# Vegeta2020/SE-SSD

Hardware: NVIDIA H100
Metric: frames_per_sec (higher is better)
Workload: dtype f32

## Files before the change

include/sessd_b200.h:

```cpp
#ifndef SESSD_B200_H
#define SESSD_B200_H

#include <stddef.h>
#include <stdint.h>

#ifdef __cplusplus
extern "C" {
#endif

#define SESSD_OK 0
#define SESSD_EINVAL (-1)
#define SESSD_ECAPACITY (-2)
#define SESSD_EWORKSPACE (-3)

const char *sessd_version(void);
long long sessd_launch_count(void);

typedef struct {
    float voxel_size[3];
    float range_min[3];
    float range_max[3];
    int grid[3];
    int max_points;
    int max_voxels;
    int num_feat;
} sessd_voxel_cfg;

size_t sessd_voxelize_workspace_bytes(int max_total_points, int batch, const sessd_voxel_cfg *cfg);

int sessd_voxelize(const float *d_points, const int *d_frame_off, int batch, int max_total_points,
                   const sessd_voxel_cfg *cfg, float *d_voxels, int *d_coors, int *d_num_points, float *d_mean,
                   int *d_num_voxels, void *workspace, size_t workspace_bytes, void *stream);

int sessd_voxelize_host(const float *h_points, int num_points, const sessd_voxel_cfg *cfg, float *h_voxels,
                        int *h_coors_zyx , int *h_num_points);

typedef struct {
    int batch;
    int shape[3];
} sessd_grid;

size_t sessd_hash_bytes(int max_rows, int *capacity_out);
int sessd_hash_build(const int *d_coors , const int *d_n, int max_rows, sessd_grid grid,
                     uint64_t *d_table, int capacity, void *stream);

size_t sessd_bitmap_words(sessd_grid grid);
size_t sessd_scan_scratch_bytes(size_t n_items);

int sessd_subm_rulebook(const int *d_coors, const int *d_n, int max_rows, sessd_grid grid, const int ksize[3],
                        int index_kind , const void *d_index, int hash_capacity,
                        int *d_nbr, void *stream);

int sessd_strided_rulebook(const int *d_in_coors, const int *d_n_in, int max_in, sessd_grid in_grid,
                           int in_index_kind, const void *d_in_index, int in_hash_capacity,
                           const int ksize[3], const int stride[3], const int padding[3],
                           sessd_grid out_grid, void *d_out_bitmap , void *d_scan_scratch,
                           int *d_out_coors, int *d_n_out, int max_out, int *d_nbr, int *d_status, void *stream);

int sessd_tile_list_stride(int kvol);
int sessd_rulebook_tile_lists(const int *d_nbr, int kvol, const int *d_n_out, int max_out, void *d_tiles, void *stream);
size_t sessd_rulebook_pairs_workspace_bytes(int max_rows, int kvol);
int sessd_rulebook_pairs(const int *d_nbr, const int *d_n_out, int max_rows, int kvol, int *d_pairs_in,
                         int *d_pairs_out, int *d_pair_num, void *workspace, size_t workspace_bytes, void *stream);

int sessd_spconv_forward(const float *d_in_feat, int cin, const int *d_nbr, int kvol, const int *d_n_out,
                         int max_out, const float *d_weight, int cout, const float *d_scale, const float *d_shift,
                         int relu, float *d_out_feat, void *stream);

int sessd_sparse_to_dense(const float *d_feat, const int *d_coors, const int *d_n, int max_rows, int channels,
                          sessd_grid grid, float *d_out, void *stream);
int sessd_sparse_to_dense_indexed(const float *d_feat, int max_rows, const void *d_bitmap_index, int channels, sessd_grid grid,
                                  float *d_out, void *stream);

int sessd_spconv_forward_rows(const float *d_in_feat, int cin, const int *d_nbr, int kvol, const int *d_n_out, int max_out,
                              const float *d_weight, int cout, const float *d_scale, const float *d_shift, int relu,
                              float *d_out_feat, float *d_amax_out, void *stream);
int sessd_spconv_forward_rows_planes(const float *d_in_feat, int cin, const int *d_nbr, int kvol, const int *d_n_out, int max_out,
                                     const float *d_weight, int cout, const float *d_scale, const float *d_shift, int relu,
                                     const float *d_amax_in, float gain, float shift_max, float *d_out_feat, void *d_out_planes, int cpo,
                                     float *d_out_info, void *stream);
int sessd_spconv_forward_cg(const void *d_in_planes, int cp, int plane_rows, const float *d_in_info, const void *d_tiles, int kvol,
                            const int *d_n_out, int max_out, const void *d_weight_h2, int cout, const float *d_scale, const float *d_shift,
                            int relu, float gain, float shift_max, float *d_out_f32, void *d_out_planes, float *d_out_info, void *stream);
void sessd_set_sp_cg_deep(int on);
int sessd_spconv_cg_blocks_per_sm(int cp, int cout, int deep);
int sessd_absmax_rows(const float *d_feat, const int *d_n, int max_rows, int channels, float *d_amax, void *stream);

int sessd_rulebook_transpose(const int *d_nbr, int kvol, const int *d_n_out, int max_out, int max_in, int *d_nbr_t, void *stream);
int sessd_sparse_split_planes(const float *d_x, const int *d_n, int max_rows, int channels, float *d_info, void *d_planes, int cp, void *stream);
int sessd_dense_grad_gather(const float *d_grad, const int *d_coors, const int *d_n, int max_rows, int channels, sessd_grid grid,
                            float *d_out, void *stream);
int sessd_spconv_wgrad_items(int max_out, int kvol);
size_t sessd_spconv_wgrad_workspace_bytes(int max_out, int kvol, int cin, int cout);
int sessd_spconv_wgrad_rows(const float *d_in_feat, int cin, const float *d_gout, int cout, const void *d_tiles, int kvol,
                            const int *d_n_out, int max_out, float *d_gw, void *d_ws, size_t ws_bytes, void *stream);
int sessd_spconv_wgrad_cg(const void *d_in_planes, int cp, const float *d_in_info, const void *d_g_planes, int cout, const float *d_g_info,
                          const void *d_tiles, int kvol, const int *d_n_out, int max_out, float *d_gw, void *d_ws, size_t ws_bytes,
                          void *stream);

typedef struct {
    int batch, in_h, in_w, cin;
    int out_h, out_w, cout;
    int grid_h, grid_w;
    int in_stride;
    int out_stride, out_off_y, out_off_x;
    int ntaps;
    int tap_dy[16], tap_dx[16];
    int relu;
} sessd_conv_desc;

int sessd_bev_conv_p2(const void *d_in_planes, const float *d_in_info, const void *d_weight_h2, int cout_pad, const float *d_scale,
                      const float *d_shift, const float *d_residual, const float *d_resid_info, float gain, float shift_max,
                      float *d_out_f32, void *d_out_planes, float *d_out_info, const sessd_conv_desc *desc, const int *d_items,
                      void *stream);
int sessd_bev_deconv_p2(const void *d_in_planes, const float *d_in_info, const void *d_weight_h2, int cout_pad, const float *d_scale,
                        const float *d_shift, const float *d_residual, const float *d_resid_info, float gain, float shift_max,
                        float *d_out_f32, void *d_out_planes, float *d_out_info, int batch, int in_h, int in_w, int cin, int cout,
                        int relu, const int *d_items, void *stream);
long long sessd_bev_skip_plan_words(int batch, int h, int w, int *offsets);
int sessd_bev_skip_plan(const void *d_bitmap_index, sessd_grid grid, int *d_plan, void *stream);
int sessd_bev_skip_fill(const int *d_record, float *d_out_f32, void *d_out_planes, int cout, void *stream);
int sessd_bev_wgrad_items(const sessd_conv_desc *desc);
size_t sessd_bev_wgrad_workspace_bytes(const sessd_conv_desc *desc);
int sessd_bev_wgrad(const void *d_in_planes, const float *d_in_info, const void *d_g_planes, const float *d_g_info,
                    const sessd_conv_desc *desc, float *d_gw, void *d_ws, size_t ws_bytes, void *stream);
int sessd_bev_split_planes(const float *d_x, long long n, float *d_info, void *d_planes, void *stream);
int sessd_sparse_to_dense_planes(const float *d_feat, int max_rows, const void *d_bitmap_index, int channels, sessd_grid grid,
                                 const float *d_amax, float *d_info, void *d_planes, void *stream);
int sessd_ssfa_fuse_planes(const float *d_x0, const float *d_x1, const float *d_w0, const float *d_w1, float s0, float t0, float s1,
                           float t1, int num_pixels, int channels, float *d_out, const float *d_info0, const float *d_info1,
                           float *d_out_info, void *d_planes, void *stream);

int sessd_absmax(const float *d_x, long long n, float *d_amax, void *stream);


typedef struct {
    float cnt_thresh;
    float dist_edge[4];
    float sigma2[3];
    float suppressed_thresh;
    float centerness_pow;
    int centerness;
} sessd_dinms_cfg;

#define SESSD_DINMS_MAX_PRE 4096

typedef struct {
    int batch;
    int num_anchors;
    int anchors_per_loc;
    int head_stride;
    float score_thresh;
    int nms_pre_max;
    int nms_post_max;
    float nms_iou_thresh;
    int nms_ge;
    float post_range[6];
    float direction_offset;
    int use_frustum;
    int nms_mode;
    sessd_dinms_cfg dinms;
} sessd_post_cfg;

size_t sessd_postprocess_workspace_bytes(const sessd_post_cfg *cfg);

int sessd_postprocess(const float *d_head, const float *d_anchors, const float *d_frustum,
                      const sessd_post_cfg *cfg, float *d_boxes, float *d_scores, int *d_labels, int *d_count,
                      int *d_aux, int *d_sel_anchor, void *workspace, size_t workspace_bytes, void *stream);

int sessd_postprocess_packed(const float *d_head, const float *d_anchors, const float *d_frustum,
                             const sessd_post_cfg *cfg, float *d_boxes, float *d_scores, int *d_labels, int *d_count,
                             int *d_aux, int *d_sel_anchor, float *d_packed, int *d_meta, const int *d_num_voxels,
                             const int *d_status, void *workspace, size_t workspace_bytes, void *stream);

size_t sessd_rotate_nms_workspace_bytes(int max_boxes, int pre_max);
int sessd_rotate_nms(const float *d_boxes5, const float *d_scores, const int *d_n, int max_boxes, int pre_max,
                     int post_max, float iou_thresh, int ge, int *d_keep, int *d_num_keep, void *workspace,
                     size_t workspace_bytes, void *stream);

size_t sessd_rotate_weighted_nms_workspace_bytes(int max_boxes, int pre_max);
int sessd_rotate_weighted_nms(const float *d_boxes7, const float *d_boxes5, const float *d_scores, const float *d_iou_preds,
                              const int *d_labels, const int *d_dirs, const float *d_anchors, const int *d_n, int max_boxes,
                              int pre_max, const sessd_dinms_cfg *cfg, float *d_out_boxes, float *d_out_scores, int *d_out_labels,
                              int *d_out_dirs, int *d_keep, int *d_selected, int *d_count, void *workspace, size_t workspace_bytes,
                              void *stream);

int sessd_boxes_overlap_bev(const float *d_a, int n, const float *d_b, int m, float *d_out, void *stream);
int sessd_boxes_aligned_overlap_bev(const float *d_a, const float *d_b, int n, float *d_out, void *stream);
int sessd_boxes_iou_bev(const float *d_a, int n, const float *d_b, int m, float *d_out, void *stream);
int sessd_boxes_iou3d(const float *d_a, int n, const float *d_b, int m, float *d_out, void *stream);
size_t sessd_nms_workspace_bytes(int n);
int sessd_nms_sorted(const float *d_boxes, int n, float thresh, int mode, long long *d_keep, int *d_num_keep,
                     void *workspace, size_t workspace_bytes, void *stream);

size_t sessd_assign_workspace_bytes(int num_anchors, int batch, int max_gt);
int sessd_assign_targets(const float *d_anchors, int num_anchors, const float *d_gt_boxes, const int *d_num_gt, int batch,
                         int max_gt, float matched_thr, float unmatched_thr, int *d_labels, float *d_bbox_targets,
                         float *d_bbox_outside_weights, int *d_pos_anchor, int *d_pos_gt_id, int *d_num_pos,
                         void *workspace, size_t workspace_bytes, void *stream);

#define SESSD_AUGMENT_MAX_GT 256
#define SESSD_AUGMENT_MAX_TRY 128
int sessd_box_collision(const double *d_boxes, int n, const double *d_qboxes, int k, uint8_t *d_out, void *stream);
int sessd_noise_per_box(const float *d_gt_boxes, const int *d_num_gt, const uint8_t *d_valid, int batch, int max_gt,
                        const double *d_loc_noise, const double *d_rot_noise, int num_try, double context, int *d_selected,
                        void *stream);
int sessd_points_in_boxes(const float *d_points, int n, int point_stride, const float *d_boxes, int m, double context, uint8_t *d_mask,
                          void *stream);
int sessd_augment_points(const float *d_points, const int *d_frame_off, int batch, int max_frame_points, const float *d_gt_boxes,
                         const int *d_num_gt, const uint8_t *d_valid, int max_gt, const double *d_loc_noise, const double *d_rot_noise,
                         int num_try, const int *d_selected, double context, const float *d_global, const int *d_perm,
                         const uint8_t *d_labeled, float *d_points_raw, float *d_points_out, void *stream);
int sessd_augment_boxes(const float *d_gt_boxes, const int *d_num_gt, const uint8_t *d_valid, const uint8_t *d_target, int batch,
                        int max_gt, const double *d_loc_noise, const double *d_rot_noise, int num_try, const int *d_selected,
                        const float *d_global, const float *range_bev, float *d_boxes_raw, int *d_num_raw, float *d_boxes_out,
                        int *d_num_out, float *d_boxes_global, int *d_num_global, void *stream);

int sessd_gtaug_select_host(const double *h_corners, int num_boxes, int num_cand, uint8_t *h_accepted);
size_t sessd_gtaug_paste_workspace_bytes(int batch, int num_points, int num_objects);
int sessd_gtaug_paste(const float *d_points, const int *d_frame_off, int batch, int num_points, const int *d_obj_off, const int *d_obj_ids,
                      int num_objects, int max_paste_points, const float *d_db_points, const int *d_db_off, const int *d_db_count,
                      const double *d_db_boxes, int db_size, void *d_workspace, size_t workspace_bytes, float *d_points_out, int capacity,
                      int *d_frame_off_out, void *stream);

#define SESSD_SADA_MAX_IDS (6 * SESSD_AUGMENT_MAX_GT)
int sessd_sada_pyramids(const float *d_boxes, int num_boxes, float *d_pyramids, float *d_planes, void *stream);
int sessd_sada_membership(const float *d_points, int n, const int *d_n, const float *d_planes, int num_pyramids, const int *d_ids, int num_ids,
                          uint32_t *d_bits, int *d_counts, void *stream);
size_t sessd_sada_compact_workspace_bytes(int n);
int sessd_sada_compact(const float *d_points, int n, const int *d_n, const uint32_t *d_bits, int num_ids, const int *d_counts, int min_count,
                       void *d_workspace, size_t workspace_bytes, float *d_out, int capacity, int *d_num_out, void *stream);
size_t sessd_sada_fps_workspace_bytes(int n, int num_ids);
int sessd_sada_fps(const float *d_points, int n, const int *d_n, const uint32_t *d_bits, int num_ids, const int *d_counts, int min_count, int k,
                   void *d_workspace, size_t workspace_bytes, float *d_out, int capacity, int *d_num, void *stream);
int sessd_sada_swap(const float *d_points, int n, const int *d_n, const uint32_t *d_bits, int num_pairs, const int *d_counts, const float *d_pyramids,
                    int num_pyramids, const int *d_ids, int max_swap_points, float *d_out, int capacity, const int *d_num_in,
                    int *d_num_out, void *stream);
int sessd_sada_shuffle(const float *d_points, const int *d_frame_off, int batch, int max_frame_points, const int *d_perm, float *d_out,
                       void *stream);

size_t sessd_prep_frustum_compact_workspace_bytes(int num_points);
int sessd_prep_frustum_compact(const float *d_points, const int *d_frame_off, int batch, int num_points, const double *d_planes,
                               void *d_workspace, size_t workspace_bytes, float *d_points_out, int capacity, int *d_frame_off_out, void *stream);
int sessd_prep_box_count(const float *d_points, const int *d_frame_off, int batch, int num_points, const double *d_box_planes,
                         const int *d_box_off, int num_boxes, int *d_counts, void *stream);
size_t sessd_prep_box_gather_workspace_bytes(int num_boxes);
int sessd_prep_box_gather(const float *d_points, const int *d_frame_off, int batch, int num_points, const double *d_box_planes,
                          const double *d_centres, const int *d_box_off, int num_boxes, const int *d_counts, int num_rows, void *d_workspace,
                          size_t workspace_bytes, float *d_rows_out, int capacity, int *d_obj_off, void *stream);

size_t sessd_head_loss_workspace_bytes(int batch);
size_t sessd_odiou_loss_workspace_bytes(int batch);
int sessd_odiou_loss(const float *d_head, const float *d_anchors, const int *d_labels, const float *d_reg_targets, int batch,
                     int num_anchors, int anchors_per_loc, int head_stride, float w_odiou, const float *d_losses, float *d_odiou_sum,
                     float *d_grad_head, void *workspace, size_t workspace_bytes, void *stream);
int sessd_odiou_pairs_host(const float *h_gboxes, const float *h_qboxes, int n, float *h_odiou, float *h_grad_q);
size_t sessd_iou_pred_loss_workspace_bytes(int batch);
int sessd_iou_pred_loss(const float *d_head, const float *d_anchors, const int *d_labels, const float *d_reg_targets, int batch,
                        int num_anchors, int anchors_per_loc, int head_stride, float sigma, float w_iou, float *d_losses,
                        float *d_grad_head, void *workspace, size_t workspace_bytes, void *stream);
int sessd_head_loss(const float *d_head, const float *d_anchors, const int *d_labels, const float *d_reg_targets, int batch,
                    int num_anchors, int anchors_per_loc, int head_stride, float alpha, float sigma, float dir_offset,
                    float pos_cls_weight, float neg_cls_weight, float w_cls, float w_loc, float w_dir, float *d_losses,
                    float *d_grad_head, void *workspace, size_t workspace_bytes, void *stream);

int sessd_axpby(float *d_y, const float *d_x, float a, float b, long long n, void *stream);
int sessd_adamw_step(float *d_param, const float *d_grad, float *d_exp_avg, float *d_exp_avg_sq, long long n, float lr, float beta1,
                     float beta2, float eps, float weight_decay, int step, void *stream);
size_t sessd_grad_sqnorm_workspace_bytes(long long n);
int sessd_grad_sqnorm(const float *d_x, long long n, float max_norm, float *d_out, void *d_workspace, void *stream);
int sessd_adamw_clip_ema_step(float *d_param, float *d_grad, float *d_exp_avg, float *d_exp_avg_sq, long long n, float lr, float beta1,
                              float beta2, float eps, float weight_decay, int step, const float *d_clip_coef, float *d_ema, double ema_alpha,
                              void *stream);

#define SESSD_KITTI_REC 13
#define SESSD_KITTI_PERSON_SITTING 11
#define SESSD_KITTI_VAN 12
typedef struct {
    int num_frames;
    const int *gt_off;
    const double *gt;
    const int *gt_code;
    const int *gt_occluded;
    const int *dc_off;
    const double *dc;
    const int *dt_off;
    const int *dt_cnt;
    const double *dt;
    const int *dt_code;
    const long long *ov_off;
} SessdKittiFrames;
size_t sessd_kitti_convert_workspace_bytes(long long capacity);
int sessd_kitti_convert_detections(const float *d_boxes7, const float *d_scores, const int *d_labels, const int *d_off, int num_frames,
                                   long long capacity, const double *d_calib, const int *d_image_hw, const int *d_label_code,
                                   int num_labels, double *d_rec, int *d_label, int *d_code, int *d_cnt, void *workspace,
                                   size_t workspace_bytes, void *stream);
int sessd_kitti_overlaps(const SessdKittiFrames *frames, int metric, int z_axis, double z_center, double *d_overlaps, void *stream);
size_t sessd_kitti_eval_workspace_bytes(int num_frames, long long total_gt, long long overlap_elems, int num_configs, int compute_aos);
int sessd_kitti_eval(const SessdKittiFrames *frames, int max_frame_dt, int metric, int z_axis, double z_center, int num_configs,
                     const int *d_cfg, const double *d_min_overlap, int compute_aos, long long total_gt, long long overlap_elems,
                     double *d_thresholds, int *d_num_thresholds, double *d_precision, double *d_aos, double *d_map, void *workspace,
                     size_t workspace_bytes, void *stream);

#ifdef __cplusplus
}
#endif
#endif
```

se-ssd_b200/csrc/bevconv_p2.cu:

```cuda
#include "bevconv_p2.cuh"

namespace sessd {

__global__ void __launch_bounds__(256) bev_split_planes_kernel(const float4 *__restrict__ x, long long n4, float *__restrict__ info,
                                                               __half *__restrict__ planes, long long plane_stride) {
    const float s = pow2_scale_for_bound(__ldg(info));
    if (blockIdx.x == 0 && threadIdx.x == 0) info[1] = s;
    for (long long i = blockIdx.x * (long long)blockDim.x + threadIdx.x; i < n4; i += (long long)gridDim.x * blockDim.x) {
        const float4 v = __ldg(x + i);
        const float a[4] = {v.x * s, v.y * s, v.z * s, v.w * s};
        __align__(8) __half hi[4], lo[4];
#pragma unroll
        for (int t = 0; t < 4; ++t) {
            hi[t] = __float2half_rn(a[t]);
            lo[t] = __float2half_rn(a[t] - __half2float(hi[t]));
        }
        *reinterpret_cast<uint2 *>(planes + 4 * i) = *reinterpret_cast<const uint2 *>(hi);
        *reinterpret_cast<uint2 *>(planes + plane_stride + 4 * i) = *reinterpret_cast<const uint2 *>(lo);
    }
}

}

using namespace sessd;

extern "C" int sessd_bev_conv_p2(const void *d_in_planes, const float *d_in_info, const void *d_weight_h2, int cout_pad, const float *d_scale,
                                 const float *d_shift, const float *d_residual, const float *d_resid_info, float gain, float shift_max,
                                 float *d_out_f32, void *d_out_planes, float *d_out_info, const sessd_conv_desc *desc, const int *d_items,
                                 void *stream) {
    return p2_conv<kP2Planes>(d_in_planes, d_in_info, d_weight_h2, cout_pad, d_scale, d_shift, d_residual, d_resid_info, gain, shift_max,
                              d_out_f32, d_out_planes, d_out_info, desc, stream, d_items);
}

extern "C" int sessd_bev_deconv_p2(const void *d_in_planes, const float *d_in_info, const void *d_weight_h2, int cout_pad, const float *d_scale,
                                   const float *d_shift, const float *d_residual, const float *d_resid_info, float gain, float shift_max,
                                   float *d_out_f32, void *d_out_planes, float *d_out_info, int batch, int in_h, int in_w, int cin, int cout,
                                   int relu, const int *d_items, void *stream) {
    return p2_deconv<kP2Planes>(d_in_planes, d_in_info, d_weight_h2, cout_pad, d_scale, d_shift, d_residual, d_resid_info, gain, shift_max,
                                d_out_f32, d_out_planes, d_out_info, batch, in_h, in_w, cin, cout, relu, stream, d_items);
}

extern "C" int sessd_bev_split_planes(const float *d_x, long long n, float *d_info, void *d_planes, void *stream) {
    if (!d_x || !d_info || !d_planes || n < 4 || (n & 3) || ((uintptr_t)d_x & 15)) return SESSD_EINVAL;
    SESSD_LAUNCH(bev_split_planes_kernel, persistent_grid(n / 4, 256), 256, 0, stream, reinterpret_cast<const float4 *>(d_x), n / 4, d_info,
                 (__half *)d_planes, n);
    return last_error();
}
```

se-ssd_b200/csrc/bevconv_p2.cuh:

```cuda
#pragma once
#include <cuda_fp16.h>

#include "tc_common.cuh"

namespace sessd {

constexpr int kP2TileU = 8, kP2TileV = 16;
constexpr int kP2MaxCopies = 6, kP2MaxRowsV = 18;
constexpr int kP2BStages = 6, kP2MaxBStages = 12;
constexpr int kP2MmaWarps = 8;
constexpr int kP2PatchWarp = 8, kP2WeightWarp = 9;
constexpr int kP2Threads = 320;
constexpr int kP2ThreadsRegA = 384, kP2RegsConsumer = 232, kP2RegsProducer = 40;
static_assert(2 * (kP2RegsConsumer - 168) <= 168 - kP2RegsProducer, "the consumers take what the producers release");
constexpr int kP2MaxSmem = 227 * 1024;
constexpr int kP2Chunk = 32;
constexpr int kP2ItemsHeader = 32;
enum { kP2Planes = 0, kP2SplitF16 = 1 };
enum { kP2NoProbe = 0, kP2ProbeClocks = 1, kP2ProbeLoads = 2 };

struct P2Params {
    int batch, cin, cout;
    int in_stride;
    int out_h, out_w;
    int grid_u, grid_v;
    int u_is_x;
    int out_stride, nclass;
    int cls_ntaps[4], cls_off_u[4], cls_off_v[4];
    int tap_copy[4][9], tap_row[4][9], tap_w[4][9];
    int ncopies, rows_v, pitch_u;
    int copy_u[kP2MaxCopies], copy_v[kP2MaxCopies];
    int copy_bytes, patch_bytes, npatch;
    int load_bytes, staging_bytes;
    int bring_bytes;
    int out_info_scale;
    const float *in_amax;
    int relu, n_tile, nblocks;
    int bstages, bstage_bytes;
    int tiles_u, tiles_v, tiles, total;
    int cls_order[4];
    const float *in_info;
    const float *resid_info;
    float gain, shift_max;
    float *out_info;
    long long out_plane_stride;
    const int *items;
    long long *prof;
};

enum P2Prof {
    kProfCta,
    kProfItems,
    kProfSteps,
    kProfItemClk,
    kProfBFull,
    kProfPatchFull,
    kProfMmaWait,
    kProfEpilogue,
    kProfPatchEmpty,
    kProfPatchTotal,
    kProfBEmpty,
    kProfBTotal,
    kP2ProfWords = 16
};

__device__ __forceinline__ int p2_item_count(const P2Params &p) { return p.items ? __ldg(p.items) : p.total; }
__device__ __forceinline__ int p2_item(const P2Params &p, int k) { return p.items ? __ldg(p.items + kP2ItemsHeader + k) : k; }

struct P2ItemIndex { int rank, nb, t; };
__host__ __device__ __forceinline__ P2ItemIndex p2_item_index(int g, int nblocks, int tiles) {
    const int rank = g / (nblocks * tiles), rem = g - rank * (nblocks * tiles), nb = rem / tiles;
    return {rank, nb, rem - nb * tiles};
}

struct P2Item { int cls, n0, b, u0, v0, ntaps; };

__device__ __forceinline__ P2Item p2_decode(const P2Params &p, int g) {
    P2Item it;
    const P2ItemIndex ix = p2_item_index(g, p.nblocks, p.tiles);
    int t = ix.t;
    it.cls = p.cls_order[ix.rank];
    it.n0 = ix.nb * p.n_tile;
    const int tu = t % p.tiles_u; t /= p.tiles_u;
    const int tv = t % p.tiles_v;
    it.b = t / p.tiles_v;
    it.u0 = tu * kP2TileU; it.v0 = tv * kP2TileV;
    it.ntaps = p.cls_ntaps[it.cls];
    return it;
}

template <int N>
__device__ __forceinline__ void p2_wgmma(float *d, uint64_t da, uint64_t db, uint32_t accumulate) {
    if constexpr (N == 32) wgmma_f16_n32(d, da, db, accumulate);
    else if constexpr (N == 64) wgmma_f16_n64(d, da, db, accumulate);
    else if constexpr (N == 128) wgmma_f16_n128(d, da, db, accumulate);
    else wgmma_f16_n256(d, da, db, accumulate);
}

template <int N>
__device__ __forceinline__ void p2_wgmma_ra(float *d, const uint32_t *a, uint64_t db, uint32_t accumulate) {
    if constexpr (N == 32) wgmma_f16_ra_n32(d, a, db, accumulate);
    else if constexpr (N == 64) wgmma_f16_ra_n64(d, a, db, accumulate);
    else if constexpr (N == 128) wgmma_f16_ra_n128(d, a, db, accumulate);
    else wgmma_f16_ra_n256(d, a, db, accumulate);
}

template <bool PROFILE>
__device__ __forceinline__ long long p2_tick() {
    if constexpr (PROFILE) return clock64();
    return 0;
}
template <bool PROFILE>
__device__ __forceinline__ void p2_tock(long long &clk, long long t0) {
    if constexpr (PROFILE) clk += clock64() - t0;
}

__device__ __forceinline__ void p2_split_patch(const P2Params &p, const unsigned char *staging, unsigned char *planes, float s_in, int ctid) {
    const int rows = p.rows_v * kP2TileU;
    const int copy_in = p.staging_bytes / p.ncopies;
    const int items = p.ncopies * rows * 4;
    for (int i = ctid; i < items; i += kP2MmaWarps * 32) {
        const int j = i & 3, r = (i >> 2) % rows, c = (i >> 2) / rows;
        unsigned char *hi = planes + 2 * c * p.copy_bytes + r * 64 + ((j ^ ((r >> 1) & 3)) << 4);
        const float4 *src = reinterpret_cast<const float4 *>(staging + c * copy_in + r * 128 + j * 32);
        const float4 a = src[0], b = src[1];
        const float x[8] = {a.x * s_in, a.y * s_in, a.z * s_in, a.w * s_in, b.x * s_in, b.y * s_in, b.z * s_in, b.w * s_in};
        __align__(16) __half h[8], l[8];
#pragma unroll
        for (int t = 0; t < 8; ++t) { h[t] = __float2half_rn(x[t]); l[t] = __float2half_rn(x[t] - __half2float(h[t])); }
        *reinterpret_cast<uint4 *>(hi) = *reinterpret_cast<const uint4 *>(h);
        *reinterpret_cast<uint4 *>(hi + p.copy_bytes) = *reinterpret_cast<const uint4 *>(l);
    }
    asm volatile("fence.proxy.async.shared::cta;\n" ::: "memory");
    asm volatile("bar.sync 1, %0;\n" ::"n"(kP2MmaWarps * 32) : "memory");
}

template <int NT, int MODE, bool REGA = false, int PROBE = kP2NoProbe>
__global__ void __launch_bounds__(REGA ? kP2ThreadsRegA : kP2Threads, 1) bev_conv_p2_kernel(const __grid_constant__ CUtensorMap map_a,
                                                                   const __grid_constant__ CUtensorMap map_b,
                                                                   const float *__restrict__ scale, const float *__restrict__ shift,
                                                                   const float *__restrict__ resid, float *__restrict__ out_f32,
                                                                   __half *__restrict__ out_planes, P2Params p) {
    static_assert(!REGA || MODE == kP2Planes, "register-fed A reads the TMA-written planes");
    constexpr bool PROFILE = PROBE != kP2NoProbe, LOADS_ONLY = PROBE == kP2ProbeLoads;
    extern __shared__ unsigned char smem_raw[];
    unsigned char *tiles = (unsigned char *)(((uintptr_t)smem_raw + 1023) & ~(uintptr_t)1023);
    unsigned char *patches = tiles + p.bring_bytes;
    unsigned char *staging = patches + p.npatch * p.patch_bytes;
    uint64_t *bars = (uint64_t *)(staging + p.npatch * p.staging_bytes);
    uint64_t *patch_full = bars, *patch_empty = bars + 2, *b_full = bars + 4, *b_empty = bars + 4 + kP2MaxBStages;
    uint32_t *s_aoff = (uint32_t *)(b_empty + kP2MaxBStages);
    float *s_scale = (float *)(((uintptr_t)(s_aoff + 4 * 9) + 15) & ~(uintptr_t)15), *s_shift = s_scale + p.cout;

    const int warp = threadIdx.x >> 5, lane = threadIdx.x & 31;
    if (threadIdx.x == kP2PatchWarp * 32) prefetch_tensormap(&map_a);
    if (threadIdx.x == kP2WeightWarp * 32) prefetch_tensormap(&map_b);
    const int nchunks = p.cin / kP2Chunk;
    const int nitems = p2_item_count(p);
    const uint32_t b_plane_bytes = (uint32_t)p.n_tile * 64u;

    if (threadIdx.x == 0) {
        for (int s = 0; s < 2; ++s) { mbar_init(&patch_full[s], 1); mbar_init(&patch_empty[s], kP2MmaWarps); }
        for (int s = 0; s < p.bstages; ++s) { mbar_init(&b_full[s], 1); mbar_init(&b_empty[s], kP2MmaWarps); }
        asm volatile("fence.mbarrier_init.release.cluster;\n" ::: "memory");
    }
    for (int idx = threadIdx.x; idx < p.nclass * 9; idx += blockDim.x) {
        const int c = idx / 9, t = idx - c * 9;
        s_aoff[idx] = REGA ? (uint32_t)p.tap_row[c][t] : (uint32_t)((2 * p.tap_copy[c][t] * p.copy_bytes + p.tap_row[c][t] * 512) >> 4);
    }
    for (int n = threadIdx.x; n < p.cout; n += blockDim.x) {
        s_scale[n] = scale ? __ldg(scale + n) : 1.f;
        s_shift[n] = shift ? __ldg(shift + n) : 0.f;
    }
    __syncthreads();
    long long clk[kP2ProfWords] = {};
    const long long t_start = p2_tick<PROFILE>();
    long long *prof_rec = PROFILE ? p.prof + (size_t)blockIdx.x * kP2ProfWords : nullptr;

    if (warp >= kP2MmaWarps) {
        if constexpr (REGA) setmaxnreg_dec<kP2RegsProducer>();
        if (warp == kP2PatchWarp) {
            int pb = 0;
            uint32_t pph = 0;
            const uint32_t patches_u32 = smem_u32(patches);
            for (int k = blockIdx.x; k < nitems; k += gridDim.x) {
                const P2Item it = p2_decode(p, p2_item(p, k));
                const int bu = it.u0 * p.in_stride, bv = it.v0 * p.in_stride;
                for (int cc = 0; cc < nchunks; ++cc) {
                    { const long long t0 = p2_tick<PROFILE>(); mbar_wait<REGA>(&patch_empty[pb], pph ^ 1u); p2_tock<PROFILE>(clk[kProfPatchEmpty], t0); }
                    if (elect_one()) {
                        mbar_expect_tx(&patch_full[pb], (uint32_t)p.load_bytes);
                        if constexpr (MODE == kP2Planes) {
                            uint32_t dst = patches_u32 + (uint32_t)(pb * p.patch_bytes);
                            for (int c = 0; c < p.ncopies; ++c, dst += 2u * (uint32_t)p.copy_bytes) {
                                const int cu = bu + p.copy_u[c], cv = bv + p.copy_v[c];
                                tma_load_5d(dst, &map_a, &patch_full[pb], cc * kP2Chunk, cu, cv, it.b, 0);
                                tma_load_5d(dst + (uint32_t)p.copy_bytes, &map_a, &patch_full[pb], cc * kP2Chunk, cu, cv, it.b, 1);
                            }
                        } else {
                            const uint32_t copy_in = (uint32_t)(p.staging_bytes / p.ncopies);
                            uint32_t dst = smem_u32(staging) + (uint32_t)(pb * p.staging_bytes);
                            for (int c = 0; c < p.ncopies; ++c, dst += copy_in)
                                tma_load_5d(dst, &map_a, &patch_full[pb], cc * kP2Chunk, bu + p.copy_u[c], bv + p.copy_v[c], it.b, 0);
                        }
                    }
                    __syncwarp();
                    if (++pb == p.npatch) { pb = 0; pph ^= 1u; }
                }
            }
            if constexpr (PROFILE)
                if (lane == 0) {
                    prof_rec[kProfPatchEmpty] = clk[kProfPatchEmpty];
                    prof_rec[kProfPatchTotal] = clock64() - t_start;
                }
        } else if (warp == kP2WeightWarp) {
            int S = 0;
            uint32_t bph = 0;
            for (int k = blockIdx.x; k < nitems; k += gridDim.x) {
                const P2Item it = p2_decode(p, p2_item(p, k));
                for (int cc = 0; cc < nchunks; ++cc)
                    for (int tap = 0; tap < it.ntaps; ++tap) {
                        { const long long t0 = p2_tick<PROFILE>(); mbar_wait<REGA>(&b_empty[S], bph ^ 1u); p2_tock<PROFILE>(clk[kProfBEmpty], t0); }
                        if (elect_one()) {
                            unsigned char *st = tiles + S * p.bstage_bytes;
                            const int wtap = p.tap_w[it.cls][tap];
                            mbar_expect_tx(&b_full[S], 2 * b_plane_bytes);
                            tma_load_4d(st + b_plane_bytes, &map_b, &b_full[S], cc * kP2Chunk, it.n0, wtap, 0);
                            tma_load_4d(st, &map_b, &b_full[S], cc * kP2Chunk, it.n0, wtap, 1);
                        }
                        __syncwarp();
                        if (++S == p.bstages) { S = 0; bph ^= 1u; }
                    }
            }
            if constexpr (PROFILE)
                if (lane == 0) {
                    prof_rec[kProfBEmpty] = clk[kProfBEmpty];
                    prof_rec[kProfBTotal] = clock64() - t_start;
                }
        }
    } else {
        if constexpr (REGA) setmaxnreg_inc<kP2RegsConsumer>();
        const int wg = warp >> 2, wq = warp & 3;
        constexpr int kAcc = NT / 2;
        const uint32_t a_rows = (uint32_t)(wg * 64 * 64) >> 4;
        const uint32_t tiles_lo = desc_lo(smem_u32(tiles));
        const uint32_t patch_lo = desc_lo(smem_u32(patches)) + a_rows;
        const uint32_t plane_lo = b_plane_bytes >> 4;
        const uint32_t copy_lo = (uint32_t)(p.copy_bytes >> 4), patch_sz = (uint32_t)(p.patch_bytes >> 4);
        const uint32_t a_row = (uint32_t)((wg * 8 + wq * 2 + ((lane >> 3) & 1)) * p.pitch_u + (lane & 7)), a_chunk = (uint32_t)(lane >> 4);
        const uint32_t patches_u32 = smem_u32(patches);
        float amax_in = 0.f, s_in = 1.f;
        if constexpr (MODE == kP2Planes) { amax_in = __ldg(p.in_info); s_in = __ldg(p.in_info + 1); }
        if constexpr (MODE == kP2SplitF16) if (p.in_amax) { amax_in = __ldg(p.in_amax); s_in = pow2_scale_for_bound(amax_in); }
        const float inv_sa = 1.f / s_in;
        float bound = amax_in * p.gain + p.shift_max;
        if (p.resid_info) bound += __ldg(p.resid_info);
        const float s_out = pow2_scale_for_bound(bound);
        if (blockIdx.x == 0 && threadIdx.x == 0 && p.out_info && p.out_info_scale) p.out_info[1] = s_out;
        float vmax = 0.f;
        const int per_cls = p.nblocks * p.tiles;
        int S = 0, pb = 0;
        uint32_t bph = 0, pph = 0;
        for (int k = blockIdx.x; k < nitems; k += gridDim.x) {
            const long long t_item = p2_tick<PROFILE>();
            const int g = p2_item(p, k);
            const int cls = p.cls_order[g / per_cls];
            const int ntaps = p.cls_ntaps[cls];
            const uint32_t *aoff = s_aoff + cls * 9;
            float acc[NT];
#pragma unroll
            for (int i = 0; i < NT; ++i) acc[i] = 0.f;
            int prevS = -1, prev_pb = -1;
            bool first = true;
            if constexpr (REGA) {
                uint32_t frag[2][16];
                int tap = 0;
                uint32_t pbase = 0;
                auto load_frags = [&](uint32_t *fa) {
                    if (tap == 0) {
                        { const long long t0 = p2_tick<PROFILE>(); mbar_wait<REGA>(&patch_full[pb], pph); p2_tock<PROFILE>(clk[kProfPatchFull], t0); }
                        pbase = patches_u32 + (uint32_t)(pb * p.patch_bytes);
                    }
                    if constexpr (!LOADS_ONLY) {
                        const uint32_t r = a_row + aoff[tap];
                        const uint32_t a_hi = pbase + r * 64u + ((a_chunk ^ ((r >> 1) & 3u)) << 4), a_lo = a_hi + (uint32_t)p.copy_bytes;
                        ldsm_x4(fa, a_hi);
                        ldsm_x4(fa + 4, a_hi ^ 32u);
                        ldsm_x4(fa + 8, a_lo);
                        ldsm_x4(fa + 12, a_lo ^ 32u);
                    }
                };
                auto step_ra = [&](const uint32_t *fa, uint32_t *fn, bool more) {
                    { const long long t0 = p2_tick<PROFILE>(); mbar_wait<REGA>(&b_full[S], bph); p2_tock<PROFILE>(clk[kProfBFull], t0); }
                    const uint64_t db_lo = kDescSw64Hi | (uint64_t)(tiles_lo + (uint32_t)(S * (p.bstage_bytes >> 4)));
                    const uint64_t db_hi = db_lo + (uint64_t)plane_lo;
                    if constexpr (!LOADS_ONLY) {
                        wgmma_fence();
                        p2_wgmma_ra<2 * NT>(acc, fa, db_lo, first ? 0u : 1u);
                        p2_wgmma_ra<2 * NT>(acc, fa + 4, db_lo + 2, 1u);
                        wgmma_commit();
                    }
                    first = false;
                    if constexpr (PROFILE) ++clk[kProfSteps];
                    { const long long t0 = p2_tick<PROFILE>(); wgmma_wait<1>(); p2_tock<PROFILE>(clk[kProfMmaWait], t0); }
                    if (lane == 0 && prevS >= 0) mbar_arrive(&b_empty[prevS]);
                    prevS = S;
                    if (++S == p.bstages) { S = 0; bph ^= 1u; }
                    if (++tap == ntaps) {
                        tap = 0;
                        if (lane == 0) mbar_arrive(&patch_empty[pb]);
                        if (++pb == p.npatch) { pb = 0; pph ^= 1u; }
                    }
                    if (more) load_frags(fn);
                    if constexpr (!LOADS_ONLY) {
                        wgmma_fence();
                        p2_wgmma_ra<NT>(acc, fa + 8, db_hi, 1u);
                        p2_wgmma_ra<NT>(acc, fa + 12, db_hi + 2, 1u);
                        wgmma_commit();
                    }
                };
                const int nsteps = nchunks * ntaps;
                load_frags(frag[0]);
#pragma unroll 1
                for (int st = 0; st + 1 < nsteps; st += 2) { step_ra(frag[0], frag[1], true); step_ra(frag[1], frag[0], st + 2 < nsteps); }
                if (nsteps & 1) step_ra(frag[0], frag[1], false);
            } else {
                for (int cc = 0; cc < nchunks; ++cc) {
                    { const long long t0 = p2_tick<PROFILE>(); mbar_wait(&patch_full[pb], pph); p2_tock<PROFILE>(clk[kProfPatchFull], t0); }
                    if constexpr (MODE == kP2SplitF16)
                        p2_split_patch(p, staging + pb * p.staging_bytes, patches + pb * p.patch_bytes, s_in, threadIdx.x);
                    const uint32_t pbase = patch_lo + (uint32_t)pb * patch_sz;
#pragma unroll 1
                    for (int tap = 0; tap < ntaps; ++tap) {
                        { const long long t0 = p2_tick<PROFILE>(); mbar_wait(&b_full[S], bph); p2_tock<PROFILE>(clk[kProfBFull], t0); }
                        if constexpr (!LOADS_ONLY) {
                            const uint64_t da_hi = kDescSw64Hi | (uint64_t)(pbase + aoff[tap]);
                            const uint64_t da_lo = da_hi + (uint64_t)copy_lo;
                            const uint64_t db_lo = kDescSw64Hi | (uint64_t)(tiles_lo + (uint32_t)(S * (p.bstage_bytes >> 4)));
                            const uint64_t db_hi = db_lo + (uint64_t)plane_lo;
                            const uint32_t accum = first ? 0u : 1u;
                            wgmma_fence();
                            if constexpr (MODE == kP2Planes) {
                                p2_wgmma<2 * NT>(acc, da_hi, db_lo, accum);
                                p2_wgmma<2 * NT>(acc, da_hi + 2, db_lo + 2, 1u);
                            } else {
                                p2_wgmma<NT>(acc + kAcc, da_hi, db_hi, accum);
                                p2_wgmma<NT>(acc + kAcc, da_hi + 2, db_hi + 2, 1u);
                                p2_wgmma<NT>(acc, da_hi, db_lo, accum);
                                p2_wgmma<NT>(acc, da_hi + 2, db_lo + 2, 1u);
                            }
                            p2_wgmma<NT>(acc, da_lo, db_hi, 1u);
                            p2_wgmma<NT>(acc, da_lo + 2, db_hi + 2, 1u);
                            wgmma_commit();
                        }
                        first = false;
                        if constexpr (PROFILE) ++clk[kProfSteps];
                        { const long long t0 = p2_tick<PROFILE>(); wgmma_wait<1>(); p2_tock<PROFILE>(clk[kProfMmaWait], t0); }
                        if (lane == 0) {
                            if (prevS >= 0) mbar_arrive(&b_empty[prevS]);
                            if (prev_pb >= 0) mbar_arrive(&patch_empty[prev_pb]);
                        }
                        prevS = S;
                        prev_pb = (tap == ntaps - 1) ? pb : -1;
                        if (++S == p.bstages) { S = 0; bph ^= 1u; }
                    }
                    if (p.npatch == 1) {
                        { const long long t0 = p2_tick<PROFILE>(); wgmma_wait<0>(); p2_tock<PROFILE>(clk[kProfMmaWait], t0); }
                        if (lane == 0) {
                            mbar_arrive(&b_empty[prevS]);
                            mbar_arrive(&patch_empty[pb]);
                        }
                        prevS = prev_pb = -1;
                    }
                    if (++pb == p.npatch) { pb = 0; pph ^= 1u; }
                }
            }
            { const long long t0 = p2_tick<PROFILE>(); wgmma_wait<0>(); p2_tock<PROFILE>(clk[kProfMmaWait], t0); }
            const long long t_epi = p2_tick<PROFILE>();
            wgmma_fence_regs<NT>(acc);
            if (lane == 0) {
                if (prevS >= 0) mbar_arrive(&b_empty[prevS]);
                if (prev_pb >= 0) mbar_arrive(&patch_empty[prev_pb]);
            }
#pragma unroll
            for (int i = 0; i < kAcc; ++i) acc[i] = acc[kAcc + i] + acc[i];
            const P2Item it = p2_decode(p, g);
            const int q = lane & 3;
            const int r0 = wg * 64 + wq * 16 + (lane >> 2);
            bool rows_ok[2];
            size_t opixs[2];
#pragma unroll
            for (int h = 0; h < 2; ++h) {
                const int r = r0 + 8 * h;
                const int lv = r / kP2TileU, lu = r % kP2TileU;
                const int gu = it.u0 + lu, gv = it.v0 + lv;
                rows_ok[h] = it.b < p.batch && gu < p.grid_u && gv < p.grid_v;
                const int ou = gu * p.out_stride + p.cls_off_u[it.cls], ov = gv * p.out_stride + p.cls_off_v[it.cls];
                const int oy = p.u_is_x ? ov : ou, ox = p.u_is_x ? ou : ov;
                opixs[h] = ((size_t)it.b * p.out_h + (size_t)oy) * p.out_w + (size_t)ox;
            }
#pragma unroll
            for (int j = 0; j < (LOADS_ONLY ? 0 : NT / 32); ++j)
#pragma unroll
                for (int h = 0; h < 2; ++h) {
                    const bool row_ok = rows_ok[h];
                    const size_t opix = opixs[h];
                    float v[8], o[8] = {};
                    quad_transpose8(acc + 16 * j + 2 * h, q, v);
                    const int n = it.n0 + 32 * j + 8 * q;
                    const size_t off = opix * p.cout + n;
                    if (row_ok && n < p.cout) {
                        float sc[8], sh[8];
#pragma unroll
                        for (int t = 0; t < 8; t += 4) {
                            const float4 a = *reinterpret_cast<const float4 *>(s_scale + n + t);
                            const float4 b = *reinterpret_cast<const float4 *>(s_shift + n + t);
                            sc[t] = a.x; sc[t + 1] = a.y; sc[t + 2] = a.z; sc[t + 3] = a.w;
                            sh[t] = b.x; sh[t + 1] = b.y; sh[t + 2] = b.z; sh[t + 3] = b.w;
                        }
#pragma unroll
                        for (int t = 0; t < 8; ++t) {
                            o[t] = fmaf(v[t] * inv_sa, sc[t], sh[t]);
                            if (p.relu) o[t] = fmaxf(o[t], 0.f);
                        }
                        if (resid) {
#pragma unroll
                            for (int t = 0; t < 8; t += 4) {
                                const float4 rr = __ldg(reinterpret_cast<const float4 *>(resid + off + t));
                                o[t] += rr.x; o[t + 1] += rr.y; o[t + 2] += rr.z; o[t + 3] += rr.w;
                            }
                        }
#pragma unroll
                        for (int t = 0; t < 8; ++t) vmax = fmaxf(vmax, fabsf(o[t]));
                        if (out_planes) {
                            __align__(16) __half2 hi[4], lo[4];
#pragma unroll
                            for (int t = 0; t < 4; ++t) {
                                const float x0 = o[2 * t] * s_out, x1 = o[2 * t + 1] * s_out;
                                hi[t] = __floats2half2_rn(x0, x1);
                                const float2 f = __half22float2(hi[t]);
                                lo[t] = __floats2half2_rn(x0 - f.x, x1 - f.y);
                            }
                            *reinterpret_cast<uint4 *>(out_planes + off) = *reinterpret_cast<const uint4 *>(hi);
                            *reinterpret_cast<uint4 *>(out_planes + p.out_plane_stride + off) = *reinterpret_cast<const uint4 *>(lo);
                        }
                    }
                    if (out_f32) {
                        const bool up = q & 2;
                        float keep[4], recv[4];
#pragma unroll
                        for (int t = 0; t < 4; ++t) {
                            keep[t] = up ? o[4 + t] : o[t];
                            recv[t] = __shfl_xor_sync(0xFFFFFFFFu, up ? o[t] : o[4 + t], 2);
                        }
                        const int n_lo = it.n0 + 32 * j + 8 * (q & 1), c_lo = n_lo + 4 * (q >> 1);
                        const float4 w_lo = up ? make_float4(recv[0], recv[1], recv[2], recv[3]) : make_float4(keep[0], keep[1], keep[2], keep[3]);
                        const float4 w_hi = up ? make_float4(keep[0], keep[1], keep[2], keep[3]) : make_float4(recv[0], recv[1], recv[2], recv[3]);
                        if (row_ok && n_lo < p.cout) *reinterpret_cast<float4 *>(out_f32 + opix * p.cout + c_lo) = w_lo;
                        if (row_ok && n_lo + 16 < p.cout) *reinterpret_cast<float4 *>(out_f32 + opix * p.cout + c_lo + 16) = w_hi;
                    }
                }
            if constexpr (PROFILE) {
                const long long t_end = clock64();
                clk[kProfEpilogue] += t_end - t_epi;
                clk[kProfItemClk] += t_end - t_item;
                ++clk[kProfItems];
            }
        }
        if constexpr (PROFILE)
            if (threadIdx.x == 0) {
                clk[kProfCta] = clock64() - t_start;
                for (int w = kProfCta; w <= kProfEpilogue; ++w) prof_rec[w] = clk[w];
            }
        if (p.out_info) {
            const unsigned m = __reduce_max_sync(0xFFFFFFFFu, __float_as_uint(vmax));
            if (lane == 0 && m != 0u) atomicMax(reinterpret_cast<unsigned *>(p.out_info), m);
        }
    }
}

static int encode_map_nd(CUtensorMap *m, const void *base, int rank, const cuuint64_t *dims, const cuuint64_t *strides_bytes ,
                         const cuuint32_t *box, const cuuint32_t *estr, CUtensorMapSwizzle swz,
                         CUtensorMapDataType dtype = CU_TENSOR_MAP_DATA_TYPE_FLOAT16) {
    EncodeTiledFn enc = get_tensor_map_encoder();
    if (!enc) return SESSD_EINVAL;
    CUresult r = enc(m, dtype, (cuuint32_t)rank, const_cast<void *>(base), dims, strides_bytes, box, estr,
                     CU_TENSOR_MAP_INTERLEAVE_NONE, swz, CU_TENSOR_MAP_L2_PROMOTION_L2_256B, CU_TENSOR_MAP_FLOAT_OOB_FILL_NONE);
    return r == CUDA_SUCCESS ? 0 : 700 + (int)r;
}

struct P2Taps { int n, dy[9], dx[9], w[9], off_y, off_x; };

static void p2_deconv_classes(P2Taps cls[4]) {
    for (int c = 0; c < 4; ++c) {
        P2Taps &k = cls[c];
        k = {};
        k.off_y = c >> 1; k.off_x = c & 1;
        for (int dy = k.off_y; dy >= 0; --dy)
            for (int dx = k.off_x; dx >= 0; --dx, ++k.n) {
                k.dy[k.n] = dy; k.dx[k.n] = dx; k.w[k.n] = (k.off_y + 1 - 2 * dy) * 3 + (k.off_x + 1 - 2 * dx);
            }
    }
}

constexpr int p2_n_tile(int cout) { return cout <= 32 ? 32 : 128; }

struct P2Geometry {
    int u_is_x, grid_u, grid_v, tiles_u, tiles_v, tiles;
    int n_tile, nblocks, nclass, total;
    int ntaps[4], off_u[4], off_v[4], order[4];
};

static int p2_geometry(P2Geometry &g, int batch, int grid_h, int grid_w, int cout, int cout_pad, const P2Taps *cls, int nclass) {
    g = {};
    if (batch < 1 || grid_h < 1 || grid_w < 1 || cout < 8 || cout % 8) return SESSD_EINVAL;
    g.n_tile = p2_n_tile(cout);
    if (cout_pad % g.n_tile || cout_pad < cout) return SESSD_EINVAL;
    g.u_is_x = div_up(grid_w, kP2TileU) * div_up(grid_h, kP2TileV) <= div_up(grid_h, kP2TileU) * div_up(grid_w, kP2TileV);
    g.grid_u = g.u_is_x ? grid_w : grid_h; g.grid_v = g.u_is_x ? grid_h : grid_w;
    g.tiles_u = div_up(g.grid_u, kP2TileU); g.tiles_v = div_up(g.grid_v, kP2TileV);
    g.tiles = g.tiles_u * g.tiles_v * batch;
    g.nblocks = cout_pad / g.n_tile;
    g.nclass = nclass; g.total = nclass * g.nblocks * g.tiles;
    for (int c = 0; c < nclass; ++c) {
        g.ntaps[c] = cls[c].n;
        g.off_u[c] = g.u_is_x ? cls[c].off_x : cls[c].off_y;
        g.off_v[c] = g.u_is_x ? cls[c].off_y : cls[c].off_x;
        g.order[c] = c;
    }
    for (int i = 1; i < nclass; ++i)
        for (int k = i; k > 0 && g.ntaps[g.order[k]] > g.ntaps[g.order[k - 1]]; --k) {
            const int tmp = g.order[k]; g.order[k] = g.order[k - 1]; g.order[k - 1] = tmp;
        }
    return 0;
}

static int p2_plan(P2Params &p, const P2Taps *cls, int nclass, int grid_h, int grid_w, int cout_pad, int mode, bool reg_a, int *smem) {
    if (reg_a && (mode != kP2Planes || p.in_stride != 1)) return SESSD_EINVAL;
    if (p.cin < 64 || p.cin % 64) return SESSD_EINVAL;
    P2Geometry g;
    if (p2_geometry(g, p.batch, grid_h, grid_w, p.cout, cout_pad, cls, nclass)) return SESSD_EINVAL;
    p.u_is_x = g.u_is_x; p.grid_u = g.grid_u; p.grid_v = g.grid_v;
    p.tiles_u = g.tiles_u; p.tiles_v = g.tiles_v; p.tiles = g.tiles;
    p.n_tile = g.n_tile; p.nblocks = g.nblocks; p.nclass = g.nclass; p.total = g.total;
    for (int c = 0; c < 4; ++c) {
        p.cls_ntaps[c] = g.ntaps[c]; p.cls_off_u[c] = g.off_u[c]; p.cls_off_v[c] = g.off_v[c]; p.cls_order[c] = g.order[c];
    }
    const int s = p.in_stride;
    p.ncopies = 0;
    int key_u[kP2MaxCopies], key_vm[kP2MaxCopies], vmin[kP2MaxCopies], vmax[kP2MaxCopies];
    for (int c = 0; c < p.nclass; ++c)
        for (int t = 0; t < cls[c].n; ++t) {
            const int tu = p.u_is_x ? cls[c].dx[t] : cls[c].dy[t], tv = p.u_is_x ? cls[c].dy[t] : cls[c].dx[t];
            const int vm = ((tv % s) + s) % s;
            int k = 0;
            for (; k < p.ncopies; ++k)
                if (key_u[k] == tu && key_vm[k] == vm) break;
            if (k == p.ncopies) {
                if (p.ncopies == kP2MaxCopies) return SESSD_EINVAL;
                key_u[k] = tu; key_vm[k] = vm; vmin[k] = tv; vmax[k] = tv;
                ++p.ncopies;
            }
            vmin[k] = min(vmin[k], tv); vmax[k] = max(vmax[k], tv);
        }
    p.rows_v = 0;
    p.pitch_u = kP2TileU;
    for (int k = 0; k < p.ncopies; ++k) p.rows_v = max(p.rows_v, kP2TileV + (vmax[k] - vmin[k]) / s);
    if (p.rows_v > kP2MaxRowsV) return SESSD_EINVAL;
    for (int k = 0; k < p.ncopies; ++k) { p.copy_u[k] = key_u[k]; p.copy_v[k] = vmin[k]; }
    if (reg_a) {
        int umin = key_u[0], umax = key_u[0];
        for (int k = 1; k < p.ncopies; ++k) {
            umin = min(umin, key_u[k]); umax = max(umax, key_u[k]);
            vmin[0] = min(vmin[0], vmin[k]); vmax[0] = max(vmax[0], vmax[k]);
        }
        p.ncopies = 1;
        p.copy_u[0] = umin; p.copy_v[0] = vmin[0];
        p.pitch_u = kP2TileU + umax - umin; p.rows_v = kP2TileV + vmax[0] - vmin[0];
        if (p.pitch_u > 256 || p.rows_v > 256) return SESSD_EINVAL;
    }
    for (int c = 0; c < p.nclass; ++c) {
        for (int t = 0; t < cls[c].n; ++t) {
            const int tu = p.u_is_x ? cls[c].dx[t] : cls[c].dy[t], tv = p.u_is_x ? cls[c].dy[t] : cls[c].dx[t];
            const int vm = ((tv % s) + s) % s;
            int k = 0;
            for (; k < p.ncopies; ++k)
                if (key_u[k] == tu && key_vm[k] == vm) break;
            p.tap_copy[c][t] = reg_a ? 0 : k;
            p.tap_row[c][t] = reg_a ? (tv - p.copy_v[0]) * p.pitch_u + (tu - p.copy_u[0]) : (tv - vmin[k]) / s;
            p.tap_w[c][t] = cls[c].w[t];
        }
    }
    p.copy_bytes = (p.rows_v * p.pitch_u * 64 + 511) & ~511;
    p.patch_bytes = p.ncopies * 2 * p.copy_bytes;
    p.staging_bytes = mode == kP2Planes ? 0 : p.ncopies * p.rows_v * kP2TileU * kP2Chunk * 4;
    p.load_bytes = mode == kP2Planes ? p.ncopies * 2 * p.rows_v * p.pitch_u * 64 : p.staging_bytes;
    const int per_buf = p.patch_bytes + p.staging_bytes, bstage = 2 * p.n_tile * 64;
    const int tail = 1536 + 16 + 2 * 4 * p.cout;
    p.npatch = (kP2BStages * bstage + tail + 2 * per_buf <= kP2MaxSmem) ? 2 : 1;
    p.bstage_bytes = bstage;
    p.bstages = min((kP2MaxSmem - tail - p.npatch * per_buf) / bstage, kP2MaxBStages);
    if (p.bstages < 2) return SESSD_EINVAL;
    p.bring_bytes = p.bstages * bstage;
    *smem = p.bring_bytes + tail + p.npatch * per_buf;
    return 0;
}

template <int MODE, int PROBE = kP2NoProbe>
static int launch_p2(const void *d_in_planes, int in_h, int in_w, const float *d_in_info, const void *d_w, int w_taps, int cout_pad,
                     const float *d_scale, const float *d_shift, const float *d_residual, const float *d_resid_info, float gain,
                     float shift_max, float *d_out_f32, void *d_out_planes, float *d_out_info, P2Params &p, const P2Taps *cls, int nclass,
                     int grid_h, int grid_w, bool reg_a, void *stream) {
    if (!d_in_planes || !d_w || (!d_out_f32 && !d_out_planes)) return SESSD_EINVAL;
    if (MODE == kP2Planes && (!d_in_info || !d_scale)) return SESSD_EINVAL;
    if (MODE != kP2Planes && d_out_planes) return SESSD_EINVAL;
    if (((uintptr_t)d_scale | (uintptr_t)d_shift | (uintptr_t)d_residual | (uintptr_t)d_out_f32 | (uintptr_t)d_out_planes) & 15)
        return SESSD_EINVAL;
    int smem = 0;
    if (p2_plan(p, cls, nclass, grid_h, grid_w, cout_pad, MODE, reg_a, &smem)) return SESSD_EINVAL;
    if (p.items && cout_pad != div_up(p.cout, p.n_tile) * p.n_tile) return SESSD_EINVAL;
    const int s = p.in_stride;
    CUtensorMap map_a, map_b;
    if (MODE != kP2Planes) {
        const cuuint64_t row_w = (cuuint64_t)p.cin * 4, row_h = (cuuint64_t)in_w * p.cin * 4;
        const cuuint64_t dims[5] = {(cuuint64_t)p.cin, (cuuint64_t)(p.u_is_x ? in_w : in_h), (cuuint64_t)(p.u_is_x ? in_h : in_w),
                                    (cuuint64_t)p.batch, 1};
        const cuuint64_t strides[4] = {p.u_is_x ? row_w : row_h, p.u_is_x ? row_h : row_w, (cuuint64_t)in_h * in_w * p.cin * 4,
                                       (cuuint64_t)p.batch * in_h * in_w * p.cin * 4};
        const cuuint32_t box[5] = {(cuuint32_t)kP2Chunk, (cuuint32_t)(kP2TileU * s), (cuuint32_t)(p.rows_v * s), 1, 1};
        const cuuint32_t estr[5] = {1, (cuuint32_t)s, (cuuint32_t)s, 1, 1};
        int rc = encode_map_nd(&map_a, d_in_planes, 5, dims, strides, box, estr, CU_TENSOR_MAP_SWIZZLE_NONE, CU_TENSOR_MAP_DATA_TYPE_FLOAT32);
        if (rc) return rc;
    } else {
        const cuuint64_t row_w = (cuuint64_t)p.cin * 2, row_h = (cuuint64_t)in_w * p.cin * 2;
        const cuuint64_t dims[5] = {(cuuint64_t)p.cin, (cuuint64_t)(p.u_is_x ? in_w : in_h), (cuuint64_t)(p.u_is_x ? in_h : in_w),
                                    (cuuint64_t)p.batch, 2};
        const cuuint64_t strides[4] = {p.u_is_x ? row_w : row_h, p.u_is_x ? row_h : row_w, (cuuint64_t)in_h * in_w * p.cin * 2,
                                       (cuuint64_t)p.batch * in_h * in_w * p.cin * 2};
        const cuuint32_t box[5] = {(cuuint32_t)kP2Chunk, (cuuint32_t)(p.pitch_u * s), (cuuint32_t)(p.rows_v * s), 1, 1};
        const cuuint32_t estr[5] = {1, (cuuint32_t)s, (cuuint32_t)s, 1, 1};
        int rc = encode_map_nd(&map_a, d_in_planes, 5, dims, strides, box, estr, CU_TENSOR_MAP_SWIZZLE_64B);
        if (rc) return rc;
    }
    {
        const cuuint64_t dims[4] = {(cuuint64_t)p.cin, (cuuint64_t)cout_pad, (cuuint64_t)w_taps, 2};
        const cuuint64_t strides[3] = {(cuuint64_t)p.cin * 2, (cuuint64_t)cout_pad * p.cin * 2, (cuuint64_t)w_taps * cout_pad * p.cin * 2};
        const cuuint32_t box[4] = {(cuuint32_t)kP2Chunk, (cuuint32_t)p.n_tile, 1, 1};
        const cuuint32_t estr[4] = {1, 1, 1, 1};
        int rc = encode_map_nd(&map_b, d_w, 4, dims, strides, box, estr, CU_TENSOR_MAP_SWIZZLE_64B);
        if (rc) return rc;
    }
    constexpr bool kRegA = MODE == kP2Planes;
    auto kernel = bev_conv_p2_kernel<128, MODE, false, PROBE>;
    if (p.n_tile == 32) kernel = reg_a ? bev_conv_p2_kernel<32, MODE, kRegA, PROBE> : bev_conv_p2_kernel<32, MODE, false, PROBE>;
    else if (reg_a) kernel = bev_conv_p2_kernel<128, MODE, kRegA, PROBE>;
    static bool attr_done[2][2] = {};
    if (!attr_done[p.n_tile == 32][reg_a]) {
        SESSD_CUDA_TRY(cudaFuncSetAttribute(kernel, cudaFuncAttributeMaxDynamicSharedMemorySize, kP2MaxSmem));
        attr_done[p.n_tile == 32][reg_a] = true;
    }
    p.in_info = MODE == kP2Planes ? d_in_info : nullptr;
    p.in_amax = MODE == kP2SplitF16 ? d_in_info : nullptr;
    p.resid_info = d_residual ? d_resid_info : nullptr;
    if (d_residual && d_out_planes && !d_resid_info) return SESSD_EINVAL;
    p.gain = gain; p.shift_max = shift_max; p.out_info = d_out_info;
    p.out_info_scale = MODE == kP2Planes ? 1 : 0;
    if (d_out_planes && !d_out_info) return SESSD_EINVAL;
    p.out_plane_stride = (long long)p.batch * p.out_h * p.out_w * p.cout;
    static int num_sms = 0;
    if (!num_sms) {
        int dev = 0;
        SESSD_CUDA_TRY(cudaGetDevice(&dev));
        SESSD_CUDA_TRY(cudaDeviceGetAttribute(&num_sms, cudaDevAttrMultiProcessorCount, dev));
    }
    const int grid = p.total < num_sms ? p.total : num_sms;
    SESSD_LAUNCH(kernel, grid, reg_a ? kP2ThreadsRegA : kP2Threads, smem, (cudaStream_t)stream, map_a, map_b, d_scale, d_shift, d_residual, d_out_f32,
                 (__half *)d_out_planes, p);
    return last_error();
}


static int p2_conv_params(const sessd_conv_desc &d, P2Params &p, P2Taps &t) {
    if (d.ntaps < 1 || d.ntaps > 9 || (d.in_stride != 1 && d.in_stride != 2) || d.out_stride < 1) return SESSD_EINVAL;
    if ((d.grid_h - 1) * d.out_stride + d.out_off_y >= d.out_h || (d.grid_w - 1) * d.out_stride + d.out_off_x >= d.out_w) return SESSD_EINVAL;
    p = {};
    p.batch = d.batch; p.cin = d.cin; p.cout = d.cout; p.in_stride = d.in_stride;
    p.out_h = d.out_h; p.out_w = d.out_w; p.out_stride = d.out_stride; p.relu = d.relu;
    t = {};
    t.n = d.ntaps; t.off_y = d.out_off_y; t.off_x = d.out_off_x;
    for (int i = 0; i < d.ntaps; ++i) { t.dy[i] = d.tap_dy[i]; t.dx[i] = d.tap_dx[i]; t.w[i] = i; }
    return 0;
}

static void p2_deconv_params(int batch, int in_h, int in_w, int cin, int cout, int relu, P2Params &p, P2Taps cls[4]) {
    p = {};
    p.batch = batch; p.cin = cin; p.cout = cout; p.in_stride = 1;
    p.out_h = 2 * in_h; p.out_w = 2 * in_w; p.out_stride = 2; p.relu = relu;
    p2_deconv_classes(cls);
}

template <int MODE, int PROBE = kP2NoProbe>
static int p2_conv(const void *d_in_planes, const float *d_in_info, const void *d_weight_h2, int cout_pad, const float *d_scale,
                   const float *d_shift, const float *d_residual, const float *d_resid_info, float gain, float shift_max,
                   float *d_out_f32, void *d_out_planes, float *d_out_info, const sessd_conv_desc *desc, void *stream,
                   const int *d_items = nullptr, long long *d_prof = nullptr, bool smem_a = false) {
    if (!desc || (PROBE != kP2NoProbe && !d_prof)) return SESSD_EINVAL;
    const sessd_conv_desc &d = *desc;
    P2Params p;
    P2Taps t;
    if (p2_conv_params(d, p, t)) return SESSD_EINVAL;
    p.items = d_items;
    p.prof = d_prof;
    return launch_p2<MODE, PROBE>(d_in_planes, d.in_h, d.in_w, d_in_info, d_weight_h2, d.ntaps, cout_pad, d_scale, d_shift, d_residual, d_resid_info, gain,
                     shift_max, d_out_f32, d_out_planes, d_out_info, p, &t, 1, d.grid_h, d.grid_w, MODE == kP2Planes && d.in_stride == 1 && !smem_a,
                     stream);
}

template <int MODE, int PROBE = kP2NoProbe>
static int p2_deconv(const void *d_in_planes, const float *d_in_info, const void *d_weight_h2, int cout_pad, const float *d_scale,
                     const float *d_shift, const float *d_residual, const float *d_resid_info, float gain, float shift_max,
                     float *d_out_f32, void *d_out_planes, float *d_out_info, int batch, int in_h, int in_w, int cin, int cout,
                     int relu, void *stream, const int *d_items = nullptr, long long *d_prof = nullptr) {
    if (PROBE != kP2NoProbe && !d_prof) return SESSD_EINVAL;
    P2Params p;
    P2Taps cls[4];
    p2_deconv_params(batch, in_h, in_w, cin, cout, relu, p, cls);
    p.items = d_items;
    p.prof = d_prof;
    return launch_p2<MODE, PROBE>(d_in_planes, in_h, in_w, d_in_info, d_weight_h2, 9, cout_pad, d_scale, d_shift, d_residual, d_resid_info, gain, shift_max,
                     d_out_f32, d_out_planes, d_out_info, p, cls, 4, in_h, in_w, MODE == kP2Planes, stream);
}

}
```

se-ssd_b200/csrc/bevskip.cu:

```cuda
#include "bevconv_p2.cuh"

namespace sessd {

enum {
    kRecCount = 0, kRecSkipped = 1, kRecNclass = 2, kRecTiles = 3, kRecTilesU = 4, kRecTilesV = 5, kRecUisX = 6, kRecOutStride = 7,
    kRecOutH = 8, kRecOutW = 9, kRecBatch = 10, kRecOffY = 11, kRecOffX = 15, kRecRep = 19, kRecSkipOff = 23, kRecFlagOff = 24
};

enum { kMX, kMB0a, kMB0b, kMX0, kMM0, kMM1, kMO0, kMO1, kMOut, kMTmp, kMB1a, kMB1b, kMX1, kMTmpH, kNumMaps };
constexpr int kNumFullMaps = kMTmp + 1;
constexpr int kSkipLaunches = 13;
constexpr int kSkipThreads = 1024;

struct SkipLaunch : P2Geometry {
    int map;
    int out_stride, out_h, out_w;
    int rec;
};

struct SkipPlan {
    int batch, depth, h, w, h2, w2, nwf, nwh;
    SkipLaunch l[kSkipLaunches];
};

static int skip_launch(SkipLaunch &L, int map, int batch, int grid_h, int grid_w, int out_h, int out_w, int cout, bool deconv) {
    P2Taps cls[4] = {};
    if (deconv) p2_deconv_classes(cls);
    else cls[0].n = 1;
    L.map = map;
    L.out_stride = deconv ? 2 : 1;
    L.out_h = out_h; L.out_w = out_w;
    return p2_geometry(L, batch, grid_h, grid_w, cout, div_up(cout, p2_n_tile(cout)) * p2_n_tile(cout), cls, deconv ? 4 : 1);
}

static long long skip_plan(SkipPlan &P, int batch, int h, int w) {
    if (batch < 1 || h < 4 || w < 4 || (h & 1) || (w & 1)) return 0;
    P.batch = batch; P.h = h; P.w = w; P.h2 = h / 2; P.w2 = w / 2;
    P.nwf = div_up(w, 32); P.nwh = div_up(P.w2, 32);
    const int h2 = P.h2, w2 = P.w2;
    SkipLaunch *L = P.l;
    const int rc = skip_launch(L[0], kMB0a, batch, h, w, h, w, 128, false)
                 | skip_launch(L[1], kMB0b, batch, h, w, h, w, 128, false)
                 | skip_launch(L[2], kMX0, batch, h, w, h, w, 128, false)
                 | skip_launch(L[3], kMB1a, batch, h2, w2, h2, w2, 256, false)
                 | skip_launch(L[4], kMB1b, batch, h2, w2, h2, w2, 256, false)
                 | skip_launch(L[5], kMX1, batch, h2, w2, h2, w2, 256, false)
                 | skip_launch(L[6], kMX0, batch, h, w, h, w, 128, false)
                 | skip_launch(L[7], kMX1, batch, h2, w2, h2, w2, 256, false)
                 | skip_launch(L[8], kMM0, batch, h2, w2, h, w, 128, true)
                 | skip_launch(L[9], kMM1, batch, h2, w2, h, w, 128, true)
                 | skip_launch(L[10], kMO0, batch, h, w, h, w, 128, false)
                 | skip_launch(L[11], kMO1, batch, h, w, h, w, 128, false)
                 | skip_launch(L[12], kMOut, batch, h, w, h, w, 24, false);
    long long words = 0;
    for (int i = 0; i < kSkipLaunches; ++i) {
        L[i].rec = (int)words;
        words += kP2ItemsHeader + L[i].total + 2LL * L[i].nclass * L[i].tiles;
    }
    return rc ? 0 : words;
}

struct BitMap {
    uint32_t *w;
    int h, wd, nw;
    __device__ __forceinline__ bool get(int y, int x) const { return (w[y * nw + (x >> 5)] >> (x & 31)) & 1u; }
    __device__ __forceinline__ uint32_t valid(int i) const {
        const int rem = wd - 32 * i;
        return rem >= 32 ? ~0u : ((1u << rem) - 1u);
    }
};

__device__ void skip_dilate3(const BitMap &in, const BitMap &tmp, const BitMap &out) {
    const int n = in.h * in.nw, last = (in.wd - 1) >> 5;
    for (int idx = threadIdx.x; idx < n; idx += blockDim.x) {
        const int y = idx / in.nw, i = idx - y * in.nw;
        const uint32_t *r = in.w + y * in.nw;
        const uint32_t c = r[i], l = i > 0 ? r[i - 1] : 0u, rr = i + 1 < in.nw ? r[i + 1] : 0u;
        uint32_t hv = c | (c << 1) | (l >> 31) | (c >> 1) | (rr << 31);
        if (i == 0) hv |= 1u;
        if (i == last) hv |= 1u << ((in.wd - 1) & 31);
        tmp.w[idx] = hv & in.valid(i);
    }
    __syncthreads();
    for (int idx = threadIdx.x; idx < n; idx += blockDim.x) {
        const int y = idx / in.nw, i = idx - y * in.nw;
        out.w[idx] = (y == 0 || y == in.h - 1) ? in.valid(i) : (tmp.w[idx - in.nw] | tmp.w[idx] | tmp.w[idx + in.nw]);
    }
    __syncthreads();
}

template <class F>
__device__ void skip_map_from(const BitMap &out, F f) {
    const int warp = threadIdx.x >> 5, lane = threadIdx.x & 31, nwarps = blockDim.x >> 5;
    for (int idx = warp; idx < out.h * out.nw; idx += nwarps) {
        const int y = idx / out.nw, x = (idx - y * out.nw) * 32 + lane;
        const unsigned bits = __ballot_sync(0xFFFFFFFFu, x < out.wd && f(y, x));
        if (lane == 0) out.w[idx] = bits;
    }
    __syncthreads();
}

template <class Pred>
__device__ int skip_compact(int n, Pred pred, int *out, int *s_scan) {
    const int warp = threadIdx.x >> 5, lane = threadIdx.x & 31, nwarps = blockDim.x >> 5;
    int base = 0;
    for (int start = 0; start < n; start += blockDim.x) {
        const int i = start + threadIdx.x;
        const bool v = i < n && pred(i);
        const unsigned bal = __ballot_sync(0xFFFFFFFFu, v);
        if (lane == 0) s_scan[warp] = __popc(bal);
        __syncthreads();
        if (warp == 0) {
            const int own = lane < nwarps ? s_scan[lane] : 0;
            int x = own;
#pragma unroll
            for (int o = 1; o < 32; o <<= 1) {
                const int y = __shfl_up_sync(0xFFFFFFFFu, x, o);
                if (lane >= o) x += y;
            }
            if (lane < nwarps) s_scan[lane] = x - own;
            if (lane == 31) s_scan[32] = x;
        }
        __syncthreads();
        if (v) out[base + s_scan[warp] + __popc(bal & ((1u << lane) - 1u))] = i;
        base += s_scan[32];
        __syncthreads();
    }
    return base;
}

__global__ void __launch_bounds__(kSkipThreads) bev_skip_plan_kernel(const uint2 *__restrict__ bitmap, int *__restrict__ plan, SkipPlan P) {
    extern __shared__ uint32_t s_bits[];
    __shared__ int s_scan[33], s_rep[4];
    BitMap m[kNumMaps];
    {
        uint32_t *p = s_bits;
        for (int i = 0; i < kNumMaps; ++i) {
            const bool full = i < kNumFullMaps;
            m[i].w = p; m[i].h = full ? P.h : P.h2; m[i].wd = full ? P.w : P.w2; m[i].nw = full ? P.nwf : P.nwh;
            p += m[i].h * m[i].nw;
        }
    }
    for (int b = 0; b < P.batch; ++b) {
        const BitMap X = m[kMX];
        for (int idx = threadIdx.x; idx < X.h * X.nw; idx += blockDim.x) {
            const int y = idx / X.nw, i = idx - y * X.nw;
            const int nbits = min(32, X.wd - 32 * i);
            uint32_t acc = 0u;
            for (int z = 0; z < P.depth; ++z) {
                const unsigned long long lin = (((unsigned long long)b * P.depth + z) * P.h + y) * P.w + 32 * i;
                const unsigned sh = (unsigned)(lin & 31);
                const uint32_t lo = __ldg(&bitmap[lin >> 5]).x, hi = sh + nbits > 32 ? __ldg(&bitmap[(lin >> 5) + 1]).x : 0u;
                acc |= __funnelshift_r(lo, hi, sh);
            }
            X.w[idx] = acc & X.valid(i);
        }
        __syncthreads();
        skip_dilate3(m[kMX], m[kMTmp], m[kMB0a]);
        skip_dilate3(m[kMB0a], m[kMTmp], m[kMB0b]);
        skip_dilate3(m[kMB0b], m[kMTmp], m[kMX0]);
        skip_dilate3(m[kMX0], m[kMTmp], m[kMX]);
        {
            const BitMap D = m[kMX];
            skip_map_from(m[kMB1a], [&](int y, int x) { return D.get(2 * y, 2 * x); });
        }
        skip_dilate3(m[kMB1a], m[kMTmpH], m[kMB1b]);
        skip_dilate3(m[kMB1b], m[kMTmpH], m[kMX1]);
        {
            const BitMap T = m[kMX1], R = m[kMX0];
            auto tget = [&](int gy, int gx) { return gy >= T.h || gx >= T.wd || T.get(gy, gx); };
            auto dc = [&](int oy, int ox) {
                const int py = oy & 1, px = ox & 1, gy = oy >> 1, gx = ox >> 1;
                return tget(gy, gx) || (py && tget(gy + 1, gx)) || (px && tget(gy, gx + 1)) || (py && px && tget(gy + 1, gx + 1));
            };
            skip_map_from(m[kMM0], [&](int y, int x) { return dc(y, x) || R.get(y, x); });
            skip_map_from(m[kMM1], dc);
        }
        skip_dilate3(m[kMM0], m[kMTmp], m[kMO0]);
        skip_dilate3(m[kMM1], m[kMTmp], m[kMO1]);
        for (int i = threadIdx.x; i < P.h * P.nwf; i += blockDim.x) m[kMOut].w[i] = m[kMO0].w[i] | m[kMO1].w[i];
        __syncthreads();
        for (int li = 0; li < kSkipLaunches; ++li) {
            const SkipLaunch &L = P.l[li];
            const BitMap &o = m[L.map];
            int *flags = plan + L.rec + kP2ItemsHeader + L.total + L.nclass * L.tiles;
            const int per_frame = L.tiles_u * L.tiles_v;
            for (int idx = threadIdx.x; idx < L.nclass * per_frame; idx += blockDim.x) {
                const int c = idx / per_frame, tf = idx - c * per_frame;
                const int tu = tf % L.tiles_u, tv = tf / L.tiles_u;
                const int u0 = tu * kP2TileU, v0 = tv * kP2TileV;
                bool run = u0 + kP2TileU > L.grid_u || v0 + kP2TileV > L.grid_v;
                if (!run && L.out_stride == 1) {
                    const int y0 = L.u_is_x ? v0 : u0, x0 = L.u_is_x ? u0 : v0;
                    const int ny = L.u_is_x ? kP2TileV : kP2TileU, nx = L.u_is_x ? kP2TileU : kP2TileV;
                    const uint32_t field = (1u << nx) - 1u;
                    for (int y = y0; y < y0 + ny && !run; ++y) run = (o.w[y * o.nw + (x0 >> 5)] >> (x0 & 31)) & field;
                } else if (!run) {
                    for (int r = 0; r < kP2TileU * kP2TileV && !run; ++r) {
                        const int ou = (u0 + (r & 7)) * L.out_stride + L.off_u[c], ov = (v0 + (r >> 3)) * L.out_stride + L.off_v[c];
                        run = L.u_is_x ? o.get(ov, ou) : o.get(ou, ov);
                    }
                }
                flags[c * L.tiles + b * per_frame + tf] = run ? 1 : 0;
            }
        }
        __syncthreads();
    }
    for (int li = 0; li < kSkipLaunches; ++li) {
        const SkipLaunch &L = P.l[li];
        int *rec = plan + L.rec;
        int *items = rec + kP2ItemsHeader, *skipped = items + L.total;
        const int *flags = skipped + L.nclass * L.tiles;
        if (threadIdx.x < 4) s_rep[threadIdx.x] = 0x7FFFFFFF;
        __syncthreads();
        for (int e = threadIdx.x; e < L.nclass * L.tiles; e += blockDim.x)
            if (!flags[e]) atomicMin(&s_rep[e / L.tiles], e % L.tiles);
        __syncthreads();
        const int count = skip_compact(L.total, [&](int g) {
            const P2ItemIndex ix = p2_item_index(g, L.nblocks, L.tiles);
            return flags[L.order[ix.rank] * L.tiles + ix.t] != 0 || ix.t == s_rep[L.order[ix.rank]];
        }, items, s_scan);
        const int nskip = skip_compact(L.nclass * L.tiles, [&](int e) {
            return flags[e] == 0 && e % L.tiles != s_rep[e / L.tiles];
        }, skipped, s_scan);
        if (threadIdx.x == 0) {
            rec[kRecCount] = count; rec[kRecSkipped] = nskip;
            rec[kRecNclass] = L.nclass; rec[kRecTiles] = L.tiles; rec[kRecTilesU] = L.tiles_u; rec[kRecTilesV] = L.tiles_v;
            rec[kRecUisX] = L.u_is_x; rec[kRecOutStride] = L.out_stride; rec[kRecOutH] = L.out_h; rec[kRecOutW] = L.out_w;
            rec[kRecBatch] = P.batch;
            for (int c = 0; c < 4; ++c) {
                rec[kRecOffY + c] = L.u_is_x ? L.off_v[c] : L.off_u[c]; rec[kRecOffX + c] = L.u_is_x ? L.off_u[c] : L.off_v[c];
                rec[kRecRep + c] = c < L.nclass && s_rep[c] != 0x7FFFFFFF ? s_rep[c] : -1;
            }
            rec[kRecSkipOff] = kP2ItemsHeader + L.total;
            rec[kRecFlagOff] = kP2ItemsHeader + L.total + L.nclass * L.tiles;
        }
        __syncthreads();
    }
}

__global__ void __launch_bounds__(256) bev_skip_fill_kernel(const int *__restrict__ rec, float *__restrict__ out_f32,
                                                            __half *__restrict__ out_planes, int cout) {
    const int nskip = __ldg(rec + kRecSkipped);
    if ((int)blockIdx.x >= nskip) return;
    const int tiles = __ldg(rec + kRecTiles), tiles_u = __ldg(rec + kRecTilesU), tiles_v = __ldg(rec + kRecTilesV);
    const int u_is_x = __ldg(rec + kRecUisX), os = __ldg(rec + kRecOutStride), out_h = __ldg(rec + kRecOutH), out_w = __ldg(rec + kRecOutW);
    const long long plane_stride = (long long)__ldg(rec + kRecBatch) * out_h * out_w * cout;
    const int *skipped = rec + __ldg(rec + kRecSkipOff);
    for (int e = blockIdx.x; e < nskip; e += gridDim.x) {
        const int ent = __ldg(skipped + e);
        const int c = ent / tiles, t = ent - c * tiles, r = __ldg(rec + kRecRep + c);
        const int oy0 = __ldg(rec + kRecOffY + c), ox0 = __ldg(rec + kRecOffX + c);
        auto pixel = [&](int tt, int lu, int lv) -> size_t {
            const int tu = tt % tiles_u, rest = tt / tiles_u, tv = rest % tiles_v, b = rest / tiles_v;
            const int gu = tu * kP2TileU + lu, gv = tv * kP2TileV + lv;
            const int gy = u_is_x ? gv : gu, gx = u_is_x ? gu : gv;
            return ((size_t)b * out_h + (size_t)(gy * os + oy0)) * out_w + (size_t)(gx * os + ox0);
        };
        if (out_f32) {
            const int q = cout / 4;
            for (int i = threadIdx.x; i < kP2TileU * kP2TileV * q; i += blockDim.x) {
                const int px = i / q, j = i - px * q;
                const float4 v = reinterpret_cast<const float4 *>(out_f32 + pixel(r, px & 7, px >> 3) * cout)[j];
                reinterpret_cast<float4 *>(out_f32 + pixel(t, px & 7, px >> 3) * cout)[j] = v;
            }
        }
        if (out_planes) {
            const int q = cout / 8, n = kP2TileU * kP2TileV * q;
            for (int i = threadIdx.x; i < 2 * n; i += blockDim.x) {
                const int pl = i / n, k = i - pl * n, px = k / q, j = k - px * q;
                const __half *src = out_planes + pl * plane_stride + pixel(r, px & 7, px >> 3) * cout;
                __half *dst = out_planes + pl * plane_stride + pixel(t, px & 7, px >> 3) * cout;
                reinterpret_cast<uint4 *>(dst)[j] = reinterpret_cast<const uint4 *>(src)[j];
            }
        }
    }
}

}

using namespace sessd;

extern "C" long long sessd_bev_skip_plan_words(int batch, int h, int w, int *offsets) {
    SkipPlan P;
    const long long words = skip_plan(P, batch, h, w);
    if (words && offsets)
        for (int i = 0; i < kSkipLaunches; ++i) offsets[i] = P.l[i].rec;
    return words;
}

extern "C" int sessd_bev_skip_plan(const void *d_bitmap_index, sessd_grid grid, int *d_plan, void *stream) {
    if (!d_bitmap_index || !d_plan || grid.shape[0] < 1) return SESSD_EINVAL;
    SkipPlan P;
    if (!skip_plan(P, grid.batch, grid.shape[1], grid.shape[2])) return SESSD_EINVAL;
    P.depth = grid.shape[0];
    const int smem = 4 * (kNumFullMaps * P.h * P.nwf + (kNumMaps - kNumFullMaps) * P.h2 * P.nwh);
    if (smem > 200 * 1024) return SESSD_EINVAL;
    static int attr_smem = 48 * 1024;
    if (smem > attr_smem) {
        SESSD_CUDA_TRY(cudaFuncSetAttribute(bev_skip_plan_kernel, cudaFuncAttributeMaxDynamicSharedMemorySize, smem));
        attr_smem = smem;
    }
    SESSD_LAUNCH(bev_skip_plan_kernel, 1, kSkipThreads, smem, (cudaStream_t)stream, (const uint2 *)d_bitmap_index, d_plan, P);
    return last_error();
}

extern "C" int sessd_bev_skip_fill(const int *d_record, float *d_out_f32, void *d_out_planes, int cout, void *stream) {
    if (!d_record || (!d_out_f32 && !d_out_planes) || cout < 8 || cout % 8) return SESSD_EINVAL;
    SESSD_LAUNCH(bev_skip_fill_kernel, 2 * kNumSMs, 256, 0, (cudaStream_t)stream, d_record, d_out_f32, (__half *)d_out_planes, cout);
    return last_error();
}
```

se-ssd_b200/sessd_b200/_lib.py:

```python
import ctypes as C
import os

_HERE = os.path.dirname(os.path.abspath(__file__))
LIB_PATH = os.path.join(os.path.dirname(_HERE), "libsessd_b200.so")
LAB_PATH = os.path.join(os.path.dirname(_HERE), "libsessd_b200_lab.so")


class SessdError(RuntimeError):
    pass


class VoxelCfg(C.Structure):
    _fields_ = [("voxel_size", C.c_float * 3), ("range_min", C.c_float * 3), ("range_max", C.c_float * 3),
                ("grid", C.c_int * 3), ("max_points", C.c_int), ("max_voxels", C.c_int), ("num_feat", C.c_int)]


class Grid(C.Structure):
    _fields_ = [("batch", C.c_int), ("shape", C.c_int * 3)]


class ConvDesc(C.Structure):
    _fields_ = [("batch", C.c_int), ("in_h", C.c_int), ("in_w", C.c_int), ("cin", C.c_int),
                ("out_h", C.c_int), ("out_w", C.c_int), ("cout", C.c_int),
                ("grid_h", C.c_int), ("grid_w", C.c_int), ("in_stride", C.c_int),
                ("out_stride", C.c_int), ("out_off_y", C.c_int), ("out_off_x", C.c_int),
                ("ntaps", C.c_int), ("tap_dy", C.c_int * 16), ("tap_dx", C.c_int * 16), ("relu", C.c_int)]


class DinmsCfg(C.Structure):
    _fields_ = [("cnt_thresh", C.c_float), ("dist_edge", C.c_float * 4), ("sigma2", C.c_float * 3), ("suppressed_thresh", C.c_float),
                ("centerness_pow", C.c_float), ("centerness", C.c_int)]


class PostCfg(C.Structure):
    _fields_ = [("batch", C.c_int), ("num_anchors", C.c_int), ("anchors_per_loc", C.c_int), ("head_stride", C.c_int),
                ("score_thresh", C.c_float), ("nms_pre_max", C.c_int), ("nms_post_max", C.c_int),
                ("nms_iou_thresh", C.c_float), ("nms_ge", C.c_int), ("post_range", C.c_float * 6),
                ("direction_offset", C.c_float), ("use_frustum", C.c_int), ("nms_mode", C.c_int), ("dinms", DinmsCfg)]


class KittiFrames(C.Structure):
    _fields_ = [("num_frames", C.c_int), ("gt_off", C.c_void_p), ("gt", C.c_void_p), ("gt_code", C.c_void_p),
                ("gt_occluded", C.c_void_p), ("dc_off", C.c_void_p), ("dc", C.c_void_p), ("dt_off", C.c_void_p),
                ("dt_cnt", C.c_void_p), ("dt", C.c_void_p), ("dt_code", C.c_void_p), ("ov_off", C.c_void_p)]


_vp, _i, _f, _sz, _ll = C.c_void_p, C.c_int, C.c_float, C.c_size_t, C.c_longlong
_I3 = C.POINTER(C.c_int)

SIGNATURES = {
    "sessd_version": (C.c_char_p, []),
    "sessd_launch_count": (_ll, []),
    "sessd_voxelize_workspace_bytes": (_sz, [_i, _i, C.POINTER(VoxelCfg)]),
    "sessd_voxelize": (_i, [_vp, _vp, _i, _i, C.POINTER(VoxelCfg), _vp, _vp, _vp, _vp, _vp, _vp, _sz, _vp]),
    "sessd_voxelize_host": (_i, [_vp, _i, C.POINTER(VoxelCfg), _vp, _vp, _vp]),
    "sessd_hash_bytes": (_sz, [_i, _I3]),
    "sessd_hash_build": (_i, [_vp, _vp, _i, Grid, _vp, _i, _vp]),
    "sessd_bitmap_words": (_sz, [Grid]),
    "sessd_scan_scratch_bytes": (_sz, [_sz]),
    "sessd_subm_rulebook": (_i, [_vp, _vp, _i, Grid, _I3, _i, _vp, _i, _vp, _vp]),
    "sessd_strided_rulebook": (_i, [_vp, _vp, _i, Grid, _i, _vp, _i, _I3, _I3, _I3, Grid, _vp, _vp, _vp, _vp, _i, _vp, _vp, _vp]),
    "sessd_tile_list_stride": (_i, [_i]),
    "sessd_rulebook_tile_lists": (_i, [_vp, _i, _vp, _i, _vp, _vp]),
    "sessd_rulebook_pairs_workspace_bytes": (_sz, [_i, _i]),
    "sessd_rulebook_pairs": (_i, [_vp, _vp, _i, _i, _vp, _vp, _vp, _vp, _sz, _vp]),
    "sessd_spconv_forward": (_i, [_vp, _i, _vp, _i, _vp, _i, _vp, _i, _vp, _vp, _i, _vp, _vp]),
    "sessd_spconv_forward_rows": (_i, [_vp, _i, _vp, _i, _vp, _i, _vp, _i, _vp, _vp, _i, _vp, _vp, _vp]),
    "sessd_spconv_forward_rows_planes": (_i, [_vp, _i, _vp, _i, _vp, _i, _vp, _i, _vp, _vp, _i, _vp, _f, _f, _vp, _vp, _i, _vp, _vp]),
    "sessd_spconv_forward_cg": (_i, [_vp, _i, _i, _vp, _vp, _i, _vp, _i, _vp, _i, _vp, _vp, _i, _f, _f, _vp, _vp, _vp, _vp]),
    "sessd_set_sp_cg_deep": (None, [_i]),
    "sessd_spconv_cg_blocks_per_sm": (_i, [_i, _i, _i]),
    "sessd_absmax_rows": (_i, [_vp, _vp, _i, _i, _vp, _vp]),
    "sessd_rulebook_transpose": (_i, [_vp, _i, _vp, _i, _i, _vp, _vp]),
    "sessd_sparse_split_planes": (_i, [_vp, _vp, _i, _i, _vp, _vp, _i, _vp]),
    "sessd_dense_grad_gather": (_i, [_vp, _vp, _vp, _i, _i, Grid, _vp, _vp]),
    "sessd_spconv_wgrad_items": (_i, [_i, _i]),
    "sessd_spconv_wgrad_workspace_bytes": (_sz, [_i, _i, _i, _i]),
    "sessd_spconv_wgrad_rows": (_i, [_vp, _i, _vp, _i, _vp, _i, _vp, _i, _vp, _vp, _sz, _vp]),
    "sessd_spconv_wgrad_cg": (_i, [_vp, _i, _vp, _vp, _i, _vp, _vp, _i, _vp, _i, _vp, _vp, _sz, _vp]),
    "sessd_sparse_to_dense_indexed": (_i, [_vp, _i, _vp, _i, Grid, _vp, _vp]),
    "sessd_sparse_to_dense": (_i, [_vp, _vp, _vp, _i, _i, Grid, _vp, _vp]),
    "sessd_bev_conv_p2": (_i, [_vp, _vp, _vp, _i, _vp, _vp, _vp, _vp, _f, _f, _vp, _vp, _vp, C.POINTER(ConvDesc), _vp, _vp]),
    "sessd_bev_deconv_p2": (_i, [_vp, _vp, _vp, _i, _vp, _vp, _vp, _vp, _f, _f, _vp, _vp, _vp, _i, _i, _i, _i, _i, _i, _vp, _vp]),
    "sessd_bev_skip_plan_words": (_ll, [_i, _i, _i, _I3]),
    "sessd_bev_skip_plan": (_i, [_vp, Grid, _vp, _vp]),
    "sessd_bev_skip_fill": (_i, [_vp, _vp, _vp, _i, _vp]),
    "sessd_bev_wgrad_items": (_i, [C.POINTER(ConvDesc)]),
    "sessd_bev_wgrad_workspace_bytes": (_sz, [C.POINTER(ConvDesc)]),
    "sessd_bev_wgrad": (_i, [_vp, _vp, _vp, _vp, C.POINTER(ConvDesc), _vp, _vp, _sz, _vp]),
    "sessd_bev_split_planes": (_i, [_vp, _ll, _vp, _vp, _vp]),
    "sessd_sparse_to_dense_planes": (_i, [_vp, _i, _vp, _i, Grid, _vp, _vp, _vp, _vp]),
    "sessd_ssfa_fuse_planes": (_i, [_vp, _vp, _vp, _vp, _f, _f, _f, _f, _i, _i, _vp, _vp, _vp, _vp, _vp, _vp]),
    "sessd_absmax": (_i, [_vp, C.c_longlong, _vp, _vp]),
    "sessd_postprocess_workspace_bytes": (_sz, [C.POINTER(PostCfg)]),
    "sessd_postprocess": (_i, [_vp, _vp, _vp, C.POINTER(PostCfg), _vp, _vp, _vp, _vp, _vp, _vp, _vp, _sz, _vp]),
    "sessd_postprocess_packed": (_i, [_vp, _vp, _vp, C.POINTER(PostCfg), _vp, _vp, _vp, _vp, _vp, _vp, _vp, _vp, _vp, _vp, _vp, _sz, _vp]),
    "sessd_rotate_nms_workspace_bytes": (_sz, [_i, _i]),
    "sessd_rotate_nms": (_i, [_vp, _vp, _vp, _i, _i, _i, _f, _i, _vp, _vp, _vp, _sz, _vp]),
    "sessd_rotate_weighted_nms_workspace_bytes": (_sz, [_i, _i]),
    "sessd_rotate_weighted_nms": (_i, [_vp, _vp, _vp, _vp, _vp, _vp, _vp, _vp, _i, _i, C.POINTER(DinmsCfg), _vp, _vp, _vp, _vp, _vp, _vp, _vp,
                                       _vp, _sz, _vp]),
    "sessd_boxes_overlap_bev": (_i, [_vp, _i, _vp, _i, _vp, _vp]),
    "sessd_boxes_aligned_overlap_bev": (_i, [_vp, _vp, _i, _vp, _vp]),
    "sessd_boxes_iou_bev": (_i, [_vp, _i, _vp, _i, _vp, _vp]),
    "sessd_boxes_iou3d": (_i, [_vp, _i, _vp, _i, _vp, _vp]),
    "sessd_nms_workspace_bytes": (_sz, [_i]),
    "sessd_nms_sorted": (_i, [_vp, _i, _f, _i, _vp, _vp, _vp, _sz, _vp]),
    "sessd_head_loss_workspace_bytes": (_sz, [_i]),
    "sessd_head_loss": (_i, [_vp, _vp, _vp, _vp, _i, _i, _i, _i, _f, _f, _f, _f, _f, _f, _f, _f, _vp, _vp, _vp, _sz, _vp]),
    "sessd_odiou_loss_workspace_bytes": (_sz, [_i]),
    "sessd_odiou_loss": (_i, [_vp, _vp, _vp, _vp, _i, _i, _i, _i, _f, _vp, _vp, _vp, _vp, _sz, _vp]),
    "sessd_odiou_pairs_host": (_i, [_vp, _vp, _i, _vp, _vp]),
    "sessd_iou_pred_loss_workspace_bytes": (_sz, [_i]),
    "sessd_iou_pred_loss": (_i, [_vp, _vp, _vp, _vp, _i, _i, _i, _i, _f, _f, _vp, _vp, _vp, _sz, _vp]),
    "sessd_axpby": (_i, [_vp, _vp, _f, _f, _ll, _vp]),
    "sessd_adamw_step": (_i, [_vp, _vp, _vp, _vp, _ll, _f, _f, _f, _f, _f, _i, _vp]),
    "sessd_grad_sqnorm_workspace_bytes": (_sz, [_ll]),
    "sessd_grad_sqnorm": (_i, [_vp, _ll, _f, _vp, _vp, _vp]),
    "sessd_adamw_clip_ema_step": (_i, [_vp, _vp, _vp, _vp, _ll, _f, _f, _f, _f, _f, _i, _vp, _vp, C.c_double, _vp]),
    "sessd_assign_workspace_bytes": (_sz, [_i, _i, _i]),
    "sessd_assign_targets": (_i, [_vp, _i, _vp, _vp, _i, _i, _f, _f, _vp, _vp, _vp, _vp, _vp, _vp, _vp, _sz, _vp]),
    "sessd_box_collision": (_i, [_vp, _i, _vp, _i, _vp, _vp]),
    "sessd_noise_per_box": (_i, [_vp, _vp, _vp, _i, _i, _vp, _vp, _i, C.c_double, _vp, _vp]),
    "sessd_points_in_boxes": (_i, [_vp, _i, _i, _vp, _i, C.c_double, _vp, _vp]),
    "sessd_augment_points": (_i, [_vp, _vp, _i, _i, _vp, _vp, _vp, _i, _vp, _vp, _i, _vp, C.c_double, _vp, _vp, _vp, _vp, _vp, _vp]),
    "sessd_augment_boxes": (_i, [_vp, _vp, _vp, _vp, _i, _i, _vp, _vp, _i, _vp, _vp, C.POINTER(C.c_float), _vp, _vp, _vp, _vp, _vp, _vp, _vp]),
    "sessd_gtaug_select_host": (_i, [_vp, _i, _i, _vp]),
    "sessd_gtaug_paste_workspace_bytes": (_sz, [_i, _i, _i]),
    "sessd_gtaug_paste": (_i, [_vp, _vp, _i, _i, _vp, _vp, _i, _i, _vp, _vp, _vp, _vp, _i, _vp, _sz, _vp, _i, _vp, _vp]),
    "sessd_sada_pyramids": (_i, [_vp, _i, _vp, _vp, _vp]),
    "sessd_sada_membership": (_i, [_vp, _i, _vp, _vp, _i, _vp, _i, _vp, _vp, _vp]),
    "sessd_sada_compact_workspace_bytes": (_sz, [_i]),
    "sessd_sada_compact": (_i, [_vp, _i, _vp, _vp, _i, _vp, _i, _vp, _sz, _vp, _i, _vp, _vp]),
    "sessd_sada_fps_workspace_bytes": (_sz, [_i, _i]),
    "sessd_sada_fps": (_i, [_vp, _i, _vp, _vp, _i, _vp, _i, _i, _vp, _sz, _vp, _i, _vp, _vp]),
    "sessd_sada_swap": (_i, [_vp, _i, _vp, _vp, _i, _vp, _vp, _i, _vp, _i, _vp, _i, _vp, _vp, _vp]),
    "sessd_sada_shuffle": (_i, [_vp, _vp, _i, _i, _vp, _vp, _vp]),
    "sessd_prep_frustum_compact_workspace_bytes": (_sz, [_i]),
    "sessd_prep_frustum_compact": (_i, [_vp, _vp, _i, _i, _vp, _vp, _sz, _vp, _i, _vp, _vp]),
    "sessd_prep_box_count": (_i, [_vp, _vp, _i, _i, _vp, _vp, _i, _vp, _vp]),
    "sessd_prep_box_gather_workspace_bytes": (_sz, [_i]),
    "sessd_prep_box_gather": (_i, [_vp, _vp, _i, _i, _vp, _vp, _vp, _i, _vp, _i, _vp, _sz, _vp, _i, _vp, _vp]),
    "sessd_kitti_convert_workspace_bytes": (_sz, [_ll]),
    "sessd_kitti_convert_detections": (_i, [_vp, _vp, _vp, _vp, _i, _ll, _vp, _vp, _vp, _i, _vp, _vp, _vp, _vp, _vp, _sz, _vp]),
    "sessd_kitti_overlaps": (_i, [C.POINTER(KittiFrames), _i, _i, C.c_double, _vp, _vp]),
    "sessd_kitti_eval_workspace_bytes": (_sz, [_i, _ll, _ll, _i, _i]),
    "sessd_kitti_eval": (_i, [C.POINTER(KittiFrames), _i, _i, _i, C.c_double, _i, _vp, _vp, _i, _ll, _ll, _vp, _vp, _vp, _vp, _vp, _vp,
                              _sz, _vp]),
}


LAB_SIGNATURES = {
    "sessd_bev_conv_h2": (_i, [_vp, _vp, _i, _vp, _vp, _vp, _vp, C.POINTER(ConvDesc), _vp, _vp, _vp]),
    "sessd_bev_deconv_h2": (_i, [_vp, _vp, _i, _vp, _vp, _vp, _vp, _i, _i, _i, _i, _i, _i, _vp, _vp, _vp]),
    "sessd_bev_conv_p2_profile": (_i, [_vp, _vp, _vp, _i, _vp, _vp, _vp, _vp, _f, _f, _vp, _vp, _vp, C.POINTER(ConvDesc), _vp, _vp, _vp]),
    "sessd_bev_deconv_p2_profile": (_i, [_vp, _vp, _vp, _i, _vp, _vp, _vp, _vp, _f, _f, _vp, _vp, _vp, _i, _i, _i, _i, _i, _i, _vp, _vp,
                                         _vp]),
    "sessd_bev_conv_p2_loads": (_i, [_vp, _vp, _vp, _i, _vp, _vp, _vp, _vp, _f, _f, _vp, _vp, _vp, C.POINTER(ConvDesc), _vp, _i, _vp, _vp]),
    "sessd_bev_p2_plan": (_i, [C.POINTER(ConvDesc), _i, _i, _i, _i, _I3]),
}


def _load(path, signatures, mode=C.DEFAULT_MODE):
    if not os.path.exists(path):
        raise ImportError(
            "sessd_b200: %s is missing -- the CUDA library has not been built (run `python se-ssd_b200/build.py`). "
            "There is no CPU fallback." % path)
    lib = C.CDLL(path, mode=mode)
    for name, (res, args) in signatures.items():
        fn = getattr(lib, name)
        fn.restype = res
        fn.argtypes = args
    return lib


class _Libs:

    def __init__(self):
        self._prod = _load(LIB_PATH, SIGNATURES, C.RTLD_GLOBAL)
        self._lab = None

    def lab(self):
        if self._lab is None:
            self._lab = _load(LAB_PATH, LAB_SIGNATURES)
        return self._lab

    @property
    def lab_loaded(self):
        return self._lab is not None

    def __getattr__(self, name):
        if name in LAB_SIGNATURES:
            return getattr(self.lab(), name)
        return getattr(self._prod, name)


lib = _Libs()


def check(rc, what):
    if rc != 0:
        kind = {-1: "invalid argument", -2: "capacity exceeded", -3: "workspace too small"}.get(rc, "cudaError %d" % rc)
        raise SessdError("%s failed: %s" % (what, kind))


def version():
    return lib.sessd_version().decode()


def launch_count():
    return int(lib.sessd_launch_count())
```

se-ssd_b200/sessd_b200/ops.py:

```python
import ctypes as C

import numpy as np
import torch

from . import _lib
from ._lib import ConvDesc, DinmsCfg, Grid, PostCfg, VoxelCfg, check, lib


def _p(t):
    return C.c_void_p(t.data_ptr()) if t is not None else C.c_void_p(0)


def _st():
    return C.c_void_p(torch.cuda.current_stream().cuda_stream)


def _cuda(t, dtype, name):
    if not (isinstance(t, torch.Tensor) and t.is_cuda and t.dtype == dtype and t.is_contiguous()):
        raise ValueError("%s must be a contiguous CUDA %s tensor" % (name, dtype))
    return t


def _i3(v):
    return (C.c_int * 3)(*[int(x) for x in v])


def make_grid(batch, shape_dhw):
    g = Grid()
    g.batch = int(batch)
    g.shape[0], g.shape[1], g.shape[2] = [int(v) for v in shape_dhw]
    return g


def make_voxel_cfg(voxel_size, pc_range, max_points, max_voxels, num_feat=4):
    cfg = VoxelCfg()
    vs = np.asarray(voxel_size, np.float32)
    rg = np.asarray(pc_range, np.float32)
    grid = np.round((rg[3:] - rg[:3]) / vs).astype(np.int64)
    for j in range(3):
        cfg.voxel_size[j] = float(vs[j])
        cfg.range_min[j] = float(rg[j])
        cfg.range_max[j] = float(rg[3 + j])
        cfg.grid[j] = int(grid[j])
    cfg.max_points, cfg.max_voxels, cfg.num_feat = int(max_points), int(max_voxels), int(num_feat)
    return cfg


class VoxelBuffers:

    def __init__(self, cfg, batch, max_total_points, device, with_mean=True):
        self.cfg, self.batch, self.max_total_points = cfg, batch, max_total_points
        nv = batch * cfg.max_voxels
        self.voxels = torch.empty((nv, cfg.max_points, cfg.num_feat), dtype=torch.float32, device=device)
        self.coors = torch.empty((nv, 4), dtype=torch.int32, device=device)
        self.num_points = torch.empty((nv,), dtype=torch.int32, device=device)
        self.mean = torch.empty((nv, cfg.num_feat), dtype=torch.float32, device=device) if with_mean else None
        self.num_voxels = torch.zeros((batch + 1,), dtype=torch.int32, device=device)
        ws = lib.sessd_voxelize_workspace_bytes(max_total_points, batch, C.byref(cfg))
        self.ws = torch.empty((ws,), dtype=torch.uint8, device=device)


def voxelize(points, frame_off, buf):
    _cuda(points, torch.float32, "points")
    _cuda(frame_off, torch.int32, "frame_off")
    if points.shape[0] > buf.max_total_points or points.shape[1] != buf.cfg.num_feat or frame_off.numel() != buf.batch + 1:
        raise ValueError("voxelize: shape/capacity mismatch")
    rc = lib.sessd_voxelize(_p(points), _p(frame_off), buf.batch, buf.max_total_points, C.byref(buf.cfg), _p(buf.voxels),
                            _p(buf.coors), _p(buf.num_points), _p(buf.mean), _p(buf.num_voxels), _p(buf.ws), buf.ws.numel(), _st())
    check(rc, "sessd_voxelize")
    return buf


def voxelize_host(points_np, cfg):
    pts = np.ascontiguousarray(points_np, np.float32)
    if pts.ndim != 2 or pts.shape[1] != cfg.num_feat:
        raise ValueError("points must be [N,%d]" % cfg.num_feat)
    voxels = np.zeros((cfg.max_voxels, cfg.max_points, cfg.num_feat), np.float32)
    coors = np.zeros((cfg.max_voxels, 3), np.int32)
    num = np.zeros((cfg.max_voxels,), np.int32)
    m = lib.sessd_voxelize_host(pts.ctypes.data_as(C.c_void_p), pts.shape[0], C.byref(cfg), voxels.ctypes.data_as(C.c_void_p),
                                coors.ctypes.data_as(C.c_void_p), num.ctypes.data_as(C.c_void_p))
    if m < 0:
        raise _lib.SessdError("sessd_voxelize_host failed (%d)" % m)
    return voxels[:m].copy(), coors[:m].copy(), num[:m].copy()


def hash_capacity(max_rows):
    cap = C.c_int(0)
    lib.sessd_hash_bytes(int(max_rows), C.byref(cap))
    return cap.value


def hash_build(coors, n, max_rows, grid, table=None):
    cap = hash_capacity(max_rows)
    if table is None:
        table = torch.empty((cap,), dtype=torch.int64, device=coors.device)
    check(lib.sessd_hash_build(_p(coors), _p(n), int(max_rows), grid, _p(table), cap, _st()), "sessd_hash_build")
    return table


def bitmap_alloc(grid, device):
    words = lib.sessd_bitmap_words(grid)
    bitmap = torch.empty((words, 2), dtype=torch.int32, device=device)
    scratch = torch.empty((lib.sessd_scan_scratch_bytes(words),), dtype=torch.uint8, device=device)
    return bitmap, scratch


def subm_rulebook(coors, n, max_rows, grid, ksize, index_kind, index, nbr=None):
    kvol = int(ksize[0] * ksize[1] * ksize[2])
    if nbr is None:
        nbr = torch.empty((max_rows, kvol), dtype=torch.int32, device=coors.device)
    cap = index.numel() if index_kind == 0 else 0
    check(lib.sessd_subm_rulebook(_p(coors), _p(n), int(max_rows), grid, _i3(ksize), int(index_kind), _p(index), cap, _p(nbr), _st()),
          "sessd_subm_rulebook")
    return nbr


def strided_rulebook(in_coors, n_in, max_in, in_grid, in_index_kind, in_index, ksize, stride, padding, out_grid, bitmap,
                     scratch, out_coors, n_out, max_out, nbr, status):
    cap = in_index.numel() if in_index_kind == 0 else 0
    check(lib.sessd_strided_rulebook(_p(in_coors), _p(n_in), int(max_in), in_grid, int(in_index_kind), _p(in_index), cap, _i3(ksize),
                                     _i3(stride), _i3(padding), out_grid, _p(bitmap), _p(scratch), _p(out_coors), _p(n_out),
                                     int(max_out), _p(nbr), _p(status), _st()), "sessd_strided_rulebook")


def rulebook_pairs(nbr, n, max_rows, kvol):
    dev = nbr.device
    pin = torch.full((kvol, max_rows), -1, dtype=torch.int32, device=dev)
    pout = torch.full((kvol, max_rows), -1, dtype=torch.int32, device=dev)
    num = torch.zeros((kvol,), dtype=torch.int32, device=dev)
    ws = torch.empty((lib.sessd_rulebook_pairs_workspace_bytes(int(max_rows), int(kvol)),), dtype=torch.uint8, device=dev)
    check(lib.sessd_rulebook_pairs(_p(nbr), _p(n), int(max_rows), int(kvol), _p(pin), _p(pout), _p(num), _p(ws), ws.numel(), _st()),
          "sessd_rulebook_pairs")
    return pin, pout, num


def spconv_forward(in_feat, nbr, n_out, max_out, weight, scale, shift, relu, out=None):
    kvol, cin, cout = weight.shape
    if out is None:
        out = torch.empty((max_out, cout), dtype=torch.float32, device=in_feat.device)
    check(lib.sessd_spconv_forward(_p(in_feat), int(cin), _p(nbr), int(kvol), _p(n_out), int(max_out), _p(weight), int(cout),
                                   _p(scale), _p(shift), int(bool(relu)), _p(out), _st()), "sessd_spconv_forward")
    return out


def spconv_forward_rows(in_feat, nbr, n_out, max_out, weight, scale, shift, relu, out, amax_out=None):
    kvol, cin, cout = weight.shape
    check(lib.sessd_spconv_forward_rows(_p(in_feat), int(cin), _p(nbr), int(kvol), _p(n_out), int(max_out), _p(weight), int(cout),
                                        _p(scale), _p(shift), int(bool(relu)), _p(out), _p(amax_out), _st()), "sessd_spconv_forward_rows")
    return out


def _fp16_split(wt):
    amax = wt.abs().amax(dim=(0, 2))
    _, ex = torch.frexp(amax)
    e = torch.where(amax > 0, 11 - ex, torch.zeros_like(ex)).clamp(-100, 100).to(torch.float32)
    ws = wt * torch.exp2(e)[None, :, None]
    hi = ws.to(torch.float16)
    return hi, (ws - hi.to(torch.float32)).to(torch.float16), torch.exp2(-e).contiguous()


def pack_weight_sp_h2(wp, cp):
    kvol, cin, cout = wp.shape
    assert cp in (32, 64) and cin == cp
    hi, lo, inv = _fp16_split(wp.permute(0, 2, 1).contiguous().to(torch.float32))
    return torch.stack([hi, lo], 1).contiguous(), inv


def alloc_planes(max_rows, cp, device):
    return torch.zeros((max_rows + 1, 2 * cp), dtype=torch.float16, device=device)


def absmax_rows(feat, n, max_rows, amax):
    check(lib.sessd_absmax_rows(_p(feat), _p(n), int(max_rows), int(feat.shape[1]), _p(amax), _st()), "sessd_absmax_rows")
    return amax


def spconv_forward_rows_planes(in_feat, nbr, n_out, max_out, weight, scale, shift, relu, amax_in, gain, shift_max, out, out_planes, out_info):
    kvol, cin, cout = weight.shape
    check(lib.sessd_spconv_forward_rows_planes(_p(in_feat), int(cin), _p(nbr), int(kvol), _p(n_out), int(max_out), _p(weight), int(cout),
                                               _p(scale), _p(shift), int(bool(relu)), _p(amax_in), float(gain), float(shift_max), _p(out),
                                               _p(out_planes), int(out_planes.shape[1] // 2), _p(out_info), _st()),
          "sessd_spconv_forward_rows_planes")
    return out_planes


def alloc_tile_lists(max_out, kvol, device):
    return torch.zeros((-(-int(max_out) // 128), int(lib.sessd_tile_list_stride(int(kvol)))), dtype=torch.int32, device=device)


def rulebook_tile_lists(nbr, n_out, max_out, tiles):
    check(lib.sessd_rulebook_tile_lists(_p(nbr), int(nbr.shape[1]), _p(n_out), int(max_out), _p(tiles), _st()), "sessd_rulebook_tile_lists")
    return tiles


def spconv_forward_cg(in_planes, in_info, tiles, n_out, max_out, weight_h2, scale, shift, relu, gain, shift_max, out, out_planes, out_info):
    cp = in_planes.shape[1] // 2
    kvol = weight_h2.shape[0]
    cout = weight_h2.shape[2]
    check(lib.sessd_spconv_forward_cg(_p(in_planes), int(cp), int(in_planes.shape[0]), _p(in_info), _p(tiles), int(kvol), _p(n_out), int(max_out),
                                      _p(weight_h2), int(cout), _p(scale), _p(shift), int(bool(relu)), float(gain), float(shift_max), _p(out),
                                      _p(out_planes), _p(out_info), _st()), "sessd_spconv_forward_cg")
    return out if out is not None else out_planes


def set_sp_cg_deep(on):
    lib.sessd_set_sp_cg_deep(int(on))


def spconv_cg_blocks_per_sm(cp, cout, deep=0):
    n = int(lib.sessd_spconv_cg_blocks_per_sm(int(cp), int(cout), int(deep)))
    check(min(n, 0), "sessd_spconv_cg_blocks_per_sm")
    return n


def rulebook_transpose(nbr, n_out, max_out, max_in, nbr_t=None):
    kvol = int(nbr.shape[1])
    if nbr_t is None:
        nbr_t = torch.empty((int(max_in), kvol), dtype=torch.int32, device=nbr.device)
    check(lib.sessd_rulebook_transpose(_p(nbr), kvol, _p(n_out), int(max_out), int(max_in), _p(nbr_t), _st()), "sessd_rulebook_transpose")
    return nbr_t


def sparse_split_planes(x, n, max_rows, info, planes):
    check(lib.sessd_sparse_split_planes(_p(x), _p(n), int(max_rows), int(x.shape[1]), _p(info), _p(planes), int(planes.shape[1] // 2), _st()),
          "sessd_sparse_split_planes")
    return planes


def dense_grad_gather(grad, coors, n, max_rows, grid, channels, out=None):
    if out is None:
        out = torch.empty((int(max_rows), int(channels)), dtype=torch.float32, device=grad.device)
    check(lib.sessd_dense_grad_gather(_p(grad), _p(coors), _p(n), int(max_rows), int(channels), grid, _p(out), _st()), "sessd_dense_grad_gather")
    return out


def wgrad_items(max_out, kvol):
    return int(lib.sessd_spconv_wgrad_items(int(max_out), int(kvol)))


def wgrad_workspace(max_out, kvol, cin, cout, device):
    return torch.empty((int(lib.sessd_spconv_wgrad_workspace_bytes(int(max_out), int(kvol), int(cin), int(cout))),), dtype=torch.uint8,
                       device=device)


def spconv_wgrad_rows(in_feat, gout, tiles, n_out, max_out, kvol, gw=None, ws=None):
    cin, cout = int(in_feat.shape[1]), int(gout.shape[1])
    if gw is None:
        gw = torch.empty((int(kvol), cin, cout), dtype=torch.float32, device=gout.device)
    if ws is None:
        ws = wgrad_workspace(max_out, kvol, cin, cout, gout.device)
    check(lib.sessd_spconv_wgrad_rows(_p(in_feat), cin, _p(gout), cout, _p(tiles), int(kvol), _p(n_out), int(max_out), _p(gw), _p(ws), ws.numel(),
                                      _st()), "sessd_spconv_wgrad_rows")
    return gw


def spconv_wgrad_cg(in_planes, in_info, g_planes, g_info, tiles, n_out, max_out, kvol, gw=None, ws=None):
    cp, cout = int(in_planes.shape[1] // 2), int(g_planes.shape[1] // 2)
    if gw is None:
        gw = torch.empty((int(kvol), cp, cout), dtype=torch.float32, device=g_planes.device)
    if ws is None:
        ws = wgrad_workspace(max_out, kvol, cp, cout, g_planes.device)
    check(lib.sessd_spconv_wgrad_cg(_p(in_planes), cp, _p(in_info), _p(g_planes), cout, _p(g_info), _p(tiles), int(kvol), _p(n_out), int(max_out),
                                    _p(gw), _p(ws), ws.numel(), _st()), "sessd_spconv_wgrad_cg")
    return gw


def sparse_planes_to_float(planes, info, channels):
    cp = planes.shape[1] // 2
    return (planes[:, :channels].float() + planes[:, cp:cp + channels].float()) / info[1]


def sparse_to_dense(feat, coors, n, max_rows, grid, out=None):
    c = feat.shape[1]
    d, h, w = grid.shape[0], grid.shape[1], grid.shape[2]
    if out is None:
        out = torch.empty((grid.batch, h, w, c * d), dtype=torch.float32, device=feat.device)
    check(lib.sessd_sparse_to_dense(_p(feat), _p(coors), _p(n), int(max_rows), int(c), grid, _p(out), _st()), "sessd_sparse_to_dense")
    return out


def sparse_to_dense_indexed(feat, bitmap_index, grid, out):
    check(lib.sessd_sparse_to_dense_indexed(_p(feat), int(feat.shape[0]), _p(bitmap_index), int(feat.shape[1]), grid, _p(out), _st()),
          "sessd_sparse_to_dense_indexed")
    return out


def conv_desc(batch, in_hw, cin, out_hw, cout, grid_hw, taps, in_stride=1, out_stride=1, out_off=(0, 0), relu=True):
    d = ConvDesc()
    d.batch, d.in_h, d.in_w, d.cin = int(batch), int(in_hw[0]), int(in_hw[1]), int(cin)
    d.out_h, d.out_w, d.cout = int(out_hw[0]), int(out_hw[1]), int(cout)
    d.grid_h, d.grid_w = int(grid_hw[0]), int(grid_hw[1])
    d.in_stride, d.out_stride, d.out_off_y, d.out_off_x = int(in_stride), int(out_stride), int(out_off[0]), int(out_off[1])
    d.ntaps = len(taps)
    for t, (dy, dx) in enumerate(taps):
        d.tap_dy[t], d.tap_dx[t] = int(dy), int(dx)
    d.relu = int(bool(relu))
    return d


def pack_weight_h2(wp, cout_pad):
    taps, cin, cout = wp.shape
    wt = torch.zeros((taps, cout_pad, cin), dtype=torch.float32, device=wp.device)
    wt[:, :cout] = wp.permute(0, 2, 1)
    hi, lo, inv = _fp16_split(wt)
    return torch.stack([hi, lo], 0).contiguous(), inv


def bev_conv_h2(x, weight_h2, scale, shift, residual, out, desc, amax_in=None, amax_out=None):
    check(lib.sessd_bev_conv_h2(_p(x), _p(weight_h2), int(weight_h2.shape[2]), _p(scale), _p(shift), _p(residual), _p(out), C.byref(desc),
                                _p(amax_in), _p(amax_out), _st()), "sessd_bev_conv_h2")
    return out


def bev_deconv_h2(x, weight_h2, scale, shift, residual, out, relu=True, amax_in=None, amax_out=None):
    b, h, w, cin = x.shape
    check(lib.sessd_bev_deconv_h2(_p(x), _p(weight_h2), int(weight_h2.shape[2]), _p(scale), _p(shift), _p(residual), _p(out),
                                  int(b), int(h), int(w), int(cin), int(out.shape[-1]), int(bool(relu)), _p(amax_in), _p(amax_out), _st()),
          "sessd_bev_deconv_h2")
    return out


def alloc_bev_planes(batch, h, w, c, device):
    return torch.zeros((2, batch, h, w, c), dtype=torch.float16, device=device)


def conv_gain(wp, scale):
    g = wp.abs().sum(dim=(0, 1)) * scale.abs().to(wp.device)[: wp.shape[2]]
    return float(g.max()) * (1.0 + 1e-5)


def bev_conv_p2(in_planes, in_info, weight_h2, scale, shift, residual, resid_info, gain, shift_max, out_f32, out_planes, out_info, desc,
                items=None):
    check(lib.sessd_bev_conv_p2(_p(in_planes), _p(in_info), _p(weight_h2), int(weight_h2.shape[2]), _p(scale), _p(shift), _p(residual),
                                _p(resid_info), float(gain), float(shift_max), _p(out_f32), _p(out_planes), _p(out_info), C.byref(desc),
                                _p(items), _st()), "sessd_bev_conv_p2")


def bev_deconv_p2(in_planes, in_info, weight_h2, scale, shift, residual, resid_info, gain, shift_max, out_f32, out_planes, out_info, relu=True,
                  items=None):
    _two, b, h, w, cin = in_planes.shape
    cout = (out_f32 if out_f32 is not None else out_planes).shape[-1]
    check(lib.sessd_bev_deconv_p2(_p(in_planes), _p(in_info), _p(weight_h2), int(weight_h2.shape[2]), _p(scale), _p(shift), _p(residual),
                                  _p(resid_info), float(gain), float(shift_max), _p(out_f32), _p(out_planes), _p(out_info), int(b), int(h),
                                  int(w), int(cin), int(cout), int(bool(relu)), _p(items), _st()), "sessd_bev_deconv_p2")


class BevSkipPlan:

    LAUNCHES = 13

    def __init__(self, batch, h, w, device):
        offs = (C.c_int * self.LAUNCHES)()
        words = lib.sessd_bev_skip_plan_words(int(batch), int(h), int(w), offs)
        if words <= 0:
            raise ValueError("no skip plan for a [%d, %d, %d] neck" % (batch, h, w))
        self.offsets = list(offs)
        self.buf = torch.zeros((int(words),), dtype=torch.int32, device=device)

    def record(self, i):
        return self.buf[self.offsets[i]:]

    def build(self, bitmap_index, grid):
        check(lib.sessd_bev_skip_plan(_p(bitmap_index), grid, _p(self.buf), _st()), "sessd_bev_skip_plan")

    def fill(self, i, out_f32, out_planes, cout):
        check(lib.sessd_bev_skip_fill(_p(self.record(i)), _p(out_f32), _p(out_planes), int(cout), _st()), "sessd_bev_skip_fill")


def bev_split_planes(x, info, planes):
    check(lib.sessd_bev_split_planes(_p(x), int(x.numel()), _p(info), _p(planes), _st()), "sessd_bev_split_planes")
    return planes


def bev_wgrad_workspace(desc, device):
    n = int(lib.sessd_bev_wgrad_workspace_bytes(C.byref(desc)))
    if n == 0:
        raise ValueError("sessd_bev_wgrad: no weight gradient for this descriptor")
    return torch.empty((n,), dtype=torch.uint8, device=device)


def bev_wgrad(in_planes, in_info, g_planes, g_info, desc, gw=None, ws=None):
    if gw is None:
        gw = torch.empty((desc.ntaps, desc.cin, desc.cout), dtype=torch.float32, device=g_planes.device)
    if ws is None:
        ws = bev_wgrad_workspace(desc, g_planes.device)
    check(lib.sessd_bev_wgrad(_p(in_planes), _p(in_info), _p(g_planes), _p(g_info), C.byref(desc), _p(gw), _p(ws), ws.numel(), _st()),
          "sessd_bev_wgrad")
    return gw


def planes_to_float(planes, info):
    return (planes[0].float() + planes[1].float()) / info[1]


def sparse_to_dense_planes(feat, bitmap_index, grid, amax, info, planes):
    check(lib.sessd_sparse_to_dense_planes(_p(feat), int(feat.shape[0]), _p(bitmap_index), int(feat.shape[1]), grid, _p(amax), _p(info),
                                           _p(planes), _st()), "sessd_sparse_to_dense_planes")
    return planes


def ssfa_fuse_planes(x0, x1, w0, w1, s0, t0, s1, t1, out, info0, info1, out_info, planes):
    npix = x0.numel() // x0.shape[-1]
    check(lib.sessd_ssfa_fuse_planes(_p(x0), _p(x1), _p(w0), _p(w1), float(s0), float(t0), float(s1), float(t1), int(npix), int(x0.shape[-1]),
                                     _p(out), _p(info0), _p(info1), _p(out_info), _p(planes), _st()), "sessd_ssfa_fuse_planes")
    return out


def absmax(x, amax):
    check(lib.sessd_absmax(_p(x), int(x.numel()), _p(amax), _st()), "sessd_absmax")
    return amax


NMS_TYPES = ("rotate_nms", "rotate_weighted_nms")
DINMS_MAX_PRE = 4096


def make_dinms_cfg(nms_cnt_thresh=2.6, nms_sigma_dist_interval=(0, 20, 40, 60), nms_sigma_square=(0.0009, 0.009, 0.1, 1),
                   suppressed_thresh=0.3, centerness_pow=2, enable_centerness=True):
    if len(nms_sigma_dist_interval) != 4 or len(nms_sigma_square) < 3:
        raise ValueError("DI-NMS takes four distance edges (three bands) and their three sigma^2")
    d = DinmsCfg()
    d.cnt_thresh, d.suppressed_thresh, d.centerness_pow = float(nms_cnt_thresh), float(suppressed_thresh), float(centerness_pow)
    for j in range(4):
        d.dist_edge[j] = float(nms_sigma_dist_interval[j])
    for j in range(3):
        d.sigma2[j] = float(nms_sigma_square[j])
    d.centerness = int(bool(enable_centerness))
    return d


def make_post_cfg(batch, num_anchors=70400, anchors_per_loc=2, head_stride=24, score_thresh=0.3, nms_pre_max=1000, nms_post_max=100,
                  nms_iou_thresh=0.01, nms_ge=True, post_range=(0, -40.0, -5.0, 70.4, 40.0, 5.0), direction_offset=0.0,
                  use_frustum=False, nms_type="rotate_nms"):
    if nms_type not in NMS_TYPES:
        raise ValueError("nms_type must be one of %s, not %r" % (NMS_TYPES, nms_type))
    c = PostCfg()
    c.batch, c.num_anchors, c.anchors_per_loc, c.head_stride = int(batch), int(num_anchors), int(anchors_per_loc), int(head_stride)
    c.score_thresh, c.nms_pre_max, c.nms_post_max = float(score_thresh), int(nms_pre_max), int(nms_post_max)
    c.nms_iou_thresh, c.nms_ge = float(nms_iou_thresh), int(bool(nms_ge))
    for j in range(6):
        c.post_range[j] = float(post_range[j])
    c.direction_offset, c.use_frustum = float(direction_offset), int(bool(use_frustum))
    if nms_type == "rotate_weighted_nms":
        c.nms_mode, c.dinms = 1, make_dinms_cfg()
    return c


def post_capacity(cfg):
    return cfg.nms_pre_max if cfg.nms_mode == 1 else cfg.nms_post_max


class PostBuffers:
    def __init__(self, cfg, device):
        self.cfg = cfg
        b, p = cfg.batch, post_capacity(cfg)
        self.boxes = torch.zeros((b, p, 7), dtype=torch.float32, device=device)
        self.scores = torch.zeros((b, p), dtype=torch.float32, device=device)
        self.labels = torch.zeros((b, p), dtype=torch.int32, device=device)
        self.count = torch.zeros((b,), dtype=torch.int32, device=device)
        self.aux = torch.zeros((b, 4), dtype=torch.int32, device=device)
        self.sel_anchor = torch.zeros((b, p), dtype=torch.int32, device=device)
        self.ws = torch.empty((lib.sessd_postprocess_workspace_bytes(C.byref(cfg)),), dtype=torch.uint8, device=device)


def postprocess(head, anchors, frustum_planes, buf):
    check(lib.sessd_postprocess(_p(head), _p(anchors), _p(frustum_planes), C.byref(buf.cfg), _p(buf.boxes), _p(buf.scores), _p(buf.labels),
                                _p(buf.count), _p(buf.aux), _p(buf.sel_anchor), _p(buf.ws), buf.ws.numel(), _st()), "sessd_postprocess")
    return buf


def postprocess_packed(head, anchors, frustum_planes, buf, packed, meta, num_voxels=None, status=None):
    check(lib.sessd_postprocess_packed(_p(head), _p(anchors), _p(frustum_planes), C.byref(buf.cfg), _p(buf.boxes), _p(buf.scores),
                                       _p(buf.labels), _p(buf.count), _p(buf.aux), _p(buf.sel_anchor), _p(packed), _p(meta),
                                       _p(num_voxels), _p(status), _p(buf.ws), buf.ws.numel(), _st()), "sessd_postprocess_packed")
    return buf


def rotate_nms(boxes5, scores, n, max_boxes, pre_max, post_max, iou_thresh, ge=True):
    dev = boxes5.device
    keep = torch.empty((post_max,), dtype=torch.int32, device=dev)
    num = torch.zeros((1,), dtype=torch.int32, device=dev)
    ws = torch.empty((lib.sessd_rotate_nms_workspace_bytes(int(max_boxes), int(pre_max)),), dtype=torch.uint8, device=dev)
    check(lib.sessd_rotate_nms(_p(boxes5), _p(scores), _p(n), int(max_boxes), int(pre_max), int(post_max), float(iou_thresh),
                               int(bool(ge)), _p(keep), _p(num), _p(ws), ws.numel(), _st()), "sessd_rotate_nms")
    return keep, num


def rotate_weighted_nms(boxes7, boxes5, scores, iou_preds, labels, dirs, anchors, n, max_boxes, pre_max, dinms_cfg, ws=None):
    dev = scores.device
    for t, dt, name in ((boxes7, torch.float32, "boxes7"), (boxes5, torch.float32, "boxes5"), (scores, torch.float32, "scores"),
                        (iou_preds, torch.float32, "iou_preds"), (labels, torch.int32, "labels"), (dirs, torch.int32, "dirs"),
                        (n, torch.int32, "n")):
        _cuda(t, dt, name)
    if anchors is not None:
        _cuda(anchors, torch.float32, "anchors")
    p = int(pre_max)
    out = dict(boxes=torch.empty((p, 7), dtype=torch.float32, device=dev), scores=torch.empty((p,), dtype=torch.float32, device=dev),
               labels=torch.empty((p,), dtype=torch.int32, device=dev), dirs=torch.empty((p,), dtype=torch.int32, device=dev),
               keep=torch.empty((p,), dtype=torch.int32, device=dev), selected=torch.empty((p,), dtype=torch.int32, device=dev),
               count=torch.zeros((2,), dtype=torch.int32, device=dev))
    if ws is None:
        ws = torch.empty((max(lib.sessd_rotate_weighted_nms_workspace_bytes(int(max_boxes), p), 1),), dtype=torch.uint8, device=dev)
    check(lib.sessd_rotate_weighted_nms(_p(boxes7), _p(boxes5), _p(scores), _p(iou_preds), _p(labels), _p(dirs), _p(anchors), _p(n),
                                        int(max_boxes), p, C.byref(dinms_cfg), _p(out["boxes"]), _p(out["scores"]), _p(out["labels"]),
                                        _p(out["dirs"]), _p(out["keep"]), _p(out["selected"]), _p(out["count"]), _p(ws), ws.numel(),
                                        _st()), "sessd_rotate_weighted_nms")
    return out


def boxes_overlap_bev(a, b, out):
    check(lib.sessd_boxes_overlap_bev(_p(a), a.shape[0], _p(b), b.shape[0], _p(out), _st()), "sessd_boxes_overlap_bev")
    return out


def boxes_aligned_overlap_bev(a, b, out):
    check(lib.sessd_boxes_aligned_overlap_bev(_p(a), _p(b), a.shape[0], _p(out), _st()), "sessd_boxes_aligned_overlap_bev")
    return out


def boxes_iou_bev(a, b, out):
    check(lib.sessd_boxes_iou_bev(_p(a), a.shape[0], _p(b), b.shape[0], _p(out), _st()), "sessd_boxes_iou_bev")
    return out


def boxes_iou3d(a, b, out):
    check(lib.sessd_boxes_iou3d(_p(a), a.shape[0], _p(b), b.shape[0], _p(out), _st()), "sessd_boxes_iou3d")
    return out


def nms_sorted(boxes, thresh, mode):
    n = boxes.shape[0]
    dev = boxes.device
    keep = torch.empty((max(n, 1),), dtype=torch.int64, device=dev)
    num = torch.zeros((1,), dtype=torch.int32, device=dev)
    ws = torch.empty((lib.sessd_nms_workspace_bytes(n),), dtype=torch.uint8, device=dev)
    check(lib.sessd_nms_sorted(_p(boxes), n, float(thresh), int(mode), _p(keep), _p(num), _p(ws), ws.numel(), _st()), "sessd_nms_sorted")
    return keep, num


class AssignBuffers:

    def __init__(self, num_anchors, batch, max_gt, device):
        self.num_anchors, self.batch, self.max_gt = int(num_anchors), int(batch), int(max_gt)
        z = lambda shape, dt: torch.zeros(shape, dtype=dt, device=device)
        self.labels = z((batch, num_anchors), torch.int32)
        self.bbox_targets = z((batch, num_anchors, 7), torch.float32)
        self.bbox_outside_weights = z((batch, num_anchors), torch.float32)
        self.pos_anchor = z((batch, num_anchors), torch.int32)
        self.pos_gt_id = z((batch, num_anchors), torch.int32)
        self.num_pos = z((batch,), torch.int32)
        self.ws = torch.empty((lib.sessd_assign_workspace_bytes(self.num_anchors, self.batch, self.max_gt),), dtype=torch.uint8,
                              device=device)


def assign_targets(anchors, gt_boxes, num_gt, buf, matched_thr=0.6, unmatched_thr=0.45):
    _cuda(anchors, torch.float32, "anchors"); _cuda(gt_boxes, torch.float32, "gt_boxes"); _cuda(num_gt, torch.int32, "num_gt")
    assert anchors.shape == (buf.num_anchors, 7) and tuple(gt_boxes.shape) == (buf.batch, buf.max_gt, 7) and num_gt.numel() == buf.batch
    check(lib.sessd_assign_targets(_p(anchors), buf.num_anchors, _p(gt_boxes), _p(num_gt), buf.batch, buf.max_gt, float(matched_thr),
                                   float(unmatched_thr), _p(buf.labels), _p(buf.bbox_targets), _p(buf.bbox_outside_weights),
                                   _p(buf.pos_anchor), _p(buf.pos_gt_id), _p(buf.num_pos), _p(buf.ws), buf.ws.numel(), _st()),
          "sessd_assign_targets")
    return buf


def head_loss(head, anchors, labels, reg_targets, alpha=0.25, sigma=3.0, dir_offset=0.0, pos_cls_weight=1.0, neg_cls_weight=1.0,
              w_cls=1.0, w_loc=2.0, w_dir=0.2, w_iou=None, with_grad=True):
    _cuda(head, torch.float32, "head"); _cuda(anchors, torch.float32, "anchors"); _cuda(labels, torch.int32, "labels")
    _cuda(reg_targets, torch.float32, "reg_targets")
    B, A = labels.shape
    assert head.shape[0] == B and head.shape[1] * 2 == A and anchors.shape == (A, 7) and tuple(reg_targets.shape) == (B, A, 7)
    losses = torch.empty((B, 8), dtype=torch.float32, device=head.device)
    grad = torch.empty_like(head) if with_grad else None
    ws = torch.empty((lib.sessd_head_loss_workspace_bytes(int(B)),), dtype=torch.uint8, device=head.device)
    check(lib.sessd_head_loss(_p(head), _p(anchors), _p(labels), _p(reg_targets), int(B), int(A), 2, int(head.shape[2]), float(alpha), float(sigma),
                              float(dir_offset), float(pos_cls_weight), float(neg_cls_weight), float(w_cls), float(w_loc), float(w_dir),
                              _p(losses), _p(grad), _p(ws), ws.numel(), _st()), "sessd_head_loss")
    if w_iou is not None:
        ws2 = torch.empty((lib.sessd_iou_pred_loss_workspace_bytes(int(B)),), dtype=torch.uint8, device=head.device)
        check(lib.sessd_iou_pred_loss(_p(head), _p(anchors), _p(labels), _p(reg_targets), int(B), int(A), 2, int(head.shape[2]), float(sigma),
                                      float(w_iou), _p(losses), _p(grad), _p(ws2), ws2.numel(), _st()), "sessd_iou_pred_loss")
    return losses, grad


def odiou_pairs_host(gboxes, qboxes, with_grad=True):
    g = np.ascontiguousarray(gboxes, np.float32).reshape(-1, 7)
    q = np.ascontiguousarray(qboxes, np.float32).reshape(-1, 7)
    assert g.shape == q.shape
    out = np.zeros((g.shape[0],), np.float32)
    grad = np.zeros_like(q) if with_grad else None
    check(lib.sessd_odiou_pairs_host(g.ctypes.data_as(C.c_void_p), q.ctypes.data_as(C.c_void_p), int(g.shape[0]), out.ctypes.data_as(C.c_void_p),
                                     grad.ctypes.data_as(C.c_void_p) if with_grad else C.c_void_p(0)), "sessd_odiou_pairs_host")
    return out, grad


def odiou_loss(head, anchors, labels, reg_targets, losses, grad_head=None, w_odiou=2.0):
    B, A = labels.shape
    out = torch.empty((B,), dtype=torch.float32, device=head.device)
    ws = torch.empty((lib.sessd_odiou_loss_workspace_bytes(int(B)),), dtype=torch.uint8, device=head.device)
    check(lib.sessd_odiou_loss(_p(head), _p(anchors), _p(labels), _p(reg_targets), int(B), int(A), 2, int(head.shape[2]), float(w_odiou),
                               _p(losses), _p(out), _p(grad_head), _p(ws), ws.numel(), _st()), "sessd_odiou_loss")
    return out


def box_collision(boxes, qboxes, out=None):
    _cuda(boxes, torch.float64, "boxes"); _cuda(qboxes, torch.float64, "qboxes")
    n, k = boxes.shape[0], qboxes.shape[0]
    if out is None:
        out = torch.empty((n, k), dtype=torch.uint8, device=boxes.device)
    check(lib.sessd_box_collision(_p(boxes), int(n), _p(qboxes), int(k), _p(out), _st()), "sessd_box_collision")
    return out


def _aug_inputs(gt_boxes, num_gt, valid, loc_noise, rot_noise, selected=None):
    _cuda(gt_boxes, torch.float32, "gt_boxes"); _cuda(num_gt, torch.int32, "num_gt"); _cuda(valid, torch.uint8, "valid")
    _cuda(loc_noise, torch.float64, "loc_noise"); _cuda(rot_noise, torch.float64, "rot_noise")
    B, M = valid.shape
    T = rot_noise.shape[2]
    if (tuple(gt_boxes.shape) != (B, M, 7) or num_gt.numel() != B or tuple(loc_noise.shape) != (B, M, T, 3)
            or tuple(rot_noise.shape) != (B, M, T)):
        raise ValueError("augmentation inputs: shape mismatch")
    if selected is not None:
        _cuda(selected, torch.int32, "selected")
        if tuple(selected.shape) != (B, M):
            raise ValueError("selected must be [B, M]")
    return B, M, T


def points_in_boxes(points, boxes, context=-1.0, mask=None):
    _cuda(points, torch.float32, "points"); _cuda(boxes, torch.float32, "boxes")
    if points.dim() != 2 or points.shape[1] < 3 or boxes.dim() != 2 or boxes.shape[1] != 7:
        raise ValueError("points_in_boxes: points [N, >=3], boxes [M, 7]")
    n, m = points.shape[0], boxes.shape[0]
    if mask is None:
        mask = torch.empty((n, m), dtype=torch.uint8, device=points.device)
    check(lib.sessd_points_in_boxes(_p(points), int(n), int(points.shape[1]), _p(boxes), int(m), float(context), _p(mask), _st()),
          "sessd_points_in_boxes")
    return mask


def noise_per_box(gt_boxes, num_gt, valid, loc_noise, rot_noise, context=-1.0, selected=None):
    B, M, T = _aug_inputs(gt_boxes, num_gt, valid, loc_noise, rot_noise)
    if selected is None:
        selected = torch.empty((B, M), dtype=torch.int32, device=gt_boxes.device)
    _cuda(selected, torch.int32, "selected")
    check(lib.sessd_noise_per_box(_p(gt_boxes), _p(num_gt), _p(valid), int(B), int(M), _p(loc_noise), _p(rot_noise), int(T),
                                  float(context), _p(selected), _st()), "sessd_noise_per_box")
    return selected


def augment_points(points, frame_off, max_frame_points, gt_boxes, num_gt, valid, loc_noise, rot_noise, selected, glob, perm, labeled=None,
                   context=-1.0, points_raw=None, points_out=None, with_raw=True):
    B, M, T = _aug_inputs(gt_boxes, num_gt, valid, loc_noise, rot_noise, selected)
    _cuda(points, torch.float32, "points"); _cuda(frame_off, torch.int32, "frame_off"); _cuda(glob, torch.float32, "glob")
    _cuda(perm, torch.int32, "perm")
    if labeled is not None:
        _cuda(labeled, torch.uint8, "labeled")
        if labeled.numel() != B:
            raise ValueError("labeled must be [B]")
    if points.dim() != 2 or points.shape[1] != 4 or frame_off.numel() != B + 1 or perm.numel() != points.shape[0] or tuple(glob.shape) != (B, 5):
        raise ValueError("augment_points: shape mismatch")
    if not with_raw:
        points_raw = None
    elif points_raw is None:
        points_raw = torch.empty_like(points)
    if points_out is None:
        points_out = torch.empty_like(points)
    written = (("points_raw", points_raw), ("points_out", points_out)) if with_raw else (("points_out", points_out),)
    for name, t in written:
        _cuda(t, torch.float32, name)
        if t.shape != points.shape:
            raise ValueError("%s must be shaped like points" % name)
    if any(t.data_ptr() % 16 for t in (points, points_out) + ((points_raw,) if with_raw else ())):
        raise ValueError("augment_points: point rows are read and written as float4 and must be 16-byte aligned")
    check(lib.sessd_augment_points(_p(points), _p(frame_off), int(B), int(max_frame_points), _p(gt_boxes), _p(num_gt), _p(valid), int(M),
                                   _p(loc_noise), _p(rot_noise), int(T), _p(selected), float(context), _p(glob), _p(perm), _p(labeled),
                                   _p(points_raw), _p(points_out), _st()), "sessd_augment_points")
    return points_raw, points_out


def augment_boxes(gt_boxes, num_gt, valid, target, loc_noise, rot_noise, selected, glob, range_bev, global_boxes=False):
    B, M, T = _aug_inputs(gt_boxes, num_gt, valid, loc_noise, rot_noise, selected)
    _cuda(glob, torch.float32, "glob")
    if tuple(glob.shape) != (B, 5):
        raise ValueError("glob must be [B, 5]")
    if target is not None:
        _cuda(target, torch.uint8, "target")
        if tuple(target.shape) != (B, M):
            raise ValueError("target must be [B, M]")
    dev = gt_boxes.device
    boxes_raw = torch.empty((B, M, 7), dtype=torch.float32, device=dev)
    boxes_out = torch.empty((B, M, 7), dtype=torch.float32, device=dev)
    num_raw = torch.empty((B,), dtype=torch.int32, device=dev)
    num_out = torch.empty((B,), dtype=torch.int32, device=dev)
    boxes_glob = torch.empty((B, M, 7), dtype=torch.float32, device=dev) if global_boxes else None
    num_glob = torch.empty((B,), dtype=torch.int32, device=dev) if global_boxes else None
    rg = (C.c_float * 4)(*[float(v) for v in range_bev])
    check(lib.sessd_augment_boxes(_p(gt_boxes), _p(num_gt), _p(valid), _p(target), int(B), int(M), _p(loc_noise), _p(rot_noise), int(T),
                                  _p(selected), _p(glob), rg, _p(boxes_raw), _p(num_raw), _p(boxes_out), _p(num_out), _p(boxes_glob),
                                  _p(num_glob), _st()), "sessd_augment_boxes")
    res = (boxes_raw, num_raw, boxes_out, num_out)
    return res + (boxes_glob, num_glob) if global_boxes else res


def gtaug_select_host(corners, num_boxes):
    corners = np.ascontiguousarray(corners, np.float64)
    if corners.ndim != 3 or corners.shape[1:] != (4, 2) or not 0 <= num_boxes <= corners.shape[0]:
        raise ValueError("gtaug_select_host: corners [num_boxes + K, 4, 2], 0 <= num_boxes <= rows")
    k = corners.shape[0] - int(num_boxes)
    acc = np.zeros(max(k, 1), np.uint8)
    rc = lib.sessd_gtaug_select_host(corners.ctypes.data_as(C.c_void_p), int(num_boxes), int(k), acc.ctypes.data_as(C.c_void_p))
    if rc < 0:
        check(rc, "sessd_gtaug_select_host")
    return acc[:k].astype(bool)


def gtaug_paste(points, frame_off, obj_off, obj_ids, db_points, db_off, db_count, db_boxes, max_paste_points, out=None,
                frame_off_out=None):
    _cuda(points, torch.float32, "points"); _cuda(frame_off, torch.int32, "frame_off"); _cuda(db_points, torch.float32, "db_points")
    _cuda(db_off, torch.int32, "db_off"); _cuda(db_count, torch.int32, "db_count"); _cuda(db_boxes, torch.float64, "db_boxes")
    B = frame_off.numel() - 1
    N = db_count.numel()
    if isinstance(obj_ids, np.ndarray) or isinstance(obj_off, np.ndarray):
        ids = np.asarray(obj_ids).reshape(-1); off = np.asarray(obj_off).reshape(-1)
        if ids.size and (ids.min() < 0 or ids.max() >= N):
            raise ValueError("gtaug_paste: object id out of range [0, %d)" % N)
        if off.size != B + 1 or off[0] != 0 or off[-1] != ids.size or (np.diff(off) < 0).any():
            raise ValueError("gtaug_paste: obj_off must be a CSR offset array [B+1] over the ids")
        host = np.concatenate([off.astype(np.int32), ids.astype(np.int32)])
        dev_ids = torch.from_numpy(host).to(points.device)
        obj_off, obj_ids = dev_ids[:B + 1], dev_ids[B + 1:]
    _cuda(obj_off, torch.int32, "obj_off"); _cuda(obj_ids, torch.int32, "obj_ids")
    if (B < 1 or points.dim() != 2 or points.shape[1] != 4 or obj_off.numel() != B + 1 or db_points.dim() != 2 or db_points.shape[1] != 4
            or db_off.numel() != N or tuple(db_boxes.shape) != (N, 7)):
        raise ValueError("gtaug_paste: shape mismatch")
    cap = int(points.shape[0]) + int(max_paste_points)
    dev = points.device
    if out is None:
        out = torch.empty((max(cap, 1), 4), dtype=torch.float32, device=dev)
    if frame_off_out is None:
        frame_off_out = torch.empty((B + 1,), dtype=torch.int32, device=dev)
    _cuda(out, torch.float32, "out"); _cuda(frame_off_out, torch.int32, "frame_off_out")
    if out.dim() != 2 or out.shape[1] != 4 or frame_off_out.numel() != B + 1:
        raise ValueError("gtaug_paste: out [capacity, 4], frame_off_out [B+1]")
    if any(t.data_ptr() % 16 for t in (points, db_points, out)):
        raise ValueError("gtaug_paste: point rows are read and written as float4 and must be 16-byte aligned")
    K = obj_ids.numel()
    ws = torch.empty((int(lib.sessd_gtaug_paste_workspace_bytes(B, int(points.shape[0]), K)),), dtype=torch.uint8, device=dev)
    check(lib.sessd_gtaug_paste(_p(points), _p(frame_off), int(B), int(points.shape[0]), _p(obj_off), _p(obj_ids), int(K),
                                int(max_paste_points), _p(db_points), _p(db_off), _p(db_count), _p(db_boxes), int(N), _p(ws),
                                ws.numel(), _p(out), int(out.shape[0]), _p(frame_off_out), _st()), "sessd_gtaug_paste")
    return out, frame_off_out


SADA_MAX_IDS = 6 * 256


def _rows4(points, name):
    _cuda(points, torch.float32, name)
    if points.dim() != 2 or points.shape[1] != 4:
        raise ValueError("%s must be [N, 4]" % name)
    if points.data_ptr() % 16:
        raise ValueError("%s: point rows are read and written as float4 and must be 16-byte aligned" % name)
    return points


def _count(d_n, name="n"):
    if d_n is not None:
        _cuda(d_n, torch.int32, name)
        if d_n.numel() < 1:
            raise ValueError("%s must hold one count" % name)
    return d_n


def _ids(ids, num_pyramids, device):
    if not isinstance(ids, torch.Tensor):
        ids = np.asarray(ids, np.int64).reshape(-1)
        if ids.size and (ids.min() < 0 or ids.max() >= num_pyramids):
            raise ValueError("pyramid id out of range [0, %d)" % num_pyramids)
        if ids.size > SADA_MAX_IDS:
            raise ValueError("at most %d listed pyramids" % SADA_MAX_IDS)
        ids = torch.from_numpy(ids.astype(np.int32)).to(device)
    return _cuda(ids, torch.int32, "ids")


def sada_pyramids(boxes):
    _cuda(boxes, torch.float32, "boxes")
    if boxes.dim() != 2 or boxes.shape[1] != 7:
        raise ValueError("sada_pyramids: boxes [K, 7]")
    K = boxes.shape[0]
    pyr = torch.empty((6 * K, 15), dtype=torch.float32, device=boxes.device)
    planes = torch.empty((6 * K, 5, 4), dtype=torch.float32, device=boxes.device)
    if K == 0:
        return pyr, planes
    check(lib.sessd_sada_pyramids(_p(boxes), int(K), _p(pyr), _p(planes), _st()), "sessd_sada_pyramids")
    return pyr, planes


def sada_membership(points, planes, ids, n=None, with_bits=True):
    _rows4(points, "points"); _cuda(planes, torch.float32, "planes"); _count(n)
    if planes.dim() != 3 or tuple(planes.shape[1:]) != (5, 4):
        raise ValueError("planes must be [P, 5, 4]")
    dev = points.device
    ids = _ids(ids, planes.shape[0], dev)
    A, N = ids.numel(), points.shape[0]
    bits = torch.empty((N, max(-(-A // 32), 1)), dtype=torch.int32, device=dev) if with_bits else None
    counts = torch.zeros((max(A, 1),), dtype=torch.int32, device=dev)
    check(lib.sessd_sada_membership(_p(points), int(N), _p(n), _p(planes), int(planes.shape[0]), _p(ids), int(A), _p(bits), _p(counts),
                                    _st()), "sessd_sada_membership")
    return bits, counts[:A], ids


def sada_compact(points, bits, counts, min_count=-1, n=None, out=None):
    _rows4(points, "points"); _cuda(bits, torch.int32, "bits"); _cuda(counts, torch.int32, "counts"); _count(n)
    N, A = points.shape[0], counts.numel()
    if bits.shape[0] != N or bits.shape[1] * 32 < A:
        raise ValueError("sada_compact: bits [N, ceil(A / 32)]")
    dev = points.device
    out = _rows4(torch.empty((max(N, 1), 4), dtype=torch.float32, device=dev) if out is None else out, "out")
    num = torch.empty((1,), dtype=torch.int32, device=dev)
    ws = torch.empty((max(int(lib.sessd_sada_compact_workspace_bytes(int(N))), 16),), dtype=torch.uint8, device=dev)
    check(lib.sessd_sada_compact(_p(points), int(N), _p(n), _p(bits), int(A), _p(counts), int(min_count), _p(ws), ws.numel(), _p(out),
                                 int(out.shape[0]), _p(num), _st()), "sessd_sada_compact")
    return out, num


def sada_fps(points, bits, counts, min_count, k, out, num, n=None):
    _rows4(points, "points"); _cuda(bits, torch.int32, "bits"); _cuda(counts, torch.int32, "counts"); _rows4(out, "out")
    _count(num, "num"); _count(n)
    N, A = points.shape[0], counts.numel()
    if bits.shape[0] != N or bits.shape[1] * 32 < A:
        raise ValueError("sada_fps: bits [N, ceil(A / 32)]")
    ws = torch.empty((max(int(lib.sessd_sada_fps_workspace_bytes(int(N), int(A))), 16),), dtype=torch.uint8, device=points.device)
    check(lib.sessd_sada_fps(_p(points), int(N), _p(n), _p(bits), int(A), _p(counts), int(min_count), int(k), _p(ws), ws.numel(), _p(out),
                             int(out.shape[0]), _p(num), _st()), "sessd_sada_fps")
    return out, num


def sada_swap(points, bits, counts, pyramids, ids, max_swap_points, out, num_in, n=None):
    _rows4(points, "points"); _cuda(bits, torch.int32, "bits"); _cuda(counts, torch.int32, "counts"); _rows4(out, "out")
    _cuda(pyramids, torch.float32, "pyramids"); _cuda(ids, torch.int32, "ids"); _count(num_in, "num_in"); _count(n)
    N, A = points.shape[0], ids.numel()
    if A % 2 or counts.numel() != A or bits.shape[0] != N or bits.shape[1] * 32 < A or pyramids.dim() != 2 or pyramids.shape[1] != 15:
        raise ValueError("sada_swap: shape mismatch")
    num_out = torch.empty((1,), dtype=torch.int32, device=points.device)
    check(lib.sessd_sada_swap(_p(points), int(N), _p(n), _p(bits), int(A // 2), _p(counts), _p(pyramids), int(pyramids.shape[0]), _p(ids),
                              int(max_swap_points), _p(out), int(out.shape[0]), _p(num_in), _p(num_out), _st()), "sessd_sada_swap")
    return out, num_out


def sada_shuffle(points, frame_off, max_frame_points, perm, out=None):
    _rows4(points, "points"); _cuda(frame_off, torch.int32, "frame_off"); _cuda(perm, torch.int32, "perm")
    if perm.numel() != points.shape[0]:
        raise ValueError("sada_shuffle: perm [P]")
    out = _rows4(torch.empty_like(points) if out is None else out, "out")
    if out.shape != points.shape:
        raise ValueError("sada_shuffle: out must be shaped like points")
    check(lib.sessd_sada_shuffle(_p(points), _p(frame_off), int(frame_off.numel() - 1), int(max_frame_points), _p(perm), _p(out), _st()),
          "sessd_sada_shuffle")
    return out


def _rows16(name, *ts):
    if any(t is not None and t.data_ptr() % 16 for t in ts):
        raise ValueError("%s: point rows are read and written as float4 and must be 16-byte aligned" % name)


def prep_frustum_compact(points, frame_off, planes, out=None, frame_off_out=None):
    _cuda(points, torch.float32, "points"); _cuda(frame_off, torch.int32, "frame_off"); _cuda(planes, torch.float64, "planes")
    B = frame_off.numel() - 1
    P = int(points.shape[0])
    if B < 1 or points.dim() != 2 or points.shape[1] != 4 or tuple(planes.shape) != (B, 6, 4):
        raise ValueError("prep_frustum_compact: points [P, 4], frame_off [B+1], planes [B, 6, 4]")
    dev = points.device
    if out is None:
        out = torch.empty((max(P, 1), 4), dtype=torch.float32, device=dev)
    if frame_off_out is None:
        frame_off_out = torch.empty((B + 1,), dtype=torch.int32, device=dev)
    _cuda(out, torch.float32, "out"); _cuda(frame_off_out, torch.int32, "frame_off_out")
    _rows16("prep_frustum_compact", points, out)
    ws = torch.empty((max(int(lib.sessd_prep_frustum_compact_workspace_bytes(P)), 16),), dtype=torch.uint8, device=dev)
    check(lib.sessd_prep_frustum_compact(_p(points), _p(frame_off), int(B), P, _p(planes), _p(ws), ws.numel(), _p(out), int(out.shape[0]),
                                         _p(frame_off_out), _st()), "sessd_prep_frustum_compact")
    return out, frame_off_out


def prep_box_count(points, frame_off, box_planes, box_off, counts=None):
    _cuda(points, torch.float32, "points"); _cuda(frame_off, torch.int32, "frame_off"); _cuda(box_planes, torch.float64, "box_planes")
    _cuda(box_off, torch.int32, "box_off")
    B = frame_off.numel() - 1
    K = int(box_planes.shape[0])
    if B < 1 or points.dim() != 2 or points.shape[1] != 4 or tuple(box_planes.shape[1:]) != (6, 4) or box_off.numel() != B + 1:
        raise ValueError("prep_box_count: points [P, 4], frame_off [B+1], box_planes [K, 6, 4], box_off [B+1]")
    if counts is None:
        counts = torch.empty((max(K, 1),), dtype=torch.int32, device=points.device)
    _cuda(counts, torch.int32, "counts")
    _rows16("prep_box_count", points)
    check(lib.sessd_prep_box_count(_p(points), _p(frame_off), int(B), int(points.shape[0]), _p(box_planes), _p(box_off), K, _p(counts),
                                   _st()), "sessd_prep_box_count")
    return counts[:K]


def prep_box_gather(points, frame_off, box_planes, centres, box_off, counts, num_rows, out=None, obj_off=None):
    _cuda(points, torch.float32, "points"); _cuda(frame_off, torch.int32, "frame_off"); _cuda(box_planes, torch.float64, "box_planes")
    _cuda(centres, torch.float64, "centres"); _cuda(box_off, torch.int32, "box_off"); _cuda(counts, torch.int32, "counts")
    B = frame_off.numel() - 1
    K = int(box_planes.shape[0])
    if (B < 1 or points.dim() != 2 or points.shape[1] != 4 or tuple(box_planes.shape[1:]) != (6, 4) or tuple(centres.shape) != (K, 3)
            or box_off.numel() != B + 1 or counts.numel() < K):
        raise ValueError("prep_box_gather: shape mismatch")
    dev = points.device
    if out is None:
        out = torch.empty((max(int(num_rows), 1), 4), dtype=torch.float32, device=dev)
    if obj_off is None:
        obj_off = torch.empty((K + 1,), dtype=torch.int32, device=dev)
    _cuda(out, torch.float32, "out"); _cuda(obj_off, torch.int32, "obj_off")
    _rows16("prep_box_gather", points, out)
    ws = torch.empty((max(int(lib.sessd_prep_box_gather_workspace_bytes(K)), 16),), dtype=torch.uint8, device=dev)
    check(lib.sessd_prep_box_gather(_p(points), _p(frame_off), int(B), int(points.shape[0]), _p(box_planes), _p(centres), _p(box_off), K,
                                    _p(counts), int(num_rows), _p(ws), ws.numel(), _p(out), int(out.shape[0]), _p(obj_off), _st()),
          "sessd_prep_box_gather")
    return out[:int(num_rows)], obj_off
```

se-ssd_b200/sessd_b200/runners.py:

```python
import itertools
import math

import torch
from sessd_data.layers import SPMIDDLE_LAYERS
from sessd_data.layers import SSFA_LAUNCHES, ssfa_extents

from . import ops

BN_EPS = 1e-3

def conv_out_shape(shape, ksize, stride, padding):
    return tuple((int(i) + 2 * p - k) // s + 1 for i, k, s, p in zip(shape, ksize, stride, padding))


def fold_bn(gamma, beta, mean, var, eps=BN_EPS):
    scale = gamma.float() / torch.sqrt(var.float() + eps)
    shift = beta.float() - mean.float() * scale
    return scale.contiguous(), shift.contiguous()


def sparse_impl(cin, use_tc=True):
    if not use_tc:
        return "simt"
    return "rows" if cin <= 16 else "cg"


def plane_width(channels):
    return 32 if channels <= 32 else 64


def spmiddle_plan(use_tc=True, keep_f32=False, cin0=4):
    plan, cin, lvl = [], cin0, 0
    for kind, cout, ks, st, pd, key in SPMIDDLE_LAYERS:
        lout = lvl if kind == "subm" else lvl + 1
        rb = key if kind == "subm" else "sp%d" % lout
        impl = sparse_impl(cin, use_tc)
        plan.append(dict(kind=kind, key=key, ks=ks, st=st, pd=pd, cin=cin, cout=cout, lin=lvl, lout=lout, rb=rb,
                         build_rb=all(p["rb"] != rb for p in plan), impl=impl, cp_in=plane_width(cin) if impl == "cg" else None))
        cin, lvl = cout, lout
    nxt = {}
    for p in reversed(plan):
        p["tile_lists"] = p["build_rb"] and any(q["impl"] == "cg" for q in plan if q["rb"] == p["rb"])
        p["cp_out"] = nxt.get("cp_in")
        p["out_f32"] = keep_f32 or p["cp_out"] is None
        p["out_info"] = p["impl"] == "cg" or p["cp_out"] is not None or (nxt.get("impl") == "rows" and nxt["cp_out"] is not None)
        nxt = p
    return plan


class SpMiddleRunner:

    GROWTH = (1.0, 4.0, 6.0, 5.0, 3.0)

    def __init__(self, batch, max_voxels_total, input_shape_xyz=(1408, 1600, 40), num_input_features=4, device="cuda",
                 growth=None, use_tc=True, keep_f32=False):
        self.batch, self.device = batch, torch.device(device)
        self.use_tc, self.keep_f32 = bool(use_tc), bool(keep_f32)
        shape = (int(input_shape_xyz[2]) + 1, int(input_shape_xyz[1]), int(input_shape_xyz[0]))
        growth = growth or self.GROWTH
        self.levels = []
        self._add_level(shape, int(max_voxels_total), hash_index=True)
        self.plan = spmiddle_plan(self.use_tc, self.keep_f32, num_input_features)
        rulebooks = {}
        for p in self.plan:
            if p["kind"] != "subm":
                oshape = conv_out_shape(self.levels[p["lin"]]["shape"], p["ks"], p["st"], p["pd"])
                cells = batch * oshape[0] * oshape[1] * oshape[2]
                self._add_level(oshape, min(cells, int(math.ceil(max_voxels_total * growth[p["lout"]]))), hash_index=False)
            if p["build_rb"]:
                cap, kvol = self.levels[p["lout"]]["cap"], p["ks"][0] * p["ks"][1] * p["ks"][2]
                rulebooks[p["rb"]] = (torch.empty((cap, kvol), dtype=torch.int32, device=self.device),
                                      ops.alloc_tile_lists(cap, kvol, self.device) if p["tile_lists"] else None)
            p["nbr"], p["tiles"] = rulebooks[p["rb"]]
        caps = [self.levels[p["lout"]]["cap"] for p in self.plan]
        self.feats = [torch.zeros((cap, p["cout"]), dtype=torch.float32, device=self.device) if p["out_f32"] else None
                      for p, cap in zip(self.plan, caps)]
        self.planes = [ops.alloc_planes(cap, p["cp_out"], self.device) if p["cp_out"] else None for p, cap in zip(self.plan, caps)]
        assert all(pl is None or pl.shape[0] <= (1 << 25) for pl in self.planes)
        last = self.levels[-1]
        self.out_channels = self.plan[-1]["cout"] * last["shape"][0]
        self.dense = torch.zeros((batch, last["shape"][1], last["shape"][2], self.out_channels), dtype=torch.float32,
                                 device=self.device)
        self.status = torch.zeros((1,), dtype=torch.int32, device=self.device)
        self.weights = None
        self.info = torch.zeros((len(self.plan), 2), dtype=torch.float32, device=self.device)

    def layer_output(self, li):
        p = self.plan[li]
        if p["out_f32"]:
            return self.feats[li]
        return ops.sparse_planes_to_float(self.planes[li][:-1], self.info[li], p["cout"])

    def _add_level(self, shape, cap, hash_index):
        grid = ops.make_grid(self.batch, shape)
        lv = dict(shape=shape, cap=cap, grid=grid, n=torch.zeros((1,), dtype=torch.int32, device=self.device))
        if hash_index:
            lv["index_kind"] = 0
            lv["index"] = torch.empty((ops.hash_capacity(cap),), dtype=torch.int64, device=self.device)
            lv["coors"] = None
        else:
            lv["index_kind"] = 1
            lv["index"], lv["scratch"] = ops.bitmap_alloc(grid, self.device)
            lv["coors"] = torch.zeros((cap, 4), dtype=torch.int32, device=self.device)
        self.levels.append(lv)

    def load_weights(self, layers):
        assert len(layers) == len(self.plan)
        self.weights = []
        for p, l in zip(self.plan, layers):
            w = torch.as_tensor(l["weight"], dtype=torch.float32, device=self.device)
            assert tuple(w.shape) == (*p["ks"], p["cin"], p["cout"]), (w.shape, p)
            sc, sh = fold_bn(*[torch.as_tensor(l[k], device=self.device) for k in ("gamma", "beta", "mean", "var")], eps=float(l.get("eps", BN_EPS)))
            wp = w.reshape(-1, p["cin"], p["cout"]).contiguous()
            p["gain"], p["shift_max"] = ops.conv_gain(wp, sc), float(sh.abs().max())
            if p["impl"] == "cg":
                tiles, inv = ops.pack_weight_sp_h2(wp, p["cp_in"])
                self.weights.append((tiles, (sc * inv).contiguous(), sh))
            else:
                self.weights.append((wp, sc, sh))

    def forward(self, feat0, coors0, n0, mark=None, dense_planes=None):
        mark = mark or (lambda label: None)
        assert self.weights is not None, "load_weights first"
        L0 = self.levels[0]
        cap0 = min(coors0.shape[0], L0["cap"])
        L0["coors"], L0["n_ext"] = coors0, n0
        ops.hash_build(coors0, n0, cap0, L0["grid"], L0["index"])
        mark("hash_build")
        if self.use_tc:
            self.info.zero_()
        x = feat0
        for li, p in enumerate(self.plan):
            lin, lout = self.levels[p["lin"]], self.levels[p["lout"]]
            n_in = lin["n_ext"] if p["lin"] == 0 else lin["n"]
            cap_in = cap0 if p["lin"] == 0 else lin["cap"]
            n_out, cap_out = (n_in, cap_in) if p["kind"] == "subm" else (lout["n"], lout["cap"])
            if p["build_rb"]:
                if p["kind"] == "subm":
                    ops.subm_rulebook(lin["coors"], n_in, cap_in, lin["grid"], p["ks"], lin["index_kind"], lin["index"], p["nbr"])
                else:
                    ops.strided_rulebook(lin["coors"], n_in, cap_in, lin["grid"], lin["index_kind"], lin["index"], p["ks"], p["st"],
                                         p["pd"], lout["grid"], lout["index"], lout["scratch"], lout["coors"], lout["n"], lout["cap"],
                                         p["nbr"], self.status)
                if p["tiles"] is not None:
                    ops.rulebook_tile_lists(p["nbr"], n_out, cap_out, p["tiles"])
                mark("rulebook:" + p["rb"])
            w, sc, sh = self.weights[li]
            out = self.feats[li]
            if p["impl"] == "rows" and p["cp_out"]:
                ops.spconv_forward_rows_planes(x, p["nbr"], n_out, cap_out, w, sc, sh, True, self.info[li - 1, 0:1], p["gain"], p["shift_max"],
                                               out, self.planes[li], self.info[li])
            elif p["impl"] == "rows":
                ops.spconv_forward_rows(x, p["nbr"], n_out, cap_out, w, sc, sh, True, out, self.info[li, 0:1] if p["out_info"] else None)
            elif p["impl"] == "cg":
                ops.spconv_forward_cg(self.planes[li - 1], self.info[li - 1], p["tiles"], n_out, cap_out, w, sc, sh, True, p["gain"],
                                      p["shift_max"], out, self.planes[li], self.info[li])
            else:
                ops.spconv_forward(x, p["nbr"], n_out, cap_out, w, sc, sh, True, out)
            mark("conv:%d" % li)
            x = out
        last = self.levels[-1]
        if dense_planes is not None:
            assert self.plan[-1]["out_info"], "the planes' scale needs the last layer's abs-max (use_tc)"
            out = ops.sparse_to_dense_planes(x, last["index"], last["grid"], self.info[-1, 0:1], dense_planes[1], dense_planes[0])
        else:
            out = ops.sparse_to_dense_indexed(x, last["index"], last["grid"], self.dense)
        mark("dense")
        return out


class RunnerCache:

    def __init__(self):
        self.runner = self.key = self.weights = None

    def get(self, module, key, build, load):
        if self.runner is None or key != self.key:
            self.runner, self.key, self.weights = build(), key, None
        weights = tuple((t.data_ptr(), t._version) for t in itertools.chain(module.parameters(), module.buffers()))
        if weights != self.weights:
            load(self.runner)
            self.weights = weights
        return self.runner


_SSFA = {L.name: L for L in SSFA_LAUNCHES}


def conv_taps(k):
    return [(dy - k // 2, dx - k // 2) for dy in range(k) for dx in range(k)]


def _pack_conv(w):
    cout, cin, kh, kw = w.shape
    packed = w.permute(2, 3, 1, 0).reshape(kh * kw, cin, cout).contiguous()
    return packed, [(ky, kx) for ky in range(kh) for kx in range(kw)]


def launch_weight(L, w):
    if L.kind == "deconv":
        return w.permute(2, 3, 0, 1).reshape(9, L.cin, L.cout).contiguous(), None
    return _pack_conv(w)[0], conv_taps(L.k)


def launch_desc(L, batch, in_hw, out_hw, taps, relu=None):
    return ops.conv_desc(batch, in_hw, L.cin, out_hw, L.cout, out_hw, taps, in_stride=L.stride, relu=L.relu if relu is None else relu)


def head_weight(param):
    w, b = (torch.cat([param(c + s) for c in ("conv_box", "conv_cls", "conv_dir", "conv_iou")], 0) for s in (".weight", ".bias"))
    pad = _SSFA["head"].cout - w.shape[0]
    return torch.cat([w, w.new_zeros((pad,) + tuple(w.shape[1:]))], 0), torch.cat([b, b.new_zeros((pad,))], 0)


def pack_head(head_sd, prefix, device):
    return head_weight(lambda name: head_sd[prefix + name].to(device, torch.float32))


def fold_ssfa_bn(sd, conv_name, device, eps=BN_EPS):
    blk, idx = conv_name.rsplit(".", 1)
    b = "%s.%d." % (blk, int(idx) + 1)
    return fold_bn(*(sd[b + k].to(device, torch.float32) for k in ("weight", "bias", "running_mean", "running_var")), eps=eps)


def pack_h2(wp, taps, scale, shift):
    planes, inv = ops.pack_weight_h2(wp, _cout_pad(wp.shape[2]))
    scale = torch.ones(wp.shape[2], device=wp.device) if scale is None else scale
    return dict(w=planes, scale=(scale * inv[:scale.numel()]).contiguous(), shift=shift.contiguous(), gain=ops.conv_gain(wp, scale),
                shift_max=float(shift.abs().max()), taps=taps)


def _cout_pad(cout):
    n_tile = 32 if cout <= 32 else 128
    return -(-cout // n_tile) * n_tile


def ssfa_weights(ssfa_sd, head_sd, head_prefix, device, bn_eps=BN_EPS):
    for L in SSFA_LAUNCHES:
        if L.name != "head":
            wp, taps = launch_weight(L, ssfa_sd[L.name + ".weight"].to(device, torch.float32))
            yield (L, wp, taps) + fold_ssfa_bn(ssfa_sd, L.name, device, bn_eps)
        elif head_sd is not None:
            w, bias = pack_head(head_sd, head_prefix, device)
            yield (L, *launch_weight(L, w), None, bias)


def ssfa_fuse_weights(ssfa_sd, device, bn_eps=BN_EPS):
    out = {}
    for name in ("w_0.0", "w_1.0"):
        sc, sh = fold_ssfa_bn(ssfa_sd, name, device, bn_eps)
        out[name] = (ssfa_sd[name + ".weight"].to(device, torch.float32).reshape(-1).contiguous(), float(sc[0]), float(sh[0]))
    return out


SSFA_SLOT = {n: i for i, n in enumerate(["x"] + [L.dst for L in SSFA_LAUNCHES if not L.f32] + ["out"] + [L.dst for L in SSFA_LAUNCHES if L.f32])}


class SSFAPlanesRunner:

    HEAD_STRIDE = 24
    SLOT = SSFA_SLOT
    SKIP_LAUNCHES = tuple(L.name for L in SSFA_LAUNCHES)

    def __init__(self, batch, hw=(200, 176), device="cuda", skip_constant=False):
        self.batch, self.h, self.w, self.device = batch, int(hw[0]), int(hw[1]), torch.device(device)
        pl = lambda hw_, c: ops.alloc_bev_planes(batch, hw_[0], hw_[1], c, self.device)
        z = lambda hw_, c: torch.zeros((batch,) + hw_ + (c,), dtype=torch.float32, device=self.device)
        H, ext = (self.h, self.w), lambda L: ssfa_extents(L, self.h, self.w)[1]
        self.planes = dict(x=pl(H, 128), **{L.dst: pl(ext(L), L.cout) for L in SSFA_LAUNCHES if not L.f32}, out=pl(H, 128))
        self.buf = dict(**{L.dst: z(ext(L), L.cout) for L in SSFA_LAUNCHES[:-1] if L.f32}, out=z(H, 128), head=z(H, self.HEAD_STRIDE))
        self.info = torch.zeros((16, 2), dtype=torch.float32, device=self.device)
        self.params = None
        self.skip_constant = bool(skip_constant)
        self.skip = ops.BevSkipPlan(batch, self.h, self.w, self.device) if self.skip_constant else None

    def _info(self, name):
        return self.info[self.SLOT[name]]

    def load_state(self, ssfa_sd, head_sd=None, head_prefix="tasks.0.", bn_eps=BN_EPS):
        P = ssfa_fuse_weights(ssfa_sd, self.device, bn_eps)
        for L, *weight in ssfa_weights(ssfa_sd, head_sd, head_prefix, self.device, bn_eps):
            P[L.name] = pack_h2(*weight)
        self.params = P

    def _split(self, x, name):
        self.info.zero_()
        ops.absmax(x, self._info(name)[0:1])
        ops.bev_split_planes(x, self._info(name), self.planes[name])

    def _launch(self, L, skip=False):
        q = self.params[L.name]
        out_f32, out_planes = (self.buf[L.dst], None) if L.f32 else (None, self.planes[L.dst])
        resid, resid_info = (self.buf[L.residual], self._info(L.residual)) if L.residual else (None, None)
        i = self.SKIP_LAUNCHES.index(L.name)
        rec = self.skip.record(i) if skip else None
        if L.kind == "conv":
            d = launch_desc(L, self.batch, *ssfa_extents(L, self.h, self.w), q["taps"])
            ops.bev_conv_p2(self.planes[L.src], self._info(L.src), q["w"], q["scale"], q["shift"], resid, resid_info, q["gain"],
                            q["shift_max"], out_f32, out_planes, self._info(L.dst), d, items=rec)
        else:
            ops.bev_deconv_p2(self.planes[L.src], self._info(L.src), q["w"], q["scale"], q["shift"], resid, resid_info, q["gain"],
                              q["shift_max"], out_f32, out_planes, self._info(L.dst), L.relu, items=rec)
        if skip:
            self.skip.fill(i, out_f32, out_planes, L.cout)

    def forward(self, x=None, mark=None, occupancy=None):
        assert self.params is not None, "load_state first"
        mark = mark or (lambda label: None)
        if x is not None:
            self._split(x, "x")
        skip = self.skip_constant and occupancy is not None
        if skip:
            index, grid = occupancy
            assert (grid.batch, grid.shape[1], grid.shape[2]) == (self.batch, self.h, self.w), "occupancy of another map"
            self.skip.build(index, grid)
            mark("neck:skip_plan")
        for L in SSFA_LAUNCHES[:-1]:
            self._launch(L, skip)
            mark("neck:" + L.name)
        w0, s0, t0 = self.params["w_0.0"]
        w1, s1, t1 = self.params["w_1.0"]
        ops.ssfa_fuse_planes(self.buf["o0"], self.buf["o1"], w0, w1, s0, t0, s1, t1, self.buf["out"], self._info("o0"), self._info("o1"),
                             self._info("out"), self.planes["out"])
        if "head" not in self.params:
            mark("neck:fuse+head")
            return self.buf["out"], None
        self.head(skip=skip)
        mark("neck:fuse+head")
        return self.buf["out"], self.buf["head"]

    def head(self, skip=False):
        self._launch(SSFA_LAUNCHES[-1], skip)
        return self.buf["head"]

    def activation(self, name):
        if name in self.buf:
            return self.buf[name]
        return ops.planes_to_float(self.planes[name], self._info(name))

    def bench_layer(self, name="bottom_up_block_0.4"):

        def launch():
            self._launch(_SSFA[name]._replace(src="x0", dst="b0b"))

        return launch, "bev_conv_p2_kernel (fp16 wgmma from pre-split fp16 planes, two-term split)"


class HeadRunner(SSFAPlanesRunner):

    def __init__(self, batch, hw, device="cuda"):
        self.batch, self.h, self.w, self.device = batch, int(hw[0]), int(hw[1]), torch.device(device)
        self.planes = dict(out=ops.alloc_bev_planes(batch, self.h, self.w, 128, self.device))
        self.buf = dict(head=torch.zeros((batch, self.h, self.w, self.HEAD_STRIDE), dtype=torch.float32, device=self.device))
        self.info = torch.zeros((len(self.SLOT), 2), dtype=torch.float32, device=self.device)
        self.params = None

    def load_state(self, head_sd, prefix=""):
        w, bias = pack_head(head_sd, prefix, self.device)
        self.params = {"head": pack_h2(*launch_weight(_SSFA["head"], w), None, bias)}

    def forward(self, x):
        self._split(x, "out")
        return self.head()
```

Measured before the change: 1547.

## Pack partially occupied tiles into strip groups for BEV conv skipping

Extends the occupancy-based skip plan with a second granularity. Occupied 8x2 strips from partly empty 8x16 tiles are packed into groups of eight, and a new kernel builds these lists. In the stride-1 register-A path, the producer loads only those strips through a second tensor map, and each consumer warp maps its rows to one strip. The skip fill kernel is taught to fill the empty strips. This aims to cut MMA and load work on sparse BEV maps, at the cost of an extra list-building launch, more per-strip TMA descriptors and more complex indexing.

```diff
diff --git a/include/sessd_b200.h b/include/sessd_b200.h
--- a/include/sessd_b200.h
+++ b/include/sessd_b200.h
@@ -112,14 +112,15 @@
 int sessd_bev_conv_p2(const void *d_in_planes, const float *d_in_info, const void *d_weight_h2, int cout_pad, const float *d_scale,
                       const float *d_shift, const float *d_residual, const float *d_resid_info, float gain, float shift_max,
                       float *d_out_f32, void *d_out_planes, float *d_out_info, const sessd_conv_desc *desc, const int *d_items,
-                      void *stream);
+                      const int *d_strips, void *stream);
 int sessd_bev_deconv_p2(const void *d_in_planes, const float *d_in_info, const void *d_weight_h2, int cout_pad, const float *d_scale,
                         const float *d_shift, const float *d_residual, const float *d_resid_info, float gain, float shift_max,
                         float *d_out_f32, void *d_out_planes, float *d_out_info, int batch, int in_h, int in_w, int cin, int cout,
-                        int relu, const int *d_items, void *stream);
+                        int relu, const int *d_items, const int *d_strips, void *stream);
 long long sessd_bev_skip_plan_words(int batch, int h, int w, int *offsets);
-int sessd_bev_skip_plan(const void *d_bitmap_index, sessd_grid grid, int *d_plan, void *stream);
-int sessd_bev_skip_fill(const int *d_record, float *d_out_f32, void *d_out_planes, int cout, void *stream);
+long long sessd_bev_skip_strip_words(int batch, int h, int w, int *offsets);
+int sessd_bev_skip_plan(const void *d_bitmap_index, sessd_grid grid, int *d_plan, int *d_strips, void *stream);
+int sessd_bev_skip_fill(const int *d_record, const int *d_strips, float *d_out_f32, void *d_out_planes, int cout, void *stream);
 int sessd_bev_wgrad_items(const sessd_conv_desc *desc);
 size_t sessd_bev_wgrad_workspace_bytes(const sessd_conv_desc *desc);
 int sessd_bev_wgrad(const void *d_in_planes, const float *d_in_info, const void *d_g_planes, const float *d_g_info,
diff --git a/se-ssd_b200/csrc/bevconv_p2.cu b/se-ssd_b200/csrc/bevconv_p2.cu
--- a/se-ssd_b200/csrc/bevconv_p2.cu
+++ b/se-ssd_b200/csrc/bevconv_p2.cu
@@ -27,17 +27,17 @@
 extern "C" int sessd_bev_conv_p2(const void *d_in_planes, const float *d_in_info, const void *d_weight_h2, int cout_pad, const float *d_scale,
                                  const float *d_shift, const float *d_residual, const float *d_resid_info, float gain, float shift_max,
                                  float *d_out_f32, void *d_out_planes, float *d_out_info, const sessd_conv_desc *desc, const int *d_items,
-                                 void *stream) {
+                                 const int *d_strips, void *stream) {
     return p2_conv<kP2Planes>(d_in_planes, d_in_info, d_weight_h2, cout_pad, d_scale, d_shift, d_residual, d_resid_info, gain, shift_max,
-                              d_out_f32, d_out_planes, d_out_info, desc, stream, d_items);
+                              d_out_f32, d_out_planes, d_out_info, desc, stream, d_items, nullptr, false, d_strips);
 }
 
 extern "C" int sessd_bev_deconv_p2(const void *d_in_planes, const float *d_in_info, const void *d_weight_h2, int cout_pad, const float *d_scale,
                                    const float *d_shift, const float *d_residual, const float *d_resid_info, float gain, float shift_max,
                                    float *d_out_f32, void *d_out_planes, float *d_out_info, int batch, int in_h, int in_w, int cin, int cout,
-                                   int relu, const int *d_items, void *stream) {
+                                   int relu, const int *d_items, const int *d_strips, void *stream) {
     return p2_deconv<kP2Planes>(d_in_planes, d_in_info, d_weight_h2, cout_pad, d_scale, d_shift, d_residual, d_resid_info, gain, shift_max,
-                                d_out_f32, d_out_planes, d_out_info, batch, in_h, in_w, cin, cout, relu, stream, d_items);
+                                d_out_f32, d_out_planes, d_out_info, batch, in_h, in_w, cin, cout, relu, stream, d_items, nullptr, d_strips);
 }
 
 extern "C" int sessd_bev_split_planes(const float *d_x, long long n, float *d_info, void *d_planes, void *stream) {
diff --git a/se-ssd_b200/csrc/bevconv_p2.cuh b/se-ssd_b200/csrc/bevconv_p2.cuh
--- a/se-ssd_b200/csrc/bevconv_p2.cuh
+++ b/se-ssd_b200/csrc/bevconv_p2.cuh
@@ -16,6 +16,8 @@
 constexpr int kP2MaxSmem = 227 * 1024;
 constexpr int kP2Chunk = 32;
 constexpr int kP2ItemsHeader = 32;
+constexpr int kP2StripHeader = 16;
+constexpr int kP2StripV = 2;
 enum { kP2Planes = 0, kP2SplitF16 = 1 };
 enum { kP2NoProbe = 0, kP2ProbeClocks = 1, kP2ProbeLoads = 2 };
 
@@ -45,6 +47,8 @@
     float *out_info;
     long long out_plane_stride;
     const int *items;
+    const int *strips;
+    int sub_rows_v, sub_bytes, strip_load_bytes;
     long long *prof;
 };
 
@@ -64,8 +68,24 @@
     kP2ProfWords = 16
 };
 
-__device__ __forceinline__ int p2_item_count(const P2Params &p) { return p.items ? __ldg(p.items) : p.total; }
-__device__ __forceinline__ int p2_item(const P2Params &p, int k) { return p.items ? __ldg(p.items + kP2ItemsHeader + k) : k; }
+__device__ __forceinline__ int p2_item_count(const P2Params &p) {
+    if (p.strips) return __ldg(p.strips) + __ldg(p.strips + 1);
+    return p.items ? __ldg(p.items) : p.total;
+}
+__device__ __forceinline__ int p2_item(const P2Params &p, int k, const int *&grp) {
+    grp = nullptr;
+    if (p.strips) {
+        const int nfull = __ldg(p.strips);
+        if (k < nfull) return __ldg(p.strips + kP2StripHeader + k);
+        grp = p.strips + kP2StripHeader + p.total + 8 * (k - nfull);
+        return __ldg(grp) >> 3;
+    }
+    return p.items ? __ldg(p.items + kP2ItemsHeader + k) : k;
+}
+__device__ __forceinline__ int p2_item(const P2Params &p, int k) {
+    const int *grp;
+    return p2_item(p, k, grp);
+}
 
 struct P2ItemIndex { int rank, nb, t; };
 __host__ __device__ __forceinline__ P2ItemIndex p2_item_index(int g, int nblocks, int tiles) {
@@ -138,6 +158,7 @@
 template <int NT, int MODE, bool REGA = false, int PROBE = kP2NoProbe>
 __global__ void __launch_bounds__(REGA ? kP2ThreadsRegA : kP2Threads, 1) bev_conv_p2_kernel(const __grid_constant__ CUtensorMap map_a,
                                                                    const __grid_constant__ CUtensorMap map_b,
+                                                                   const __grid_constant__ CUtensorMap map_s,
                                                                    const float *__restrict__ scale, const float *__restrict__ shift,
                                                                    const float *__restrict__ resid, float *__restrict__ out_f32,
                                                                    __half *__restrict__ out_planes, P2Params p) {
@@ -155,6 +176,7 @@
     const int warp = threadIdx.x >> 5, lane = threadIdx.x & 31;
     if (threadIdx.x == kP2PatchWarp * 32) prefetch_tensormap(&map_a);
     if (threadIdx.x == kP2WeightWarp * 32) prefetch_tensormap(&map_b);
+    if (REGA && p.strips && threadIdx.x == kP2PatchWarp * 32) prefetch_tensormap(&map_s);
     const int nchunks = p.cin / kP2Chunk;
     const int nitems = p2_item_count(p);
     const uint32_t b_plane_bytes = (uint32_t)p.n_tile * 64u;
@@ -184,11 +206,28 @@
             uint32_t pph = 0;
             const uint32_t patches_u32 = smem_u32(patches);
             for (int k = blockIdx.x; k < nitems; k += gridDim.x) {
-                const P2Item it = p2_decode(p, p2_item(p, k));
-                const int bu = it.u0 * p.in_stride, bv = it.v0 * p.in_stride;
+                const int *grp;
+                const int g = p2_item(p, k, grp);
                 for (int cc = 0; cc < nchunks; ++cc) {
                     { const long long t0 = p2_tick<PROFILE>(); mbar_wait<REGA>(&patch_empty[pb], pph ^ 1u); p2_tock<PROFILE>(clk[kProfPatchEmpty], t0); }
-                    if (elect_one()) {
+                    if (REGA && grp) {
+                        if (elect_one()) {
+                            int nstrips = 0;
+                            for (int i = 0; i < 8; ++i) nstrips += __ldg(grp + i) >= 0;
+                            mbar_expect_tx(&patch_full[pb], (uint32_t)(nstrips * p.strip_load_bytes));
+                            const uint32_t dst = patches_u32 + (uint32_t)(pb * p.patch_bytes);
+                            for (int i = 0; i < nstrips; ++i) {
+                                const int sw = __ldg(grp + i);
+                                const P2Item st = p2_decode(p, sw >> 3);
+                                const int cu = st.u0 + p.copy_u[0], cv = st.v0 + kP2StripV * (sw & 7) + p.copy_v[0];
+                                const uint32_t d = dst + (uint32_t)(i * p.sub_bytes);
+                                tma_load_5d(d, &map_s, &patch_full[pb], cc * kP2Chunk, cu, cv, st.b, 0);
+                                tma_load_5d(d + (uint32_t)p.copy_bytes, &map_s, &patch_full[pb], cc * kP2Chunk, cu, cv, st.b, 1);
+                            }
+                        }
+                    } else if (elect_one()) {
+                        const P2Item it = p2_decode(p, g);
+                        const int bu = it.u0 * p.in_stride, bv = it.v0 * p.in_stride;
                         mbar_expect_tx(&patch_full[pb], (uint32_t)p.load_bytes);
                         if constexpr (MODE == kP2Planes) {
                             uint32_t dst = patches_u32 + (uint32_t)(pb * p.patch_bytes);
@@ -240,14 +279,14 @@
         }
     } else {
         if constexpr (REGA) setmaxnreg_inc<kP2RegsConsumer>();
-        const int wg = warp >> 2, wq = warp & 3;
+        const int wg = warp >> 2;
         constexpr int kAcc = NT / 2;
         const uint32_t a_rows = (uint32_t)(wg * 64 * 64) >> 4;
         const uint32_t tiles_lo = desc_lo(smem_u32(tiles));
         const uint32_t patch_lo = desc_lo(smem_u32(patches)) + a_rows;
         const uint32_t plane_lo = b_plane_bytes >> 4;
         const uint32_t copy_lo = (uint32_t)(p.copy_bytes >> 4), patch_sz = (uint32_t)(p.patch_bytes >> 4);
-        const uint32_t a_row = (uint32_t)((wg * 8 + wq * 2 + ((lane >> 3) & 1)) * p.pitch_u + (lane & 7)), a_chunk = (uint32_t)(lane >> 4);
+        const uint32_t a_row_lane = (uint32_t)(((lane >> 3) & 1) * p.pitch_u + (lane & 7)), a_chunk = (uint32_t)(lane >> 4);
         const uint32_t patches_u32 = smem_u32(patches);
         float amax_in = 0.f, s_in = 1.f;
         if constexpr (MODE == kP2Planes) { amax_in = __ldg(p.in_info); s_in = __ldg(p.in_info + 1); }
@@ -263,8 +302,10 @@
         uint32_t bph = 0, pph = 0;
         for (int k = blockIdx.x; k < nitems; k += gridDim.x) {
             const long long t_item = p2_tick<PROFILE>();
-            const int g = p2_item(p, k);
+            const int *grp;
+            const int g = p2_item(p, k, grp);
             const int cls = p.cls_order[g / per_cls];
+            const uint32_t a_row = a_row_lane + (uint32_t)(grp ? warp * (p.sub_bytes >> 6) : kP2StripV * warp * p.pitch_u);
             const int ntaps = p.cls_ntaps[cls];
             const uint32_t *aoff = s_aoff + cls * 9;
             float acc[NT];
@@ -384,17 +425,18 @@
             }
 #pragma unroll
             for (int i = 0; i < kAcc; ++i) acc[i] = acc[kAcc + i] + acc[i];
-            const P2Item it = p2_decode(p, g);
+            p2_item(p, k, grp);
+            const int wstrip = grp ? __ldg(grp + warp) : -1;
+            const P2Item it = p2_decode(p, wstrip >= 0 ? wstrip >> 3 : g);
             const int q = lane & 3;
-            const int r0 = wg * 64 + wq * 16 + (lane >> 2);
+            const int v_warp = it.v0 + kP2StripV * (wstrip >= 0 ? (wstrip & 7) : warp);
+            const bool warp_ok = !grp || wstrip >= 0;
             bool rows_ok[2];
             size_t opixs[2];
 #pragma unroll
             for (int h = 0; h < 2; ++h) {
-                const int r = r0 + 8 * h;
-                const int lv = r / kP2TileU, lu = r % kP2TileU;
-                const int gu = it.u0 + lu, gv = it.v0 + lv;
-                rows_ok[h] = it.b < p.batch && gu < p.grid_u && gv < p.grid_v;
+                const int gu = it.u0 + (lane >> 2), gv = v_warp + h;
+                rows_ok[h] = warp_ok && it.b < p.batch && gu < p.grid_u && gv < p.grid_v;
                 const int ou = gu * p.out_stride + p.cls_off_u[it.cls], ov = gv * p.out_stride + p.cls_off_v[it.cls];
                 const int oy = p.u_is_x ? ov : ou, ox = p.u_is_x ? ou : ov;
                 opixs[h] = ((size_t)it.b * p.out_h + (size_t)oy) * p.out_w + (size_t)ox;
@@ -535,8 +577,10 @@
     return 0;
 }
 
-static int p2_plan(P2Params &p, const P2Taps *cls, int nclass, int grid_h, int grid_w, int cout_pad, int mode, bool reg_a, int *smem) {
+static int p2_plan(P2Params &p, const P2Taps *cls, int nclass, int grid_h, int grid_w, int cout_pad, int mode, bool reg_a, int *smem,
+                   bool strips = false) {
     if (reg_a && (mode != kP2Planes || p.in_stride != 1)) return SESSD_EINVAL;
+    if (strips && !reg_a) return SESSD_EINVAL;
     if (p.cin < 64 || p.cin % 64) return SESSD_EINVAL;
     P2Geometry g;
     if (p2_geometry(g, p.batch, grid_h, grid_w, p.cout, cout_pad, cls, nclass)) return SESSD_EINVAL;
@@ -593,6 +637,13 @@
     }
     p.copy_bytes = (p.rows_v * p.pitch_u * 64 + 511) & ~511;
     p.patch_bytes = p.ncopies * 2 * p.copy_bytes;
+    if (strips) {
+        p.sub_rows_v = p.rows_v - kP2TileV + kP2StripV;
+        p.sub_bytes = (p.sub_rows_v * p.pitch_u * 64 + 511) & ~511;
+        p.strip_load_bytes = 2 * p.sub_rows_v * p.pitch_u * 64;
+        p.copy_bytes = max(p.copy_bytes, 8 * p.sub_bytes);
+        p.patch_bytes = 2 * p.copy_bytes;
+    }
     p.staging_bytes = mode == kP2Planes ? 0 : p.ncopies * p.rows_v * kP2TileU * kP2Chunk * 4;
     p.load_bytes = mode == kP2Planes ? p.ncopies * 2 * p.rows_v * p.pitch_u * 64 : p.staging_bytes;
     const int per_buf = p.patch_bytes + p.staging_bytes, bstage = 2 * p.n_tile * 64;
@@ -617,10 +668,10 @@
     if (((uintptr_t)d_scale | (uintptr_t)d_shift | (uintptr_t)d_residual | (uintptr_t)d_out_f32 | (uintptr_t)d_out_planes) & 15)
         return SESSD_EINVAL;
     int smem = 0;
-    if (p2_plan(p, cls, nclass, grid_h, grid_w, cout_pad, MODE, reg_a, &smem)) return SESSD_EINVAL;
-    if (p.items && cout_pad != div_up(p.cout, p.n_tile) * p.n_tile) return SESSD_EINVAL;
+    if (p2_plan(p, cls, nclass, grid_h, grid_w, cout_pad, MODE, reg_a, &smem, p.strips != nullptr)) return SESSD_EINVAL;
+    if ((p.items || p.strips) && cout_pad != div_up(p.cout, p.n_tile) * p.n_tile) return SESSD_EINVAL;
     const int s = p.in_stride;
-    CUtensorMap map_a, map_b;
+    CUtensorMap map_a, map_b, map_s;
     if (MODE != kP2Planes) {
         const cuuint64_t row_w = (cuuint64_t)p.cin * 4, row_h = (cuuint64_t)in_w * p.cin * 4;
         const cuuint64_t dims[5] = {(cuuint64_t)p.cin, (cuuint64_t)(p.u_is_x ? in_w : in_h), (cuuint64_t)(p.u_is_x ? in_h : in_w),
@@ -631,6 +682,7 @@
         const cuuint32_t estr[5] = {1, (cuuint32_t)s, (cuuint32_t)s, 1, 1};
         int rc = encode_map_nd(&map_a, d_in_planes, 5, dims, strides, box, estr, CU_TENSOR_MAP_SWIZZLE_NONE, CU_TENSOR_MAP_DATA_TYPE_FLOAT32);
         if (rc) return rc;
+        map_s = map_a;
     } else {
         const cuuint64_t row_w = (cuuint64_t)p.cin * 2, row_h = (cuuint64_t)in_w * p.cin * 2;
         const cuuint64_t dims[5] = {(cuuint64_t)p.cin, (cuuint64_t)(p.u_is_x ? in_w : in_h), (cuuint64_t)(p.u_is_x ? in_h : in_w),
@@ -641,6 +693,12 @@
         const cuuint32_t estr[5] = {1, (cuuint32_t)s, (cuuint32_t)s, 1, 1};
         int rc = encode_map_nd(&map_a, d_in_planes, 5, dims, strides, box, estr, CU_TENSOR_MAP_SWIZZLE_64B);
         if (rc) return rc;
+        map_s = map_a;
+        if (p.strips) {
+            const cuuint32_t sbox[5] = {(cuuint32_t)kP2Chunk, (cuuint32_t)p.pitch_u, (cuuint32_t)p.sub_rows_v, 1, 1};
+            rc = encode_map_nd(&map_s, d_in_planes, 5, dims, strides, sbox, estr, CU_TENSOR_MAP_SWIZZLE_64B);
+            if (rc) return rc;
+        }
     }
     {
         const cuuint64_t dims[4] = {(cuuint64_t)p.cin, (cuuint64_t)cout_pad, (cuuint64_t)w_taps, 2};
@@ -674,7 +732,7 @@
         SESSD_CUDA_TRY(cudaDeviceGetAttribute(&num_sms, cudaDevAttrMultiProcessorCount, dev));
     }
     const int grid = p.total < num_sms ? p.total : num_sms;
-    SESSD_LAUNCH(kernel, grid, reg_a ? kP2ThreadsRegA : kP2Threads, smem, (cudaStream_t)stream, map_a, map_b, d_scale, d_shift, d_residual, d_out_f32,
+    SESSD_LAUNCH(kernel, grid, reg_a ? kP2ThreadsRegA : kP2Threads, smem, (cudaStream_t)stream, map_a, map_b, map_s, d_scale, d_shift, d_residual, d_out_f32,
                  (__half *)d_out_planes, p);
     return last_error();
 }
@@ -703,13 +761,14 @@
 static int p2_conv(const void *d_in_planes, const float *d_in_info, const void *d_weight_h2, int cout_pad, const float *d_scale,
                    const float *d_shift, const float *d_residual, const float *d_resid_info, float gain, float shift_max,
                    float *d_out_f32, void *d_out_planes, float *d_out_info, const sessd_conv_desc *desc, void *stream,
-                   const int *d_items = nullptr, long long *d_prof = nullptr, bool smem_a = false) {
+                   const int *d_items = nullptr, long long *d_prof = nullptr, bool smem_a = false, const int *d_strips = nullptr) {
     if (!desc || (PROBE != kP2NoProbe && !d_prof)) return SESSD_EINVAL;
     const sessd_conv_desc &d = *desc;
     P2Params p;
     P2Taps t;
     if (p2_conv_params(d, p, t)) return SESSD_EINVAL;
     p.items = d_items;
+    p.strips = d_strips;
     p.prof = d_prof;
     return launch_p2<MODE, PROBE>(d_in_planes, d.in_h, d.in_w, d_in_info, d_weight_h2, d.ntaps, cout_pad, d_scale, d_shift, d_residual, d_resid_info, gain,
                      shift_max, d_out_f32, d_out_planes, d_out_info, p, &t, 1, d.grid_h, d.grid_w, MODE == kP2Planes && d.in_stride == 1 && !smem_a,
@@ -720,12 +779,13 @@
 static int p2_deconv(const void *d_in_planes, const float *d_in_info, const void *d_weight_h2, int cout_pad, const float *d_scale,
                      const float *d_shift, const float *d_residual, const float *d_resid_info, float gain, float shift_max,
                      float *d_out_f32, void *d_out_planes, float *d_out_info, int batch, int in_h, int in_w, int cin, int cout,
-                     int relu, void *stream, const int *d_items = nullptr, long long *d_prof = nullptr) {
+                     int relu, void *stream, const int *d_items = nullptr, long long *d_prof = nullptr, const int *d_strips = nullptr) {
     if (PROBE != kP2NoProbe && !d_prof) return SESSD_EINVAL;
     P2Params p;
     P2Taps cls[4];
     p2_deconv_params(batch, in_h, in_w, cin, cout, relu, p, cls);
     p.items = d_items;
+    p.strips = d_strips;
     p.prof = d_prof;
     return launch_p2<MODE, PROBE>(d_in_planes, in_h, in_w, d_in_info, d_weight_h2, 9, cout_pad, d_scale, d_shift, d_residual, d_resid_info, gain, shift_max,
                      d_out_f32, d_out_planes, d_out_info, p, cls, 4, in_h, in_w, MODE == kP2Planes, stream);
diff --git a/se-ssd_b200/csrc/bevskip.cu b/se-ssd_b200/csrc/bevskip.cu
--- a/se-ssd_b200/csrc/bevskip.cu
+++ b/se-ssd_b200/csrc/bevskip.cu
@@ -16,11 +16,17 @@
     int map;
     int out_stride, out_h, out_w;
     int rec;
+    int srec;
+    bool strips;
 };
+
+enum { kSrecFull = 0, kSrecGroups = 1, kSrecDead = 2, kSrecDeadOff = 3, kSrecMaskOff = 4, kSrecListOff = 5 };
+static_assert(kP2StripHeader >= 6, "strip record header");
 
 struct SkipPlan {
     int batch, depth, h, w, h2, w2, nwf, nwh;
     SkipLaunch l[kSkipLaunches];
+    long long strip_words;
 };
 
 static int skip_launch(SkipLaunch &L, int map, int batch, int grid_h, int grid_w, int out_h, int out_w, int cout, bool deconv) {
@@ -57,6 +63,13 @@
         L[i].rec = (int)words;
         words += kP2ItemsHeader + L[i].total + 2LL * L[i].nclass * L[i].tiles;
     }
+    long long swords = 0;
+    for (int i = 0; i < kSkipLaunches; ++i) {
+        L[i].strips = i != 3;
+        L[i].srec = (int)swords;
+        swords += kP2StripHeader + 9LL * L[i].total + 17LL * L[i].nclass * L[i].tiles;
+    }
+    P.strip_words = swords;
     return rc ? 0 : words;
 }
 
@@ -129,9 +142,9 @@
     return base;
 }
 
-__global__ void __launch_bounds__(kSkipThreads) bev_skip_plan_kernel(const uint2 *__restrict__ bitmap, int *__restrict__ plan, SkipPlan P) {
+__global__ void __launch_bounds__(kSkipThreads) bev_skip_plan_kernel(const uint2 *__restrict__ bitmap, int *__restrict__ plan,
+                                                                     int *__restrict__ strips, SkipPlan P) {
     extern __shared__ uint32_t s_bits[];
-    __shared__ int s_scan[33], s_rep[4];
     BitMap m[kNumMaps];
     {
         uint32_t *p = s_bits;
@@ -184,30 +197,43 @@
             const SkipLaunch &L = P.l[li];
             const BitMap &o = m[L.map];
             int *flags = plan + L.rec + kP2ItemsHeader + L.total + L.nclass * L.tiles;
+            int *masks = strips && L.strips ? strips + L.srec + kP2StripHeader + 9 * L.total + 8 * L.nclass * L.tiles : nullptr;
             const int per_frame = L.tiles_u * L.tiles_v;
             for (int idx = threadIdx.x; idx < L.nclass * per_frame; idx += blockDim.x) {
                 const int c = idx / per_frame, tf = idx - c * per_frame;
                 const int tu = tf % L.tiles_u, tv = tf / L.tiles_u;
                 const int u0 = tu * kP2TileU, v0 = tv * kP2TileV;
-                bool run = u0 + kP2TileU > L.grid_u || v0 + kP2TileV > L.grid_v;
-                if (!run && L.out_stride == 1) {
+                uint32_t live = u0 + kP2TileU > L.grid_u || v0 + kP2TileV > L.grid_v ? 0xFFu : 0u;
+                if (!live && L.out_stride == 1) {
                     const int y0 = L.u_is_x ? v0 : u0, x0 = L.u_is_x ? u0 : v0;
                     const int ny = L.u_is_x ? kP2TileV : kP2TileU, nx = L.u_is_x ? kP2TileU : kP2TileV;
                     const uint32_t field = (1u << nx) - 1u;
-                    for (int y = y0; y < y0 + ny && !run; ++y) run = (o.w[y * o.nw + (x0 >> 5)] >> (x0 & 31)) & field;
-                } else if (!run) {
-                    for (int r = 0; r < kP2TileU * kP2TileV && !run; ++r) {
+                    for (int y = y0; y < y0 + ny; ++y) {
+                        const uint32_t bits = (o.w[y * o.nw + (x0 >> 5)] >> (x0 & 31)) & field;
+                        if (L.u_is_x) {
+                            if (bits) live |= 1u << ((y - y0) >> 1);
+                        } else {
+                            for (int st = 0; st < 8; ++st) if ((bits >> (2 * st)) & 3u) live |= 1u << st;
+                        }
+                    }
+                } else if (!live) {
+                    for (int r = 0; r < kP2TileU * kP2TileV; ++r) {
                         const int ou = (u0 + (r & 7)) * L.out_stride + L.off_u[c], ov = (v0 + (r >> 3)) * L.out_stride + L.off_v[c];
-                        run = L.u_is_x ? o.get(ov, ou) : o.get(ou, ov);
+                        if (L.u_is_x ? o.get(ov, ou) : o.get(ou, ov)) live |= 1u << (r >> 4);
                     }
                 }
-                flags[c * L.tiles + b * per_frame + tf] = run ? 1 : 0;
-            }
-        }
-        __syncthreads();
-    }
-    for (int li = 0; li < kSkipLaunches; ++li) {
-        const SkipLaunch &L = P.l[li];
+                flags[c * L.tiles + b * per_frame + tf] = live ? 1 : 0;
+                if (masks) masks[c * L.tiles + b * per_frame + tf] = (int)live;
+            }
+        }
+        __syncthreads();
+    }
+}
+
+__global__ void __launch_bounds__(kSkipThreads) bev_skip_lists_kernel(int *__restrict__ plan, int *__restrict__ strips, SkipPlan P) {
+    __shared__ int s_scan[33], s_rep[4], s_live[4];
+    {
+        const SkipLaunch &L = P.l[blockIdx.x];
         int *rec = plan + L.rec;
         int *items = rec + kP2ItemsHeader, *skipped = items + L.total;
         const int *flags = skipped + L.nclass * L.tiles;
@@ -236,43 +262,96 @@
             rec[kRecFlagOff] = kP2ItemsHeader + L.total + L.nclass * L.tiles;
         }
         __syncthreads();
-    }
-}
-
-__global__ void __launch_bounds__(256) bev_skip_fill_kernel(const int *__restrict__ rec, float *__restrict__ out_f32,
-                                                            __half *__restrict__ out_planes, int cout) {
-    const int nskip = __ldg(rec + kRecSkipped);
-    if ((int)blockIdx.x >= nskip) return;
+        if (!strips) return;
+        int *srec = strips + L.srec;
+        int *full = srec + kP2StripHeader, *groups = full + L.total, *dead = groups + 8 * L.total;
+        const int *masks = dead + 8 * L.nclass * L.tiles;
+        int *lists = const_cast<int *>(masks) + L.nclass * L.tiles;
+        int nfull = 0, ngroups = 0, ndead = 0;
+        auto live = [&](int c, int t) {
+            const int m = masks[c * L.tiles + t];
+            return m != 0 && s_rep[c] == 0x7FFFFFFF ? 0xFF : m;
+        };
+        if (L.strips) {
+            nfull = skip_compact(L.total, [&](int g) {
+                const P2ItemIndex ix = p2_item_index(g, L.nblocks, L.tiles);
+                const int c = L.order[ix.rank];
+                return live(c, ix.t) == 0xFF || ix.t == s_rep[c];
+            }, full, s_scan);
+            for (int c = 0; c < L.nclass; ++c) {
+                const int n = skip_compact(8 * L.tiles, [&](int e) {
+                    const int m = live(c, e >> 3);
+                    return m != 0xFF && ((m >> (e & 7)) & 1);
+                }, lists + 8 * c * L.tiles, s_scan);
+                if (threadIdx.x == 0) s_live[c] = n;
+            }
+            __syncthreads();
+            for (int rank = 0; rank < L.nclass; ++rank) {
+                const int c = L.order[rank], n = s_live[c], ng = (n + 7) / 8;
+                const int *list = lists + 8 * c * L.tiles;
+                for (int nb = 0; nb < L.nblocks; ++nb) {
+                    int *grp = groups + 8 * ngroups;
+                    const int item0 = (rank * L.nblocks + nb) * L.tiles;
+                    for (int j = threadIdx.x; j < 8 * ng; j += blockDim.x)
+                        grp[j] = j < n ? (item0 + (list[j] >> 3)) * 8 + (list[j] & 7) : -1;
+                    ngroups += ng;
+                }
+            }
+            ndead = skip_compact(8 * L.nclass * L.tiles, [&](int e) {
+                const int m = live((e >> 3) / L.tiles, (e >> 3) % L.tiles);
+                return m != 0 && m != 0xFF && !((m >> (e & 7)) & 1);
+            }, dead, s_scan);
+        }
+        if (threadIdx.x == 0) {
+            srec[kSrecFull] = nfull; srec[kSrecGroups] = ngroups; srec[kSrecDead] = ndead;
+            srec[kSrecDeadOff] = kP2StripHeader + 9 * L.total;
+            srec[kSrecMaskOff] = kP2StripHeader + 9 * L.total + 8 * L.nclass * L.tiles;
+            srec[kSrecListOff] = kP2StripHeader + 9 * L.total + 9 * L.nclass * L.tiles;
+        }
+    }
+}
+
+__global__ void __launch_bounds__(256) bev_skip_fill_kernel(const int *__restrict__ rec, const int *__restrict__ srec,
+                                                            float *__restrict__ out_f32, __half *__restrict__ out_planes, int cout) {
+    const int nskip = __ldg(rec + kRecSkipped), ndead = srec ? __ldg(srec + kSrecDead) : 0;
+    if ((int)blockIdx.x >= nskip + ndead) return;
     const int tiles = __ldg(rec + kRecTiles), tiles_u = __ldg(rec + kRecTilesU), tiles_v = __ldg(rec + kRecTilesV);
     const int u_is_x = __ldg(rec + kRecUisX), os = __ldg(rec + kRecOutStride), out_h = __ldg(rec + kRecOutH), out_w = __ldg(rec + kRecOutW);
     const long long plane_stride = (long long)__ldg(rec + kRecBatch) * out_h * out_w * cout;
-    const int *skipped = rec + __ldg(rec + kRecSkipOff);
-    for (int e = blockIdx.x; e < nskip; e += gridDim.x) {
-        const int ent = __ldg(skipped + e);
+    const int *skipped = rec + __ldg(rec + kRecSkipOff), *dead = srec ? srec + __ldg(srec + kSrecDeadOff) : nullptr;
+    for (int e = blockIdx.x; e < nskip + ndead; e += gridDim.x) {
+        const int ent = e < nskip ? __ldg(skipped + e) : __ldg(dead + (e - nskip)) >> 3;
+        const int px0 = e < nskip ? 0 : kP2TileU * kP2StripV * (__ldg(dead + (e - nskip)) & 7);
+        const int npx = e < nskip ? kP2TileU * kP2TileV : kP2TileU * kP2StripV;
         const int c = ent / tiles, t = ent - c * tiles, r = __ldg(rec + kRecRep + c);
         const int oy0 = __ldg(rec + kRecOffY + c), ox0 = __ldg(rec + kRecOffX + c);
-        auto pixel = [&](int tt, int lu, int lv) -> size_t {
+        auto pixel = [&](int tt) -> size_t {
             const int tu = tt % tiles_u, rest = tt / tiles_u, tv = rest % tiles_v, b = rest / tiles_v;
-            const int gu = tu * kP2TileU + lu, gv = tv * kP2TileV + lv;
+            const int gu = tu * kP2TileU, gv = tv * kP2TileV;
             const int gy = u_is_x ? gv : gu, gx = u_is_x ? gu : gv;
             return ((size_t)b * out_h + (size_t)(gy * os + oy0)) * out_w + (size_t)(gx * os + ox0);
         };
+        const size_t du = (size_t)(u_is_x ? 1 : out_w) * os, dv = (size_t)(u_is_x ? out_w : 1) * os;
+        const size_t src0 = pixel(r), dst0 = pixel(t);
         if (out_f32) {
             const int q = cout / 4;
-            for (int i = threadIdx.x; i < kP2TileU * kP2TileV * q; i += blockDim.x) {
-                const int px = i / q, j = i - px * q;
-                const float4 v = reinterpret_cast<const float4 *>(out_f32 + pixel(r, px & 7, px >> 3) * cout)[j];
-                reinterpret_cast<float4 *>(out_f32 + pixel(t, px & 7, px >> 3) * cout)[j] = v;
+            for (int i = threadIdx.x; i < npx * q; i += blockDim.x) {
+                const int px = px0 + i / q, j = i - (i / q) * q;
+                const size_t o = (px & 7) * du + (px >> 3) * dv;
+                const float4 v = reinterpret_cast<const float4 *>(out_f32 + (src0 + o) * cout)[j];
+                reinterpret_cast<float4 *>(out_f32 + (dst0 + o) * cout)[j] = v;
             }
         }
         if (out_planes) {
-            const int q = cout / 8, n = kP2TileU * kP2TileV * q;
-            for (int i = threadIdx.x; i < 2 * n; i += blockDim.x) {
-                const int pl = i / n, k = i - pl * n, px = k / q, j = k - px * q;
-                const __half *src = out_planes + pl * plane_stride + pixel(r, px & 7, px >> 3) * cout;
-                __half *dst = out_planes + pl * plane_stride + pixel(t, px & 7, px >> 3) * cout;
-                reinterpret_cast<uint4 *>(dst)[j] = reinterpret_cast<const uint4 *>(src)[j];
-            }
+            const int q = cout / 8, n = npx * q;
+            for (int pl = 0; pl < 2; ++pl)
+                for (int i = threadIdx.x; i < n; i += blockDim.x) {
+                    const int px = px0 + i / q, j = i - (i / q) * q;
+                    const size_t o = (px & 7) * du + (px >> 3) * dv;
+                    const __half *src = out_planes + pl * plane_stride + (src0 + o) * cout;
+                    __half *dst = out_planes + pl * plane_stride + (dst0 + o) * cout;
+                    reinterpret_cast<uint4 *>(dst)[j] = reinterpret_cast<const uint4 *>(src)[j];
+                }
         }
     }
 }
@@ -289,7 +368,15 @@
     return words;
 }
 
-extern "C" int sessd_bev_skip_plan(const void *d_bitmap_index, sessd_grid grid, int *d_plan, void *stream) {
+extern "C" long long sessd_bev_skip_strip_words(int batch, int h, int w, int *offsets) {
+    SkipPlan P;
+    if (!skip_plan(P, batch, h, w)) return 0;
+    if (offsets)
+        for (int i = 0; i < kSkipLaunches; ++i) offsets[i] = P.l[i].srec;
+    return P.strip_words;
+}
+
+extern "C" int sessd_bev_skip_plan(const void *d_bitmap_index, sessd_grid grid, int *d_plan, int *d_strips, void *stream) {
     if (!d_bitmap_index || !d_plan || grid.shape[0] < 1) return SESSD_EINVAL;
     SkipPlan P;
     if (!skip_plan(P, grid.batch, grid.shape[1], grid.shape[2])) return SESSD_EINVAL;
@@ -301,12 +388,14 @@
         SESSD_CUDA_TRY(cudaFuncSetAttribute(bev_skip_plan_kernel, cudaFuncAttributeMaxDynamicSharedMemorySize, smem));
         attr_smem = smem;
     }
-    SESSD_LAUNCH(bev_skip_plan_kernel, 1, kSkipThreads, smem, (cudaStream_t)stream, (const uint2 *)d_bitmap_index, d_plan, P);
+    SESSD_LAUNCH(bev_skip_plan_kernel, 1, kSkipThreads, smem, (cudaStream_t)stream, (const uint2 *)d_bitmap_index, d_plan, d_strips, P);
+    SESSD_LAUNCH(bev_skip_lists_kernel, kSkipLaunches, kSkipThreads, 0, (cudaStream_t)stream, d_plan, d_strips, P);
     return last_error();
 }
 
-extern "C" int sessd_bev_skip_fill(const int *d_record, float *d_out_f32, void *d_out_planes, int cout, void *stream) {
+extern "C" int sessd_bev_skip_fill(const int *d_record, const int *d_strips, float *d_out_f32, void *d_out_planes, int cout, void *stream) {
     if (!d_record || (!d_out_f32 && !d_out_planes) || cout < 8 || cout % 8) return SESSD_EINVAL;
-    SESSD_LAUNCH(bev_skip_fill_kernel, 2 * kNumSMs, 256, 0, (cudaStream_t)stream, d_record, d_out_f32, (__half *)d_out_planes, cout);
+    SESSD_LAUNCH(bev_skip_fill_kernel, 2 * kNumSMs, 256, 0, (cudaStream_t)stream, d_record, d_strips, d_out_f32, (__half *)d_out_planes,
+                 cout);
     return last_error();
 }
diff --git a/se-ssd_b200/sessd_b200/_lib.py b/se-ssd_b200/sessd_b200/_lib.py
--- a/se-ssd_b200/sessd_b200/_lib.py
+++ b/se-ssd_b200/sessd_b200/_lib.py
@@ -80,11 +80,12 @@
     "sessd_spconv_wgrad_cg": (_i, [_vp, _i, _vp, _vp, _i, _vp, _vp, _i, _vp, _i, _vp, _vp, _sz, _vp]),
     "sessd_sparse_to_dense_indexed": (_i, [_vp, _i, _vp, _i, Grid, _vp, _vp]),
     "sessd_sparse_to_dense": (_i, [_vp, _vp, _vp, _i, _i, Grid, _vp, _vp]),
-    "sessd_bev_conv_p2": (_i, [_vp, _vp, _vp, _i, _vp, _vp, _vp, _vp, _f, _f, _vp, _vp, _vp, C.POINTER(ConvDesc), _vp, _vp]),
-    "sessd_bev_deconv_p2": (_i, [_vp, _vp, _vp, _i, _vp, _vp, _vp, _vp, _f, _f, _vp, _vp, _vp, _i, _i, _i, _i, _i, _i, _vp, _vp]),
+    "sessd_bev_conv_p2": (_i, [_vp, _vp, _vp, _i, _vp, _vp, _vp, _vp, _f, _f, _vp, _vp, _vp, C.POINTER(ConvDesc), _vp, _vp, _vp]),
+    "sessd_bev_deconv_p2": (_i, [_vp, _vp, _vp, _i, _vp, _vp, _vp, _vp, _f, _f, _vp, _vp, _vp, _i, _i, _i, _i, _i, _i, _vp, _vp, _vp]),
     "sessd_bev_skip_plan_words": (_ll, [_i, _i, _i, _I3]),
-    "sessd_bev_skip_plan": (_i, [_vp, Grid, _vp, _vp]),
-    "sessd_bev_skip_fill": (_i, [_vp, _vp, _vp, _i, _vp]),
+    "sessd_bev_skip_strip_words": (_ll, [_i, _i, _i, _I3]),
+    "sessd_bev_skip_plan": (_i, [_vp, Grid, _vp, _vp, _vp]),
+    "sessd_bev_skip_fill": (_i, [_vp, _vp, _vp, _vp, _i, _vp]),
     "sessd_bev_wgrad_items": (_i, [C.POINTER(ConvDesc)]),
     "sessd_bev_wgrad_workspace_bytes": (_sz, [C.POINTER(ConvDesc)]),
     "sessd_bev_wgrad": (_i, [_vp, _vp, _vp, _vp, C.POINTER(ConvDesc), _vp, _vp, _sz, _vp]),
diff --git a/se-ssd_b200/sessd_b200/ops.py b/se-ssd_b200/sessd_b200/ops.py
--- a/se-ssd_b200/sessd_b200/ops.py
+++ b/se-ssd_b200/sessd_b200/ops.py
@@ -331,19 +331,19 @@
 
 
 def bev_conv_p2(in_planes, in_info, weight_h2, scale, shift, residual, resid_info, gain, shift_max, out_f32, out_planes, out_info, desc,
-                items=None):
+                items=None, strips=None):
     check(lib.sessd_bev_conv_p2(_p(in_planes), _p(in_info), _p(weight_h2), int(weight_h2.shape[2]), _p(scale), _p(shift), _p(residual),
                                 _p(resid_info), float(gain), float(shift_max), _p(out_f32), _p(out_planes), _p(out_info), C.byref(desc),
-                                _p(items), _st()), "sessd_bev_conv_p2")
+                                _p(items), _p(strips), _st()), "sessd_bev_conv_p2")
 
 
 def bev_deconv_p2(in_planes, in_info, weight_h2, scale, shift, residual, resid_info, gain, shift_max, out_f32, out_planes, out_info, relu=True,
-                  items=None):
+                  items=None, strips=None):
     _two, b, h, w, cin = in_planes.shape
     cout = (out_f32 if out_f32 is not None else out_planes).shape[-1]
     check(lib.sessd_bev_deconv_p2(_p(in_planes), _p(in_info), _p(weight_h2), int(weight_h2.shape[2]), _p(scale), _p(shift), _p(residual),
                                   _p(resid_info), float(gain), float(shift_max), _p(out_f32), _p(out_planes), _p(out_info), int(b), int(h),
-                                  int(w), int(cin), int(cout), int(bool(relu)), _p(items), _st()), "sessd_bev_deconv_p2")
+                                  int(w), int(cin), int(cout), int(bool(relu)), _p(items), _p(strips), _st()), "sessd_bev_deconv_p2")
 
 
 class BevSkipPlan:
@@ -351,21 +351,27 @@
     LAUNCHES = 13
 
     def __init__(self, batch, h, w, device):
-        offs = (C.c_int * self.LAUNCHES)()
+        offs, soffs = (C.c_int * self.LAUNCHES)(), (C.c_int * self.LAUNCHES)()
         words = lib.sessd_bev_skip_plan_words(int(batch), int(h), int(w), offs)
         if words <= 0:
             raise ValueError("no skip plan for a [%d, %d, %d] neck" % (batch, h, w))
-        self.offsets = list(offs)
+        swords = lib.sessd_bev_skip_strip_words(int(batch), int(h), int(w), soffs)
+        self.offsets, self.strip_offsets = list(offs), list(soffs)
         self.buf = torch.zeros((int(words),), dtype=torch.int32, device=device)
+        self.strips = torch.zeros((int(swords),), dtype=torch.int32, device=device)
 
     def record(self, i):
         return self.buf[self.offsets[i]:]
 
+    def strip_record(self, i):
+        return self.strips[self.strip_offsets[i]:]
+
     def build(self, bitmap_index, grid):
-        check(lib.sessd_bev_skip_plan(_p(bitmap_index), grid, _p(self.buf), _st()), "sessd_bev_skip_plan")
-
-    def fill(self, i, out_f32, out_planes, cout):
-        check(lib.sessd_bev_skip_fill(_p(self.record(i)), _p(out_f32), _p(out_planes), int(cout), _st()), "sessd_bev_skip_fill")
+        check(lib.sessd_bev_skip_plan(_p(bitmap_index), grid, _p(self.buf), _p(self.strips), _st()), "sessd_bev_skip_plan")
+
+    def fill(self, i, out_f32, out_planes, cout, strips=True):
+        srec = self.strip_record(i) if strips else None
+        check(lib.sessd_bev_skip_fill(_p(self.record(i)), _p(srec), _p(out_f32), _p(out_planes), int(cout), _st()), "sessd_bev_skip_fill")
 
 
 def bev_split_planes(x, info, planes):
diff --git a/se-ssd_b200/sessd_b200/runners.py b/se-ssd_b200/sessd_b200/runners.py
--- a/se-ssd_b200/sessd_b200/runners.py
+++ b/se-ssd_b200/sessd_b200/runners.py
@@ -294,15 +294,16 @@
         resid, resid_info = (self.buf[L.residual], self._info(L.residual)) if L.residual else (None, None)
         i = self.SKIP_LAUNCHES.index(L.name)
         rec = self.skip.record(i) if skip else None
+        strips = self.skip.strip_record(i) if skip and L.stride == 1 else None
         if L.kind == "conv":
             d = launch_desc(L, self.batch, *ssfa_extents(L, self.h, self.w), q["taps"])
             ops.bev_conv_p2(self.planes[L.src], self._info(L.src), q["w"], q["scale"], q["shift"], resid, resid_info, q["gain"],
-                            q["shift_max"], out_f32, out_planes, self._info(L.dst), d, items=rec)
+                            q["shift_max"], out_f32, out_planes, self._info(L.dst), d, items=rec, strips=strips)
         else:
             ops.bev_deconv_p2(self.planes[L.src], self._info(L.src), q["w"], q["scale"], q["shift"], resid, resid_info, q["gain"],
-                              q["shift_max"], out_f32, out_planes, self._info(L.dst), L.relu, items=rec)
+                              q["shift_max"], out_f32, out_planes, self._info(L.dst), L.relu, items=rec, strips=strips)
         if skip:
-            self.skip.fill(i, out_f32, out_planes, L.cout)
+            self.skip.fill(i, out_f32, out_planes, L.cout, strips=strips is not None)
 
     def forward(self, x=None, mark=None, occupancy=None):
         assert self.params is not None, "load_state first"
```

After: 1573, median of 6. 1.02x the previous value.
